# ostadabbas/TePose

Measured on AMD Instinct MI355X. Metric: 16-frame windows/sec (whole node), higher is better.
Workload: dtype f32 via 3 fp16 MFMAs on hi+lo halves (22 bits/operand, fp32 acc); exact-f32 MFMA run = value_exact_fp32; 1 GPU; cfg-C synthetic [8192,16,2133] fp32 windows per GPU, TePose n_layers=2 hidden=1024, random-init weights, synthetic SMPL tables, H36M-14 joint path; seqlen=16, parallelism=clip-sharded dp1

## Files before the change

### tepose_amd/csrc/api.hip

```cpp
#include <stdlib.h>
#include <string.h>

#include <new>

#include "plan.h"

using namespace tepose;

static inline void fault_collected(const tepose_model* m) {
  std::lock_guard<std::mutex> g(m->q_mu);
  ++m->collected;
}

static void read_env_knobs(tepose_model* m) {
  m->opt = options_from_env();
  const char* e = getenv("TEPOSE_EXACT_FP32");
  m->split = m->split_env = !(e && atoi(e) != 0);
  e = getenv("TEPOSE_LARGE_BATCH_KERNELS");
  m->large_scaled = !(e && std::string(e) == "twoacc");
  e = getenv("TEPOSE_GRU_STATE");
  m->state_planes = !(e && std::string(e) == "fp32");
  e = getenv("TEPOSE_COLLAPSE_REGRESSOR");
  m->collapse_env = !(e && atoi(e) == 0);
  e = getenv("TEPOSE_S_MIN_B");
  m->s_min_b = e ? atoi(e) : 640;
  e = getenv("TEPOSE_PERSISTENT");
  m->persist = !(e && atoi(e) == 0);
  e = getenv("TEPOSE_SEQ_SPIN_LIMIT");
  if (e && atol(e) > 0) m->spin_limit = (unsigned)atol(e);
  e = getenv("TEPOSE_TEST_FAULT");
  m->test_fault = e ? (unsigned)atoi(e) : 0u;
  e = getenv("TEPOSE_BLEND16_MIN_N");
  m->blend16_min_n = e ? atoi(e) : 512;
  e = getenv("TEPOSE_GI_BLK");
  m->gi_blk = e ? atoi(e) : 1;
  refresh_kernel_info(m);
}

extern "C" {

int tepose_version(void) { return TEPOSE_ABI_VERSION; }

const char* tepose_build_info(void) {
#ifdef TEPOSE_NO_PACKED_FP32
  return "gfx950 packed_fp32=off";
#else
  return "gfx950 packed_fp32=on";
#endif
}

const char* tepose_kernel_info(const tepose_model* m) { return m ? m->kinfo.c_str() : ""; }

const char* tepose_select_kernels(const tepose_model* m, int B, int T) {
  static thread_local std::string buf;
  if (!m || B < 1 || T < 1) return "";
  buf = describe_plan(m, B, T);
  return buf.c_str();
}

const char* tepose_error_string(int code) {
  switch (code) {
    case 0: return "ok";
    case TEPOSE_E_ARG: return "tepose: bad argument";
    case TEPOSE_E_SHAPE: return "tepose: unsupported shape";
    case TEPOSE_E_WORKSPACE: return "tepose: workspace too small";
    case TEPOSE_E_STATE: return "tepose: model not packed";
    case TEPOSE_E_TIMEOUT: return "tepose: a persistent kernel's bounded wait expired (GPU shared or CU-masked?); "
                                  "outputs of that forward are NaN -- tepose_status() clears, TEPOSE_PERSISTENT=0 / "
                                  "tepose_set_persistent(m, 0) selects the step-per-launch kernels";
    default: return code > 0 ? hipGetErrorString((hipError_t)code) : "tepose: unknown error";
  }
}

int tepose_create(int n_layers, int hidden, tepose_model** out) {
  if (!out || n_layers < 1 || hidden < 1) return TEPOSE_E_ARG;
  if (n_layers > 8 || hidden > 8192) return TEPOSE_E_SHAPE;
  tepose_model* m = new (std::nothrow) tepose_model();
  if (!m) return TEPOSE_E_ARG;
  m->L = n_layers; m->H = hidden; m->Hp = round_up(hidden, 64);
  read_env_knobs(m);
  layout(m);
  *out = m;
  return 0;
}

void tepose_destroy(tepose_model* m) {
  if (!m) return;
  for (hipEvent_t e : m->ev) (void)hipEventDestroy(e);
  for (hipEvent_t e : m->ev_gru) (void)hipEventDestroy(e);
  if (m->fault) (void)hipHostFree(m->fault);
  delete m;
}


int tepose_status_peek(const tepose_model* m) {
  if (!m) return TEPOSE_E_ARG;
  return fault_pending(m) ? TEPOSE_E_TIMEOUT : 0;
}

int tepose_status(tepose_model* m, void* stream) {
  if (!m) return TEPOSE_E_ARG;
  CK(hipStreamSynchronize((hipStream_t)stream));
  if (!m->fault) return 0;
  const unsigned code = __atomic_exchange_n(m->fault, 0u, __ATOMIC_RELAXED);
  if (code) { m->last_fault_code = (int)code; fault_collected(m); }
  return code != 0u ? TEPOSE_E_TIMEOUT : 0;
}

int tepose_forward_status(tepose_model* m, void* workspace, void* stream) {
  if (!m || !workspace) return TEPOSE_E_ARG;
  hipStream_t s = (hipStream_t)stream;
  CK(hipStreamSynchronize(s));
  if (m->fault && __atomic_load_n(m->fault, __ATOMIC_RELAXED) == 0u) {
    std::lock_guard<std::mutex> g(m->q_mu);
    auto it = m->q_gen.find(workspace);
    if (it != m->q_gen.end() && it->second == m->collected) return 0;
  }
  unsigned* sy = (unsigned*)workspace;
  unsigned span[32 + 96 + 1];
  static_assert(sizeof(span) == (32 + 96 + 1) * sizeof(unsigned), "span");
  CK(hipMemcpyAsync(span, sync_gru_status(m, sy), sizeof(span), hipMemcpyDeviceToHost, s));
  CK(hipStreamSynchronize(s));
  const unsigned st[2] = {span[0], span[32 + 96]};
  if ((st[0] | st[1]) == 0u) return 0;
  CK(hipMemsetAsync(sync_gru_status(m, sy), 0, sizeof(unsigned), s));
  CK(hipMemsetAsync(sync_reg_status(m, sy), 0, sizeof(unsigned), s));
  CK(hipStreamSynchronize(s));
  m->last_fault_code = (int)(st[0] ? st[0] : st[1]);
  if (m->fault && __atomic_exchange_n(m->fault, 0u, __ATOMIC_RELAXED) != 0u) fault_collected(m);
  return TEPOSE_E_TIMEOUT;
}

int tepose_set_option(tepose_model* m, const char* name, long value) {
  if (!m || !name) return TEPOSE_E_ARG;
  if (m->enc_packed || m->reg_packed || m->smpl_packed || m->vibe_packed || m->bb_packed) return TEPOSE_E_STATE;
  const char* n = strncmp(name, "TEPOSE_", 7) == 0 ? name + 7 : name;
  if (int* f = option_field(m->opt, n)) *f = (int)value;
  else if (strcmp(n, "S_MIN_B") == 0) m->s_min_b = (int)value;
  else if (strcmp(n, "BLEND16_MIN_N") == 0) m->blend16_min_n = (int)value;
  else if (strcmp(n, "GI_BLK") == 0) m->gi_blk = (int)value;
  else if (strcmp(n, "SEQ_SPIN_LIMIT") == 0) { if (value <= 0) return TEPOSE_E_ARG; m->spin_limit = (unsigned)value; }
  else return TEPOSE_E_ARG;
  refresh_kernel_info(m);
  return 0;
}

long tepose_get_option(const tepose_model* m, const char* name) {
  if (!m || !name) return -1;
  const char* n = strncmp(name, "TEPOSE_", 7) == 0 ? name + 7 : name;
  Options o = m->opt;
  if (const int* f = option_field(o, n)) return *f;
  if (strcmp(n, "S_MIN_B") == 0) return m->s_min_b;
  if (strcmp(n, "BLEND16_MIN_N") == 0) return m->blend16_min_n;
  if (strcmp(n, "GI_BLK") == 0) return m->gi_blk;
  if (strcmp(n, "SEQ_SPIN_LIMIT") == 0) return (long)m->spin_limit;
  return -1;
}

int tepose_fault_code(const tepose_model* m) {
  if (!m) return TEPOSE_E_ARG;
  const unsigned live = m->fault ? __atomic_load_n(m->fault, __ATOMIC_RELAXED) : 0u;
  return live ? (int)live : m->last_fault_code;
}

int tepose_set_persistent(tepose_model* m, int on) {
  if (!m) return TEPOSE_E_ARG;
  __atomic_store_n(&m->persist, on != 0, __ATOMIC_RELAXED);
  return 0;
}

unsigned tepose_debug_kernel_errors(void) { return h3s16c_read_err(); }

int tepose_debug_set_test_fault(tepose_model* m, unsigned bits) {
  if (!m) return TEPOSE_E_ARG;
  m->test_fault = bits;
  return 0;
}

int tepose_uses_persistent(const tepose_model* m, int B, int T) {
  if (!m || B < 1) return 0;
  if (!persist_on(m) || !m->split || B <= m->opt.split_min_m) return 0;
  const int cap = seq_rows_cap(m) > reg_seq_rows_cap(m) ? seq_rows_cap(m) : reg_seq_rows_cap(m);
  (void)T;
  return B <= cap ? 1 : 0;
}

int tepose_create_vibe_ex(int n_layers, int hidden, int bidirectional, int add_linear, tepose_model** out) {
  if (!out || n_layers < 1 || hidden < 1) return TEPOSE_E_ARG;
  if (n_layers > 8 || hidden > 8192) return TEPOSE_E_SHAPE;
  tepose_model* m = new (std::nothrow) tepose_model();
  if (!m) return TEPOSE_E_ARG;
  m->kind = 1; m->L = n_layers; m->H = hidden; m->Hp = round_up(hidden, 64);
  m->vibe_bidir = bidirectional != 0;
  m->vibe_linear = bidirectional != 0 || add_linear != 0;
  read_env_knobs(m);
  layout_vibe(m);
  *out = m;
  return 0;
}

int tepose_create_hmr(tepose_model** out) {
  if (!out) return TEPOSE_E_ARG;
  tepose_model* m = new (std::nothrow) tepose_model();
  if (!m) return TEPOSE_E_ARG;
  m->kind = 2;
  m->L = 1; m->H = m->Hp = 64;
  read_env_knobs(m);
  layout_hmr(m);
  *out = m;
  return 0;
}

int tepose_create_vibe(int n_layers, int hidden, tepose_model** out) {
  return tepose_create_vibe_ex(n_layers, hidden, 0, 1, out);
}

int tepose_vibe_feature_dim(const tepose_model* m) {
  if (!m || m->kind != 1) return 0;
  return m->vibe_linear ? kFeat : m->H;
}

int tepose_profile_enable(tepose_model* m, int on) {
  if (!m) return TEPOSE_E_ARG;
  m->prof = on != 0;
  m->ev_used = 0;
  m->prof_flops = 0.0;
  m->ev_gru_used = 0;
  m->prof_gru_flops = 0.0;
  m->prof_l1_flops = 0.0;
  return 0;
}

int tepose_profile_read(tepose_model* m, double* total_ms, int* n_launches, double* flops_per_launch) {
  if (!m || !total_ms || !n_launches || !flops_per_launch) return TEPOSE_E_ARG;
  double tot = 0.0;
  for (size_t i = 0; i + 1 < m->ev_used; i += 2) {
    CK(hipEventSynchronize(m->ev[i + 1]));
    float ms = 0.f;
    CK(hipEventElapsedTime(&ms, m->ev[i], m->ev[i + 1]));
    tot += ms;
  }
  *total_ms = tot;
  *n_launches = (int)(m->ev_used / 2);
  *flops_per_launch = m->prof_flops;
  m->ev_used = 0;
  return 0;
}

int tepose_profile_read_gru(tepose_model* m, double* total_ms, int* n_forwards, double* flops_per_forward) {
  if (!m || !total_ms || !n_forwards || !flops_per_forward) return TEPOSE_E_ARG;
  double tot = 0.0;
  for (size_t i = 0; i + 1 < m->ev_gru_used; i += 2) {
    CK(hipEventSynchronize(m->ev_gru[i + 1]));
    float ms = 0.f;
    CK(hipEventElapsedTime(&ms, m->ev_gru[i], m->ev_gru[i + 1]));
    tot += ms;
  }
  const int nf = (int)(m->ev_gru_used / (2 * (size_t)m->L));
  *total_ms = tot;
  *n_forwards = nf;
  *flops_per_forward = nf > 0 ? m->prof_gru_flops / nf : 0.0;
  m->ev_gru_used = 0;
  m->prof_gru_flops = 0.0;
  m->prof_l1_flops = 0.0;
  return 0;
}

int tepose_profile_read_l1proj(tepose_model* m, double* total_ms, int* n_forwards, double* flops_per_forward) {
  if (!m || !total_ms || !n_forwards || !flops_per_forward) return TEPOSE_E_ARG;
  const size_t per = 2 * (size_t)m->L;
  double tot = 0.0;
  for (size_t f = 0; (f + 1) * per <= m->ev_gru_used; ++f)
    for (int l = 1; l < m->L; ++l) {
      CK(hipEventSynchronize(m->ev_gru[f * per + 2 * l]));
      float ms = 0.f;
      CK(hipEventElapsedTime(&ms, m->ev_gru[f * per + 2 * l - 1], m->ev_gru[f * per + 2 * l]));
      tot += ms;
    }
  const int nf = (int)(m->ev_gru_used / per);
  *total_ms = tot;
  *n_forwards = nf;
  *flops_per_forward = nf > 0 ? m->prof_l1_flops / nf : 0.0;
  return 0;
}

int tepose_metrics_joints(const float* pred, const float* target, int N, int J, int pelvis_mode, float* mpjpe,
                          float* pa_mpjpe, float* accel, void* stream) {
  if (!pred || !target || !mpjpe || !pa_mpjpe || !accel || N < 1) return TEPOSE_E_ARG;
  if (J < 4 || J > 17 || (pelvis_mode != 0 && pelvis_mode != 1)) return TEPOSE_E_SHAPE;
  CK(launch_metrics_joints(pred, target, N, J, pelvis_mode, mpjpe, pa_mpjpe, accel, (hipStream_t)stream));
  return 0;
}

int tepose_metrics_verts(const float* pred_verts, const float* target_verts, int N, float* mpvpe, void* stream) {
  if (!pred_verts || !target_verts || !mpvpe || N < 1) return TEPOSE_E_ARG;
  CK(launch_metrics_verts(pred_verts, target_verts, N, mpvpe, (hipStream_t)stream));
  return 0;
}

int tepose_filter_one_euro(float* x, int N, int D, float min_cutoff, float beta, float d_cutoff, void* stream) {
  if (!x || N < 1 || D < 1) return TEPOSE_E_ARG;
  CK(launch_one_euro(x, N, D, min_cutoff, beta, d_cutoff, (hipStream_t)stream));
  return 0;
}

int tepose_filter_slerp(const float* rotmat_in, float* rotmat_out, int N, int J, double ratio, void* stream) {
  if (!rotmat_in || !rotmat_out || N < 1 || J < 1) return TEPOSE_E_ARG;
  CK(launch_slerp_smooth(rotmat_in, rotmat_out, N, J, ratio, (hipStream_t)stream));
  return 0;
}

int tepose_rotmat_to_angle_axis(const float* R, int N, float* aa, void* stream) {
  if (!R || !aa || N < 1) return TEPOSE_E_ARG;
  CK(launch_rotmat_to_aa(R, N, aa, (hipStream_t)stream));
  return 0;
}

int tepose_rot6d_to_rotmat(const float* x6, int N, float* R, void* stream) {
  if (!x6 || !R || N < 1) return TEPOSE_E_ARG;
  CK(launch_rot6d_to_rotmat(x6, N, R, (hipStream_t)stream));
  return 0;
}

size_t tepose_gemm_h3_workspace_bytes(int M, int N, int K) {
  if (M < 1 || N < 1 || K < 1) return 0;
  const size_t a = gemm_h3_ws_bytes(M, N, K), b = gemm_h3s_ws_bytes(M, N, K);
  return a > b ? a : b;
}

int tepose_gemm_h3_f32(const float* A, long lda, const float* W, long ldw, const float* bias, float* C, long ldc,
                       int M, int N, int K, void* workspace, size_t ws_bytes, void* stream) {
  if (!A || !W || !C || !workspace || M < 1 || N < 1 || K < 1) return TEPOSE_E_ARG;
  if (K % 32 != 0) return TEPOSE_E_SHAPE;
  if (ws_bytes < gemm_h3_ws_bytes(M, N, K)) return TEPOSE_E_WORKSPACE;
  const char* pe = getenv("TEPOSE_H3S");
  const Options opt = options_from_env();
  if (pe && pe[0] && std::string(pe) != "0" && std::string(pe).rfind("skinny", 0) != 0 && ws_bytes >= gemm_h3s_ws_bytes(M, N, K)) {
    CK(launch_gemm_h3s_f32(A, lda, W, ldw, C, ldc, M, N, K, 256.f, 16384.f, workspace, (hipStream_t)stream, opt, bias, std::string(pe) == "mid" ? 1 : 0));
    return 0;
  }
  CK(launch_gemm_h3_f32(A, lda, W, ldw, bias, C, ldc, M, N, K, workspace, (hipStream_t)stream, opt, pe && std::string(pe) == "skinny" ? 1 : 0));
  return 0;
}

size_t tepose_gemm_workspace_bytes(int N, int K) {
  if (N < 1 || K < 1) return 0;
  return (size_t)round_up(N, 128) * round_up(K, 32) * sizeof(float) + 256;
}

int tepose_gemm_f32(const float* A, long lda, const float* W, long ldw, const float* bias, float* C, long ldc,
                    int M, int N, int K, int relu_a, void* workspace, size_t ws_bytes, void* stream) {
  if (!A || !W || !C || !workspace || M < 1 || N < 1 || K < 1) return TEPOSE_E_ARG;
  if (lda % 4 != 0 || ((uintptr_t)A & 15) != 0 || K % 32 != 0) return TEPOSE_E_SHAPE;
  if (ws_bytes < tepose_gemm_workspace_bytes(N, K)) return TEPOSE_E_WORKSPACE;
  hipStream_t s = (hipStream_t)stream;
  float* wp = (float*)workspace;
  CK((hipError_t)pack(W, ldw, N, K, wp, round_up(N, 128), K, 0, 0, 0, 1, s));
  const GemmArgs g{A, lda, wp, K, C, ldc, bias, nullptr, 0, 1.f, M, N, relu_a};
  CK(launch_gemm(g, s, options_from_env()));
  return 0;
}

}
```

### tepose_amd/csrc/blob.hip

```cpp
#include <algorithm>

#include "hmr.h"
#include "model.h"

using namespace tepose;

namespace {

constexpr size_t kAlignF = 64;

size_t take(size_t& cur, size_t n) {
  const size_t o = cur;
  cur = align_up(cur + n, kAlignF);
  return o;
}

void take_w(size_t& cur, Weight& w, size_t Np, size_t Kp, size_t nb = 0) {
  w.Np = (int)Np; w.Kp = (int)Kp;
  w.w = take(cur, Np * Kp);
  if (nb) w.b = take(cur, nb);
}

void plane(tepose_model* m, size_t& cur, Owner owner, Weight& dst, int rows, size_t R, Fmt f, const Weight* src = nullptr, int k0 = 0) {
  if (f == Fmt::scaled) { dst.s = take(cur, R * dst.Kp); dst.Rs = (int)R; }
// ... 215 lines not shown
    CK(launch_dmm(G3, 1, S, B + m->init, 0, 1, nullptr, 0, nullptr, 0, t2, 1, S, 1, S, 1.0, 0, s));
    CK(launch_dmm(Ss, 1, S, c, 1, 1, t2, 1, nullptr, 0, k0, 1, S, 1, S, 1.0, 0, s));
    CK(launch_d2f_pad(Mf, kFeat, S, kFeat, B + m->mf.w, m->mf.Np, m->mf.Kp, s));
    CK(launch_d2f_pad(k0, S, 1, S, B + m->mf.b, 1, kState, s));
    CK((hipError_t)derive_planes(m, Owner::collapsed_regressor, s));
    CK(hipStreamSynchronize(s));
    return 0;
  };
  const int rc = run();
  (void)hipFree(d);
  if (rc) return rc;
  bool ok = false;
  CK((hipError_t)range_check(m, m->mf.w, m->mf.p, &ok, s));
  m->reg_collapsed = ok;
  return 0;
}

int collapse_tail(tepose_model* m, hipStream_t s) {
  m->tail_collapsed = false;
  if (m->kind != 0 || !m->collapse_env || !m->reg_collapsed || !m->enc_packed) return 0;
  constexpr int S = 157;
  const int Hp = m->Hp, K3 = 3 * Hp;
  float* B = m->blob;
  double* d = nullptr;
  CK(hipMalloc((void**)&d, ((size_t)S * K3 + 2 * S) * sizeof(double)));
  double *Mt = d, *t = Mt + (size_t)S * K3, *kt = t + S;
  auto run = [&]() -> int {
    CK(launch_dmm(B + m->mf.w, 0, kFeat, B + m->wlf.w, 0, Hp, nullptr, 0, nullptr, 0, Mt, K3, S, Hp, kFeat, 0.5, 0, s));
    CK(launch_dmm(B + m->mf.w, 0, kFeat, B + m->wlr.w, 0, 2 * Hp, nullptr, 0, nullptr, 0, Mt + Hp, K3, S, 2 * Hp, kFeat, 0.5, 0, s));
    CK(launch_dmm(B + m->mf.w, 0, kFeat, B + m->wlf.b, 0, 1, nullptr, 0, nullptr, 0, t, 1, S, 1, kFeat, 0.5, 0, s));
    CK(launch_dmm(B + m->mf.w, 0, kFeat, B + m->wlr.b, 0, 1, t, 1, B + m->mf.b, 1, kt, 1, S, 1, kFeat, 0.5, 0, s));
    CK(launch_d2f_pad(Mt, K3, S, K3, B + m->mt.w, m->mt.Np, m->mt.Kp, s));
    CK(launch_d2f_pad(kt, S, 1, S, B + m->mt.b, 1, kState, s));
    CK((hipError_t)derive_planes(m, Owner::collapsed_tail, s));
    CK(hipStreamSynchronize(s));
    return 0;
  };
  const int rc = run();
  (void)hipFree(d);
  if (rc) return rc;
  bool ok = false;
  CK((hipError_t)range_check(m, m->mt.w, m->mt.p, &ok, s));
  m->tail_collapsed = ok;
  return 0;
}
}

extern "C" {

size_t tepose_packed_bytes(const tepose_model* m) { return m ? m->blob_floats * sizeof(float) : 0; }

int tepose_set_blob(tepose_model* m, void* blob, size_t bytes) {
  if (!m || !blob) return TEPOSE_E_ARG;
  if (bytes < m->blob_floats * sizeof(float)) return TEPOSE_E_WORKSPACE;
  m->blob = (float*)blob;
  h3s16c_warm();
  if (!m->fault) {
    unsigned* f = nullptr;
    if (hipHostMalloc((void**)&f, 64, hipHostMallocDefault) == hipSuccess && f) { *f = 0u; m->fault = f; }
    else (void)hipGetLastError();
  }
  return 0;
}

int tepose_adopt_blob(tepose_model* m) {
  if (!m) return TEPOSE_E_ARG;
  if (!m->blob) return TEPOSE_E_STATE;
  BlobHeader h{};
  CK(hipMemcpy(&h, m->blob + m->hdr, sizeof(h), hipMemcpyDeviceToHost));
  const uint64_t lf = ((uint64_t)h.layout_floats_hi << 32) | h.layout_floats_lo;
  if (h.magic != kBlobMagic || h.abi != TEPOSE_ABI_VERSION || h.kind != header_kind(m) || (int)h.L != m->L ||
      (int)h.H != m->H || (int)h.Hp != m->Hp || lf != (uint64_t)m->blob_floats)
    return TEPOSE_E_STATE;
  m->enc_packed = m->kind == 0 && (h.sections & 1u);
  m->vibe_packed = m->kind == 1 && (h.sections & 1u);
  m->reg_packed = (h.sections & 2u) != 0;
  m->smpl_packed = (h.sections & 4u) != 0;
  m->bb_packed = m->kind == 2 && (h.sections & 64u) != 0;
  m->enc_range_ok = m->reg_range_ok = m->smpl_range_ok = m->bb_range_ok = !(h.sections & 8u);
  m->reg_collapsed = m->collapse_env && (h.sections & 16u) != 0;
  m->tail_collapsed = m->collapse_env && m->kind == 0 && (h.sections & 32u) != 0;
  m->split = m->split_env && m->enc_range_ok;
  m->maxdepth = kNJ - 1;
  int max_nnz = kNJ;
  CK(hipMemcpy(&max_nnz, m->blob + m->smpl.lbs_nnz, sizeof(int), hipMemcpyDeviceToHost));
  m->lbs_sparse = max_nnz <= 4 ? 1 : 0;
  for (const PlaneSpec& p : m->planes) {
    if (p.fmt != Fmt::scaled || (p.owner == Owner::encoder && !m->enc_packed)) continue;
    CK(hipMemcpy(&p.dst->scale, m->blob + p.dst->scale_at, sizeof(float), hipMemcpyDeviceToHost));
    if (!(p.dst->scale > 0.f)) p.dst->scale = 1.f;
  }
  return 0;
}

int tepose_fp32_ranges(const tepose_model* m, size_t* offsets, size_t* sizes, int cap) {
  if (!m || !offsets || !sizes) return TEPOSE_E_ARG;
  std::vector<std::pair<size_t, size_t>> derived, r;
  for (const PlaneSpec& p : m->planes) {
    const Weight& w = *p.dst;
    if (p.fmt == Fmt::blocked) derived.emplace_back(w.p, align_up(w.p + (size_t)w.Rp * w.Kp, kAlignF));
    else {
      derived.emplace_back(w.s, align_up(w.s + (size_t)w.Rs * w.Kp, kAlignF));
      derived.emplace_back(w.scale_at / kAlignF * kAlignF, w.scale_at / kAlignF * kAlignF + kAlignF);
    }
  }
  derived.emplace_back(m->blob_floats, m->blob_floats);
  std::sort(derived.begin(), derived.end());
  size_t at = 0;
  for (const auto& d : derived) {
    if (d.first > at) r.emplace_back(at, d.first);
    at = std::max(at, d.second);
  }
  if ((int)r.size() > cap) return TEPOSE_E_ARG;
  for (size_t i = 0; i < r.size(); ++i) { offsets[i] = r[i].first * sizeof(float); sizes[i] = (r[i].second - r[i].first) * sizeof(float); }
  return (int)r.size();
}

int tepose_derive_planes(tepose_model* m, void* stream) {
  if (!m) return TEPOSE_E_ARG;
  if (!m->blob) return TEPOSE_E_STATE;
  int rc = tepose_adopt_blob(m);
  if (rc) return rc;
  hipStream_t s = (hipStream_t)stream;
  const bool enc = m->kind == 0 && m->enc_packed;
  const std::pair<Owner, bool> owners[] = {{Owner::encoder, enc}, {Owner::collapsed_tail, enc && m->tail_collapsed}, {Owner::regressor, m->reg_packed},
                                           {Owner::collapsed_regressor, m->reg_packed && m->reg_collapsed}, {Owner::smpl, m->smpl_packed},
                                           {Owner::backbone, m->bb_packed}};
  for (const auto& o : owners)
    if (o.second) CK((hipError_t)derive_planes(m, o.first, s));
  CK(hipStreamSynchronize(s));
  return 0;
}

int tepose_pack_vibe_encoder(tepose_model* m, const float* const* w, int n_w, void* stream) {
  if (!m || !w || m->kind != 1) return TEPOSE_E_ARG;
  if (!m->blob) return TEPOSE_E_STATE;
  const int L = m->L, H = m->H, Hp = m->Hp, D = m->vibe_bidir ? 2 : 1;
  if (n_w != 4 * L * D + (m->vibe_linear ? 2 : 0)) return TEPOSE_E_ARG;
  for (int i = 0; i < n_w; ++i)
    if (!w[i]) return TEPOSE_E_ARG;
  hipStream_t s = (hipStream_t)stream;
  const Packer pk{m, s};
  const int cmap = D == 2 ? COL_SPLIT2 : COL_PLAIN;
  for (int l = 0; l < L; ++l) {
    const int K = l == 0 ? kFeat : D * H;
    for (int d = 0; d < D; ++d) {
      const float* const* q = w + 4 * (l * D + d);
      const WView ih(m->vibe[l].ih, d * 3 * Hp), hh(m->vibe[l].hh, d * 3 * Hp);
      CK((hipError_t)pk.rows(q[0], K, 3 * H, K, ih, d == D - 1 ? 0 : 3 * Hp, ROW_GATES, l == 0 ? COL_PLAIN : cmap));
      CK((hipError_t)pk.bias(q[2], 3 * H, ih, 3 * Hp, ROW_GATES));
      CK((hipError_t)pk.rows(q[1], H, 3 * H, H, hh, 3 * Hp, ROW_GATES_TILED, COL_PLAIN));
      CK((hipError_t)pk.bias(q[3], 3 * H, hh, 3 * Hp, ROW_GATES));
    }
  }
  if (m->vibe_linear) {
    CK((hipError_t)pk.rows(w[4 * L * D], D * H, kFeat, D * H, m->vlin, 0, ROW_PLAIN, cmap));
    CK((hipError_t)pk.bias(w[4 * L * D + 1], kFeat, m->vlin, kFeat, ROW_PLAIN));
  }
  m->vibe_packed = true;
  CK((hipError_t)range_check(m, m->vibe[0].ih.w, m->w1a.w, &m->enc_range_ok, s));
  return write_header(m, s);
}

int tepose_pack_hmr_backbone(tepose_model* m, const float* const* w, int n_w, void* stream) {
  if (!m || !w || m->kind != 2 || n_w != 5 * kHmrConvs) return TEPOSE_E_ARG;
  if (!m->blob) return TEPOSE_E_STATE;
  for (int i = 0; i < n_w; ++i)
    if (!w[i]) return TEPOSE_E_ARG;
  hipStream_t s = (hipStream_t)stream;
  float* B = m->blob;
  int* err = (int*)(B + m->hdr + 48);
  m->bb_packed = false;
  CK(hipMemsetAsync(err, 0, sizeof(int), s));
  int rc = hmr_walk(1, [&](const ConvStep& c) {
    const float* const* q = w + 5 * c.idx;
    const Weight& bw = m->bb[c.idx];
    return (int)launch_hmr_fold_pack(q[0], q[1], q[2], q[3], q[4], c.l->cout, c.l->cin, c.l->R, B + bw.w, bw.Np, bw.Kp, B + bw.b, err, s);
  });
  if (rc) return rc;
  int bad = 0;
  CK(hipMemcpyAsync(&bad, err, sizeof(int), hipMemcpyDeviceToHost, s));
  CK(hipStreamSynchronize(s));
  if (bad) return TEPOSE_E_ARG;
  CK((hipError_t)derive_planes(m, Owner::backbone, s));
  m->bb_packed = true;
  CK((hipError_t)range_check(m, m->bb[0].w, m->bb[0].p, &m->bb_range_ok, s));
  return write_header(m, s);
}

int tepose_pack_encoder(tepose_model* m, const float* const* w, int n_w, void* stream) {
  if (!m || !w || m->kind != 0) return TEPOSE_E_ARG;
  if (!m->blob) return TEPOSE_E_STATE;
  const int L = m->L, H = m->H, Hp = m->Hp;
  if (n_w != 12 * L + 4) return TEPOSE_E_ARG;
  for (int i = 0; i < n_w; ++i)
    if (!w[i]) return TEPOSE_E_ARG;
  hipStream_t s = (hipStream_t)stream;
  float* B = m->blob;
  const Packer pk{m, s};
  CK(launch_fill(B + m->wih0.w, (size_t)m->wih0.Np * m->wih0.Kp, 0.f, s));
  auto fwd_w = [&](int l, int k) { return w[4 * l + k]; };
  auto rec_w = [&](int l, int rev, int k) { return w[4 * L + 8 * l + 4 * rev + k]; };
  const float* l0[3] = {fwd_w(0, 0), rec_w(0, 1, 0), rec_w(0, 0, 0)};
  const float* l0b[3] = {fwd_w(0, 2), rec_w(0, 1, 2), rec_w(0, 0, 2)};
  for (int d = 0; d < 3; ++d) {
    const WView v(m->wih0, d * 3 * Hp);
    CK((hipError_t)pk.rows(l0[d], kInput, 3 * H, kInput, v, 3 * Hp, ROW_GATES, COL_PLAIN));
    CK((hipError_t)pk.bias(l0b[d], 3 * H, v, 3 * Hp, ROW_GATES));
  }
  for (int l = 0; l < L; ++l) {
    struct { DirW* d; const float *ih, *hh, *bih, *bhh; bool split; } dirs[3] = {
        {&m->fwd[l], fwd_w(l, 0), fwd_w(l, 1), fwd_w(l, 2), fwd_w(l, 3), false},
        {&m->rec_f[l], rec_w(l, 0, 0), rec_w(l, 0, 1), rec_w(l, 0, 2), rec_w(l, 0, 3), true},
        {&m->rec_r[l], rec_w(l, 1, 0), rec_w(l, 1, 1), rec_w(l, 1, 2), rec_w(l, 1, 3), true}};
    for (auto& d : dirs) {
      if (l > 0) {
        const int K = d.split ? 2 * H : H;
        CK((hipError_t)pk.rows(d.ih, K, 3 * H, K, d.d->ih, 0, ROW_GATES, d.split ? COL_SPLIT2 : COL_PLAIN));
        CK((hipError_t)pk.bias(d.bih, 3 * H, d.d->ih, 3 * Hp, ROW_GATES));
      }
      CK((hipError_t)pk.rows(d.hh, H, 3 * H, H, d.d->hh, 0, ROW_GATES_TILED, COL_PLAIN));
      CK((hipError_t)pk.bias(d.bhh, 3 * H, d.d->hh, 3 * Hp, ROW_GATES));
    }
  }
  const float* const* t = w + 12 * L;
  CK((hipError_t)pk.rows(t[0], H, kFeat, H, m->wlf, 0, ROW_PLAIN, COL_PLAIN));
  CK((hipError_t)pk.bias(t[1], kFeat, m->wlf, kFeat, ROW_PLAIN));
  CK((hipError_t)pk.rows(t[2], 2 * H, kFeat, 2 * H, m->wlr, 0, ROW_PLAIN, COL_SPLIT2));
  CK((hipError_t)pk.bias(t[3], kFeat, m->wlr, kFeat, ROW_PLAIN));
  CK((hipError_t)derive_planes(m, Owner::encoder, s));
  m->enc_packed = true;
  CK((hipError_t)range_check(m, m->wih0.w, m->wih0.p, &m->enc_range_ok, s));
  CK((hipError_t)collapse_tail(m, s));
  return write_header(m, s);
}

int tepose_pack_regressor(tepose_model* m, const float* const* w, int n_w, void* stream) {
  if (!m || !w || n_w != 13) return TEPOSE_E_ARG;
  if (!m->blob) return TEPOSE_E_STATE;
  for (int i = 0; i < n_w; ++i)
    if (!w[i]) return TEPOSE_E_ARG;
  hipStream_t s = (hipStream_t)stream;
  float* B = m->blob;
  const Packer pk{m, s};
  const int ld1 = kFeat + kNPose + 13;
  CK((hipError_t)pk.rows(w[0], ld1, 1024, kFeat, m->w1a, 0, ROW_PLAIN, COL_PLAIN));
  CK((hipError_t)pk.bias(w[1], 1024, m->w1a, 1024, ROW_PLAIN));
  CK((hipError_t)pk.rows(w[0] + kFeat, ld1, 1024, 157, m->w1b, 0, ROW_PLAIN, COL_PLAIN));
  CK((hipError_t)pk.rows(w[2], 1024, 1024, 1024, m->w2, 0, ROW_PLAIN, COL_PLAIN));
  CK((hipError_t)pk.bias(w[3], 1024, m->w2, 1024, ROW_PLAIN));
  CK(launch_fill(B + m->wdec.w, (size_t)m->wdec.Np * m->wdec.Kp, 0.f, s));
  CK(launch_fill(B + m->wdec.b, kState, 0.f, s));
  CK(launch_fill(B + m->init, kState, 0.f, s));
  const int rows[3] = {kNPose, 10, 3}, off[3] = {0, kNPose, kNPose + 10};
  for (int i = 0; i < 3; ++i) {
    const WView v(m->wdec, off[i]);
    CK((hipError_t)pk.rows(w[4 + 2 * i], 1024, rows[i], 1024, v, rows[i], ROW_PLAIN, COL_PLAIN));
    CK((hipError_t)pk.bias(w[5 + 2 * i], rows[i], v, rows[i], ROW_PLAIN));
    CK((hipError_t)pack(w[10 + i], 1, rows[i], 1, B + m->init + off[i], rows[i], 1, 0, 0, 0, 1, s));
  }
  CK((hipError_t)derive_planes(m, Owner::regressor, s));
  m->reg_packed = true;
  CK((hipError_t)range_check(m, m->w1a.w, m->smpl.J0, &m->reg_range_ok, s));
  CK((hipError_t)collapse_regressor(m, s));
  CK((hipError_t)collapse_tail(m, s));
  return write_header(m, s);
}

int tepose_pack_smpl(tepose_model* m, const float* v_template, const float* shapedirs,
                     const float* posedirs, const float* J_regressor, const float* lbs_weights,
                     const float* J_regressor_extra, const int32_t* parents_host, void* stream) {
  if (!m || !v_template || !shapedirs || !posedirs || !J_regressor || !lbs_weights ||
      !J_regressor_extra || !parents_host)
    return TEPOSE_E_ARG;
  if (!m->blob) return TEPOSE_E_STATE;
  hipStream_t s = (hipStream_t)stream;
  float* B = m->blob;
  int par[kNJ], dep[kNJ];
  for (int j = 0; j < kNJ; ++j) {
    par[j] = j == 0 ? -1 : parents_host[j];
    if (j > 0 && (par[j] < 0 || par[j] >= j)) return TEPOSE_E_ARG;
  }
  const int maxd = chain_depths(par, dep);
  m->maxdepth = maxd;
  CK(hipMemcpyAsync(B + m->smpl.parents, par, sizeof(par), hipMemcpyHostToDevice, s));
  CK(hipMemcpyAsync(B + m->smpl.depth, dep, sizeof(dep), hipMemcpyHostToDevice, s));
  CK(hipStreamSynchronize(s));
  CK(launch_smpl_consts(v_template, shapedirs, posedirs, J_regressor, B + m->smpl.J0, B + m->smpl.JS,
                        B + m->blend.w, s));
  CK((hipError_t)pack(lbs_weights, kNJ, kNV, kNJ, B + m->smpl.lbsW, kNV, kNJ, 0, 0, 0, 1, s));
  CK(launch_lbs_compact(lbs_weights, (int*)(B + m->smpl.lbs_cidx), B + m->smpl.lbs_cval, (int*)(B + m->smpl.lbs_nnz), s));
  int max_nnz = 0;
  CK(hipMemcpyAsync(&max_nnz, B + m->smpl.lbs_nnz, sizeof(int), hipMemcpyDeviceToHost, s));
  CK(hipStreamSynchronize(s));
  m->lbs_sparse = max_nnz <= 4 ? 1 : 0;
  CK(launch_csr_build(J_regressor_extra, 9, kNV, (int*)(B + m->smpl.xr_ptr), (int*)(B + m->smpl.xr_idx),
                      B + m->smpl.xr_val, 9 * kNV, s));
  CK((hipError_t)derive_planes(m, Owner::smpl, s));
  m->smpl_packed = true;
  CK((hipError_t)range_check(m, m->smpl.J0, m->smpl.lbs_cidx, &m->smpl_range_ok, s));
  return write_header(m, s);
}

size_t tepose_jreg_packed_bytes(void) { return (32 + (size_t)17 * kNV * 2) * 4; }

int tepose_pack_jreg(const float* J, void* packed, void* stream) {
  if (!J || !packed) return TEPOSE_E_ARG;
  int* p = (int*)packed;
  CK(launch_csr_build(J, 17, kNV, p, p + 32, (float*)(p + 32 + 17 * kNV), 17 * kNV, (hipStream_t)stream));
  return 0;
}

}
```

### tepose_amd/csrc/common.h

```cpp
#pragma once
#include <hip/hip_runtime.h>
#include <stdint.h>

#include "formats.h"
#include "shapes.h"

namespace tepose {

typedef _Float16 half_t;
constexpr float kLoScale = 2048.f;
__host__ __device__ inline void split_hi_lo(float a, half_t& hi, half_t& lo) {
  hi = (half_t)a;
  lo = (half_t)((a - (float)hi) * kLoScale);
}
__host__ __device__ inline void split_hi_lo16(float v, half_t& hi, half_t& lo) {
  hi = (half_t)v;
  lo = (half_t)(v - (float)hi);
}

inline dim3 grid_of(const Launch& l) { return dim3(l.gx, l.gy, l.gz); }
inline dim3 block_of(const Launch& l) { return dim3(l.threads); }

struct GemmArgs {
  const float* A; long lda;
  const float* W; int Kp;
  float* C; long ldc;
  const float* bias;
  const float* addend; long ldadd;
  float scale;
  int M, N;
  int relu_a;
};
hipError_t launch_gemm(const GemmArgs& a, hipStream_t s, const Options& o);
hipError_t launch_gemm_tiles(const GemmArgs& a, hipStream_t s, const Options& o);

struct GruDir {
  const float* hprev; long ldh;
  const float* Whh;
  const float* bhh;
  const float* gi; long ldgi;
  float* hout; long ldo;
  long gi_blk = 0;
  const float* hprev_b = nullptr; long hp_blk = 0;
  float* hout_b = nullptr; long ho_blk = 0;
};
struct GruArgs {
  GruDir d[3];
  int ndir;
  int M, Hp;
  int first;
};
hipError_t launch_gru_step(const GruArgs& a, hipStream_t s, const Options& o);
hipError_t launch_gru_step_tiles(const GruArgs& a, hipStream_t s);
hipError_t launch_skinny_gemm(const GemmArgs& a, hipStream_t s);
hipError_t launch_skinny_gru(const GruArgs& a, hipStream_t s);

enum RowMap { ROW_PLAIN = 0, ROW_GATES = 1, ROW_GATES_TILED = 2 };
enum ColMap { COL_PLAIN = 0, COL_SPLIT2 = 1 };
struct PackArgs {
  const float* src; long ld_src; int N, K;
  float* dst; int Np, Kp;
  int rowmap, colmap;
  int H, Hp;
};
hipError_t launch_pack(const PackArgs& a, hipStream_t s);
hipError_t launch_pad_input(const float* x, float* xp, long rows, hipStream_t s);
hipError_t launch_pad_rows(const float* feat, long feat_ld, const float* theta, long theta_ld, float* xp,
                           long rows, hipStream_t s);
hipError_t launch_fill(float* p, size_t n, float v, hipStream_t s);
hipError_t launch_dmm(const void* A, int a64, long lda, const void* B, int b64, long ldb, const double* Cadd, long ldadd,
                      const float* Cadd32, long ldadd32, double* C, long ldc, int M, int N, int K, double alpha,
                      int add_identity, hipStream_t s);
hipError_t launch_d2f_pad(const double* src, long ld, int rows, int cols, float* dst, int Rp, int Cp, hipStream_t s);
hipError_t launch_copy_cols(const float* src, long lds, const float* add, long lda, float* dst, long ldd, long rows,
                            int cols, hipStream_t s);
struct TapView;
hipError_t launch_tap_gather(const TapView& v, const float* ws, float* out, hipStream_t s);
hipError_t launch_init_state(const float* init160, float* xs, int N, hipStream_t s);
hipError_t launch_init_state_rows(const float* init160, const float* pose, const float* shape, const float* cam,
                                  float* xs, int N, hipStream_t s);
hipError_t launch_rotmat_to_aa(const float* R, int N, float* aa, hipStream_t s);
hipError_t launch_rot6d_to_rotmat(const float* x6, int N, float* R, hipStream_t s);

struct SmplConsts {
  const float* J0;
  const float* JS;
  const float* blendW;
  const float* lbsW;
  const int* lbs_cidx;
  const float* lbs_cval;
  int lbs_sparse;
  const int* parents;
  const int* depth;
  int maxdepth;
  const int* xr_ptr;
  const int* xr_idx;
  const float* xr_val;
};
struct JregPacked {
  const int* ptr; const int* idx; const float* val;
};
hipError_t launch_smpl_prep(const SmplConsts& c, const float* xs, int N, float* pf, float* Amat,
                            float* posed, float* rotmat, float* theta, hipStream_t s, void* pf_hi = nullptr,
                            void* pf_lo = nullptr, long pf_kst = 0);
hipError_t launch_smpl_prep_pose(const SmplConsts& c, int mode, const float* pose, int pose_ld,
                                 const float* betas, int betas_ld, int N, float* pf, float* Amat, float* posed,
                                 hipStream_t s, void* pf_hi = nullptr, void* pf_lo = nullptr, long pf_kst = 0);
bool smpl_small_rows_ok(int N, const Options& o);
hipError_t launch_smpl_small(const SmplConsts& c, int mode, const float* pose, int pose_ld, const float* betas, int betas_ld,
                             const float* cam, int cam_ld, int N, float* Amat, float* posed, float* rotmat, float* theta,
                             float* verts, hipStream_t s);
hipError_t launch_smpl_person(const SmplConsts& c, const float* pf, const float* Amat, int N, float* verts, hipStream_t s);
hipError_t launch_lbs_compact(const float* lbsW, int* cidx, float* cval, int* max_nnz, hipStream_t s);
hipError_t launch_smpl_skin(const SmplConsts& c, const float* vposed, const float* Amat, int N,
                            float* verts, hipStream_t s);
hipError_t launch_smpl_joints(const SmplConsts& c, const JregPacked* jr, const float* verts,
                              const float* posed, const float* xs, int N, float* kp3d,
                              float* kp2d, hipStream_t s);
hipError_t launch_csr_build(const float* dense, int rows, int cols, int* ptr, int* idx, float* val,
                            int cap, hipStream_t s);
hipError_t launch_smpl_consts(const float* v_template, const float* shapedirs, const float* posedirs,
                              const float* J_regressor, float* J0, float* JS, float* blendW,
                              hipStream_t s);

hipError_t launch_smpl_joints_bwd(const float* g_j49, int N, float* gsrc, hipStream_t s);
hipError_t launch_smpl_skin_bwd(const SmplConsts& c, const float* vposed, const float* Amat, const float* g_verts, const float* gsrc, int N,
                                float* gvp, float* partial, hipStream_t s);
hipError_t launch_smpl_blend_bwd(const float* blendW, const float* gvp, int N, float* part, float* gf, hipStream_t s);
hipError_t launch_smpl_chain_bwd(const SmplConsts& c, int mode, const float* pose, const float* betas, int N, const float* partial,
                                 const float* gsrc, const float* gf, float* g_pose, float* g_betas, hipStream_t s);

hipError_t launch_metrics_joints(const float* pred, const float* target, int N, int J, int pelvis_mode,
                                 float* mpjpe, float* pa, float* accel, hipStream_t s);
hipError_t launch_metrics_verts(const float* pred, const float* target, int N, float* mpvpe, hipStream_t s);

hipError_t launch_one_euro(float* x, int N, int D, float min_cutoff, float beta, float d_cutoff, hipStream_t s);
hipError_t launch_slerp_smooth(const float* in, float* out, int N, int J, double ratio, hipStream_t s);
hipError_t launch_session_smooth(const float* theta, const float* hist, int S, int T, const int* ops, float* state, float* saved, float min_cutoff,
                                 float beta, float d_cutoff, float* theta_hat, float* pose_hat, float* betas_hat, hipStream_t s);

struct H3Args {
  const half_t *Ah, *Al; long a_kst;
  const half_t *Wh, *Wl; long w_kst;
  int Kp;
  float* C; long ldc;
  const float* bias;
  int M, N;
  const float* addend; long ldadd;
  float scale;
  half_t *Chi, *Clo; long c_kst;
  const float* row_scale;
  int grp_rows, grp_stride;
  float* C2; long ldc2; int c_split;
};
struct GateDir {
  const float* gi; long ldgi;
  const float* bhh;
  const float* hprev; long ldh;
  float* hout; long ldo;
  half_t *hout_hi, *hout_lo; long okst;
  long gi_blk = 0;
  const float* hprev_b = nullptr; long hp_blk = 0;
  float* hout_b = nullptr; long ho_blk = 0;
};
struct H3Batch { H3Args p[3]; GateDir gate[3]; int n; int Hp; };
hipError_t launch_gemm_h3(const H3Batch& b, hipStream_t s, const Options& o);
hipError_t launch_gru_h3(const H3Batch& b, hipStream_t s);
hipError_t launch_skinny_gru_h3(const H3Batch& b, hipStream_t s);
hipError_t launch_skinny_gemm_h3(const H3Args& a, hipStream_t s, const Options& o);
struct H3ArgsBatch { H3Args p[3]; int n; };
hipError_t launch_skinny_gemm_h3_batch(const H3ArgsBatch& b, hipStream_t s, const Options& o);
struct GruSeqStep {
  const float* gi; float* hout;
  int ldgi, ldo;
  unsigned poff, pkst;
};
struct GruSeqArgs {
  GruSeqStep st[3][kSeqMaxT];
  const half_t* whi[3]; const half_t* wlo[3]; long w_kst;
  const float* bhh[3];
  half_t *phi, *plo;
  unsigned* counters;
  unsigned* status;
  unsigned* fault;
  unsigned spin_limit;
  unsigned inject;
  int ndir, T, M, Hp;
  const float* x_gi; const float* x_bhh; float* x_hout;
  int x_ldgi, x_ldo;
  unsigned x_poff, x_pkst;
  half_t *rhi, *rlo;
  unsigned r_off[3], x_roff, r_kst;
  unsigned long long* stamps;
  unsigned long long* gran;
  unsigned tag_base;
};
constexpr unsigned kNoPlane = 0xffffffffu;
struct RegSeqArgs {
  const half_t *fh, *fl; long f_kst;
  const half_t *w1a_h, *w1a_l, *w1b_h, *w1b_l, *w2_h, *w2_l, *wd_h, *wd_l;
  const float *b1, *b2, *bdec;
  const float *init160, *ipose, *ishape, *icam;
  half_t *h1h, *h1l, *h2h, *h2l; long h_kst;
  half_t *xh, *xl; long x_kst;
  float* xs;
  unsigned* counters;
  unsigned* status;
  unsigned* fault; unsigned spin_limit; unsigned inject;
  int N, n_iter;
};
hipError_t launch_reg_seq(const RegSeqArgs& a, hipStream_t s);
int device_cus(const Options& o);
hipError_t launch_gru_seq(const GruSeqArgs& a, hipStream_t s, const Options& o);
struct GateBatch { GateDir d[3]; };
hipError_t launch_gru_first(const GateBatch& gb, int ndir, int M, int Hp, hipStream_t s, int scaled16 = 0, bool rows16 = false);
hipError_t launch_split_planes(const float* src, long ld, long rows, int K, int Kp, long R, void* hi, void* lo,
                               hipStream_t s, int relu = 0);
struct RowPairSrc { const float* f0; const float* th0; const float* f1; long fld, thld; long B; };
hipError_t launch_split_rows(const float* src, long ld, long rows, int K, int Kp, long R, int fmt16, void* hi, void* lo,
                             float* row_scale, hipStream_t s, bool few, void* zero = nullptr, size_t zero_bytes = 0,
                             int permT = 0, const RowPairSrc* pair = nullptr);
hipError_t launch_gemm_h3_f32(const float* A, long lda, const float* W, long ldw, const float* bias, float* C,
                              long ldc, int M, int N, int K, void* ws, hipStream_t s, const Options& o, int kind = 0);
size_t gemm_h3_ws_bytes(int M, int N, int K);
constexpr float kStateScale = 16384.f;
struct H3SArgs {
  const half_t *Ah, *Al; long a_kst;
  const half_t *Wh, *Wl; long w_kst;
  int Kp;
  float* C; long ldc;
  const float* bias;
  float inv_scale;
  int M, N;
  const float* row_scale;
  unsigned* status = nullptr;
  unsigned* fault = nullptr;
  unsigned inject = 0;
  int c_blk_hp = 0;
};
struct H3SBatch { H3SArgs p[3]; GateDir gate[3]; int n; int Hp; float state_scale; };
hipError_t launch_gemm_h3s(const H3SArgs& a, hipStream_t s, const Options& o, int tag = 1);
bool gemm_h3s16_ok(const H3SArgs& a);
hipError_t launch_gemm_h3s16c(const H3SArgs& a, hipStream_t s, int tag, int gm, int walk);
unsigned h3s16c_read_err();
void h3s16c_warm();
bool gru_step16_ok(const H3SBatch& b);
bool gru_step16_planes_ok(const H3SBatch& b);
hipError_t launch_gru_step16(const H3SBatch& b, hipStream_t s, bool planes, int gm);
unsigned* h3s16c_err_of_device();
bool gemm_h3s_mid_ok(const H3SArgs& a);
hipError_t launch_gemm_h3s_mid(const H3SArgs& a, hipStream_t s);
hipError_t launch_split_planes16(const float* src, long ld, long rows, int K, int Kp, long R, float p, void* hi,
                                 void* lo, hipStream_t s);
hipError_t launch_absmax(const float* src, size_t n, float* out, hipStream_t s);
size_t gemm_h3s_ws_bytes(int M, int N, int K);
hipError_t launch_gemm_h3s_f32(const float* A, long lda, const float* W, long ldw, float* C, long ldc, int M, int N,
                               int K, float pA, float pW, void* ws, hipStream_t s, const Options& o, const float* bias = nullptr,
                               int mid = 0);

}
```

### tepose_amd/csrc/forward.hip

```cpp
#include "plan.h"
#include "state.h"
#include "tap.h"

using namespace tepose;

namespace {

struct Carver : Carve {
  char* base; size_t cap;
  Carver(void* p, size_t c) : base((char*)p), cap(c) {}
  float* at(size_t off) const { return base && off != kNoRef ? (float*)base + off : nullptr; }
  float* f(size_t n) { return at(take(n)); }
};

Planes carve_planes(Carver& c, size_t R, size_t C, bool on) {
  Planes p;
  p.hi = (half_t*)c.f(on ? R * C / 2 + 64 : 0);
  p.lo = (half_t*)c.f(on ? R * C / 2 + 64 : 0);
  p.kst = (long)R * 32;
  return p;
}

struct EncWs {
  EncLayout o;
  float* base = nullptr;
  float *xp, *g0, *g0c, *y1, *rs, *rs0;
  half_t *state_hi, *state_lo, *x0h, *x0l;
  unsigned long long* gran;
  unsigned* sync;
  size_t Bs = 0;
  float* at(size_t off) const { return base && off != kNoRef ? base + off : nullptr; }
  float* rows(const StateBuf& b) const { return at(b.off); }
  Planes planes(const StateRef& r) const { return Planes{state_hi + r.p, state_lo + r.p, r.kst}; }
  Planes tail(long k0) const {
    half_t *hi = (half_t*)at(o.tailA.hi), *lo = (half_t*)at(o.tailA.lo);
    return Planes{hi ? hi + o.tailA.k(k0) : nullptr, lo ? lo + o.tailA.k(k0) : nullptr, o.tailA.kst};
  }
};

inline size_t seq_gran_words(const tepose_model* m, const KernelPlan& k) { return k.gran ? (size_t)3 * 2 * kSeqGranRows * m->Hp * 2 : 0; }
inline size_t sync_zero_bytes(const tepose_model* m, const KernelPlan& k) {
  return align_up(sync_words(m) * sizeof(unsigned), 256) + seq_gran_words(m, k) * sizeof(float);
}

void carve_encoder(const tepose_model* m, const KernelPlan& k, int B, int T, Carver& c, EncWs& w) {
  w.o = carve_encoder(EncShape{m->L, m->Hp, B, T, k.h3, k.scaled, k.gblk, sync_words(m), seq_gran_words(m, k)}, c);
  const EncLayout& o = w.o;
  w.base = (float*)c.base; w.Bs = o.Bs;
  w.sync = (unsigned*)c.at(o.sync); w.gran = (unsigned long long*)c.at(o.gran);
  w.xp = c.at(o.xp); w.g0 = c.at(o.g0); w.g0c = c.at(o.g0c); w.y1 = c.at(o.y1); w.rs = c.at(o.rs); w.rs0 = c.at(o.rs0);
  w.state_hi = (half_t*)c.at(o.state_hi); w.state_lo = (half_t*)c.at(o.state_lo);
  w.x0h = (half_t*)c.at(o.x0h); w.x0l = (half_t*)c.at(o.x0l);
}

bool carve_encoder(const tepose_model* m, const KernelPlan& k, int B, int T, void* workspace, size_t bytes, EncWs& w) {
  Carver c(workspace, bytes);
  carve_encoder(m, k, B, T, c, w);
  return c.cur <= bytes;
}

struct Act {
  float* rows = nullptr; long ld = 0; Planes P;
  AOperand A() const { return AOperand{rows, ld, P}; }
};

struct RegWs {
  unsigned* sync;
  bool split;
  Act feat, xs, h1, h2, pf;
  float *base, *amat, *posed, *vposed;
  half_t *pf16h = nullptr, *pf16l = nullptr; float* pfrs = nullptr;
};

void carve_regressor(const tepose_model* m, const KernelPlan& k, int N, Carver& c, RegWs& w) {
  w.split = k.h3;
  w.sync = (unsigned*)c.f(sync_words(m));
  w.feat.ld = kFeat; w.xs.ld = kState; w.h1.ld = w.h2.ld = 1024; w.pf.ld = kBlendK;
  for (Act* a : {&w.feat, &w.xs, &w.h1, &w.h2, &w.pf}) a->P = carve_planes(c, N, a->ld, w.split);
  w.base = c.f((size_t)N * 1024);
  for (Act* a : {&w.h1, &w.h2, &w.xs, &w.pf}) a->rows = c.f((size_t)N * a->ld);
  w.amat = c.f((size_t)N * kNJ * 12);
  w.posed = c.f((size_t)N * kNJ * 3);
  w.vposed = c.f((size_t)N * kVertLd);
  if (k.blend16) {
    w.pf16h = (half_t*)c.f((size_t)N * kBlendK / 2);
    w.pf16l = (half_t*)c.f((size_t)N * kBlendK / 2);
    w.pfrs = c.f((size_t)N);
  }
}

bool carve_regressor(const tepose_model* m, const KernelPlan& k, int N, void* workspace, size_t bytes, RegWs& w) {
  Carver c(workspace, bytes);
  carve_regressor(m, k, N, c, w);
  return c.cur <= bytes;
}

hipError_t init_state(const float* init160, const float* pose, const float* shape, const float* cam, float* xs, int N,
                      hipStream_t s) {
  if (pose || shape || cam) return launch_init_state_rows(init160, pose, shape, cam, xs, N, s);
  return launch_init_state(init160, xs, N, s);
}

H3Args h3_args(const float* blob, const AOperand& A, WView W, float* C, long ldc, int M, int N, const Epilogue& e) {
  const WPlanes wp = w_planes(blob, W, Fmt::blocked);
  H3Args p{A.p.hi, A.p.lo, A.p.kst, wp.hi, wp.lo, wp.kst, W.w->Kp, C, ldc, e.bias, M, N};
  p.addend = e.addend; p.ldadd = e.ldadd; p.scale = e.scale; p.row_scale = A.row_scale;
  if (e.out) { p.Chi = e.out->hi; p.Clo = e.out->lo; p.c_kst = e.out->kst; }
  return p;
}

H3SArgs h3s_args(const tepose_model* m, const AOperand& A, WView W, float* C, long ldc, int M, int N, const Epilogue& e) {
  const WPlanes ws = w_planes(m->blob, W, Fmt::scaled);
  H3SArgs a{A.s.hi, A.s.lo, A.s.kst, ws.hi, ws.lo, ws.kst, W.w->Kp, C, ldc, e.bias, W.w->inv_scale(A.s_scale), M, N, A.row_scale};
  if (e.sync) a.status = e.reg ? sync_reg_status(m, e.sync) : sync_gru_status(m, e.sync);
  a.fault = m->fault;
  a.inject = e.reg ? 0u : (m->test_fault >> 2) & 1u;
  a.c_blk_hp = e.c_blk_hp;
  return a;
}

}

int tepose::product(const tepose_model* m, Mm f, const AOperand& A, WView W, float* C, long ldc, int M, int N, const Epilogue& e, hipStream_t s, bool tail_stage) {
  switch (f) {
    case Mm::f32: return (int)launch_gemm_tiles(f32_args(m->blob, A, W, C, ldc, M, N, e), s, m->opt);
    case Mm::f32_skinny: return (int)launch_skinny_gemm(f32_args(m->blob, A, W, C, ldc, M, N, e), s);
    case Mm::h3:
    case Mm::h3_skinny: {
      H3Batch b{};
      b.p[0] = h3_args(m->blob, A, W, C, ldc, M, N, e);
      if (f == Mm::h3_skinny || (tail_stage && N <= 256)) return (int)launch_skinny_gemm_h3(b.p[0], s, m->opt);
      b.n = 1;
      return (int)launch_gemm_h3(b, s, m->opt);
    }
    case Mm::h3s_mid: return (int)launch_gemm_h3s_mid(h3s_args(m, A, W, C, ldc, M, N, e), s);
    case Mm::h3s0:
    case Mm::h3s: return (int)launch_gemm_h3s(h3s_args(m, A, W, C, ldc, M, N, e), s, m->opt, e.tag);
  }
  return (int)hipErrorInvalidValue;
}

namespace {

int tail_product(const tepose_model* m, const KernelPlan& plan, const AOperand& A, WView W, float* C, long ldc, int M, int N, const Epilogue& e, hipStream_t s) {
  return product(m, plan.tail, A, W, C, ldc, M, N, e, s, true);
}

int blend_shapes(const tepose_model* m, const KernelPlan& k, const RegWs& w, int N, hipStream_t s) {
  AOperand A = w.pf.A();
  Epilogue e;
  if (k.smpl == Smpl::h3s) {
    CK(launch_split_rows(w.pf.rows, kBlendK, N, kBlendK, kBlendK, N, 1, w.pf16h, w.pf16l, w.pfrs, s, k.input_blend == Rows::split_few));
    A.s = Planes{w.pf16h, w.pf16l, (long)N * 16}; A.row_scale = w.pfrs;
    e.sync = w.sync; e.reg = true;
  }
  const Mm f = k.smpl == Smpl::h3s ? Mm::h3s : k.smpl == Smpl::h3 ? Mm::h3 : k.smpl == Smpl::f32_skinny ? Mm::f32_skinny : Mm::f32;
  return product(m, f, A, m->blend, w.vposed, kVertLd, N, 3 * kNV, e, s);
}

template <class Small, class Prep>
int smpl_chain(const tepose_model* m, const KernelPlan& k, const SmplConsts& sc, const RegWs& w, int N, float* verts, hipStream_t s, Small small, Prep prep) {
  if (k.smpl == Smpl::small) return (int)small();
  CK(prep(w.split ? w.pf.P.hi : nullptr, w.split ? w.pf.P.lo : nullptr, w.pf.P.kst));
  CK((hipError_t)blend_shapes(m, k, w, N, s));
  CK(launch_smpl_skin(sc, w.vposed, w.amat, N, verts, s));
  return 0;
}

JregPacked jreg_view(const void* jreg_packed) {
  const int* p = (const int*)jreg_packed;
  return JregPacked{p, p + 32, (const float*)(p + 32 + 17 * kNV)};
}

struct G0Src {
  const float* base; long frame_stride, row_stride;
  int first, ring;
  const float* last; long last_ld;
  const float* single; long single_ld;
  long blk = 0;
};

tepose_model* prof_of(const tepose_model* m) { return m->prof ? const_cast<tepose_model*>(m) : nullptr; }
int prof_mark(std::vector<hipEvent_t>& ev, size_t& used, hipStream_t s) {
  if (ev.size() < used + 1) {
    hipEvent_t e;
    CK(hipEventCreate(&e));
    ev.push_back(e);
  }
  CK(hipEventRecord(ev[used++], s));
  return 0;
}

struct Gi { const float* p; long ld, blk; };
Gi gate_in(const G0Src& src, const EncWs& w, int T, int H3, int l, int dir, const DirStep& d) {
  if (l > 0) return Gi{w.at(d.gi.f), d.gi.ld, d.gi.bst};
  if (d.frame < 0) return Gi{src.single, src.single_ld, 0};
  if (src.last && d.frame == T - 1) return Gi{src.last + (long)dir * H3, src.last_ld, src.blk};
  const int slot = src.ring ? (src.first + d.frame) % src.ring : d.frame;
  return Gi{src.base + (long)slot * src.frame_stride + (long)dir * H3 * (src.blk ? 16 : 1), src.row_stride, src.blk};
}

struct LayerDirs { const DirW* d[3]; };
LayerDirs layer_dirs(const tepose_model* m, int l) { return LayerDirs{{&m->fwd[l], &m->rec_r[l], &m->rec_f[l]}}; }

int project_l1(const tepose_model* m, const KernelPlan& plan, const EncWs& w, Mm f, const StateBuf& in, const DirW& d, const StateBuf& out, int M, hipStream_t s) {
  const int H3 = 3 * m->Hp;
  AOperand A{w.rows(in), d.ih.Kp};
  if (f == Mm::h3s) { A.s = w.planes(in.at(0)); A.s_scale = kStateScale; }
  Epilogue e{w_bias(m->blob, d.ih)};
  e.sync = w.sync; e.c_blk_hp = plan.gblk ? m->Hp : 0;
  return product(m, f, A, d.ih, w.rows(out), H3, M, H3, e, s);
}

int layer_projections(const tepose_model* m, const KernelPlan& plan, const EncWs& w, int B, int T, int l, hipStream_t s) {
  const int Hp = m->Hp, H3 = 3 * Hp;
  const float* Bl = m->blob;
  const long Bs = (long)w.Bs;
  const bool top = l == m->L - 1;
  const StateBuf &inf = w.o.sf[(l - 1) & 1], &inr = w.o.sr[(l - 1) & 1];
  const int MT = (int)(Bs * T);
  const int Mf = top ? B : MT;
  const Mm ff = top ? plan.proj_one : plan.proj_l1;
  if (plan.proj_l1 != Mm::h3 && plan.proj_l1 != Mm::h3_skinny) {
    CK((hipError_t)project_l1(m, plan, w, plan.proj_l1, inf, m->fwd[l], w.o.gf, MT, s));
    CK((hipError_t)project_l1(m, plan, w, plan.proj_l1, inr, m->rec_r[l], w.o.grr, MT, s));
    return project_l1(m, plan, w, ff, inr, m->rec_f[l], w.o.grf, Mf, s);
  }
  const Planes vf = w.planes(inf.at(0)), vr = w.planes(inr.at(0));
  auto mk = [&](const Planes& v, const DirW& d, float* out, int M) {
    return h3_args(Bl, AOperand{nullptr, 0, v}, d.ih, out, H3, M, H3, Epilogue{w_bias(Bl, d.ih)});
  };
  H3Args pa[3] = {mk(vr, m->rec_r[l], w.rows(w.o.grr), MT), mk(vr, m->rec_f[l], w.rows(w.o.grf), Mf), mk(vf, m->fwd[l], w.rows(w.o.gf), MT)};
  const Mm fam[3] = {plan.proj_l1, ff, plan.proj_l1};
  H3ArgsBatch sk{};
  H3Batch big{};
  for (int i = 0; i < 3; ++i) {
    H3Args& a = pa[i];
    if (fam[i] == Mm::h3_skinny) {
      if (a.M == MT && Bs != B) { a.M = B * T; a.grp_rows = B; a.grp_stride = (int)Bs; }
      sk.p[sk.n++] = a;
    }
    else if (big.n == 0 || (big.p[0].M == a.M && big.p[0].N == a.N)) big.p[big.n++] = a;
    else {
      H3Batch one{};
      one.p[0] = a; one.n = 1;
      CK(launch_gemm_h3(one, s, m->opt));
    }
  }
  if (big.n) CK(launch_gemm_h3(big, s, m->opt));
  if (sk.n) CK(launch_skinny_gemm_h3_batch(sk, s, m->opt));
  return 0;
}


GruArgs gru_args(const tepose_model* m, const G0Src& src, const EncWs& w, int B, int T, int l, const CellStep& c, const LayerDirs& dw) {
  GruArgs a{};
  a.M = B; a.Hp = m->Hp; a.first = c.first; a.ndir = c.ndir;
  for (int k = 0; k < c.ndir; ++k) {
    const DirStep& q = c.d[k];
    const Gi gi = gate_in(src, w, T, 3 * m->Hp, l, k, q);
    GruDir& d = a.d[k];
    d.Whh = w_rows(m->blob, dw.d[k]->hh); d.bhh = w_bias(m->blob, dw.d[k]->hh);
    d.gi = gi.p; d.ldgi = gi.ld; d.gi_blk = gi.blk;
    d.hprev = w.at(q.hprev.f); d.ldh = q.hprev.ld;
    d.hout = w.at(q.hout.f); d.ldo = q.hout.ld;
  }
  return a;
}

int launch_cell_step(const tepose_model* m, const KernelPlan& plan, const G0Src& src, const EncWs& w, Step f, int B, int T, int l, const CellStep& c,
                     const LayerDirs& dw, hipStream_t s) {
  if (f == Step::f32_skinny) return (int)launch_skinny_gru(gru_args(m, src, w, B, T, l, c, dw), s);
  if (f == Step::f32) return (int)launch_gru_step_tiles(gru_args(m, src, w, B, T, l, c, dw), s);
  const int Hp = m->Hp, H3 = 3 * Hp;
  const bool s16 = f == Step::s16 || f == Step::s16_planes;
  H3SBatch b16{};
  H3Batch b{};
  GateBatch gb{};
  for (int d = 0; d < c.ndir; ++d) {
    const DirStep& q = c.d[d];
    const Gi gi = gate_in(src, w, T, H3, l, d, q);
    const Planes vo = w.planes(q.hout);
    GateDir g{gi.p, gi.ld, w_bias(m->blob, dw.d[d]->hh), w.at(q.hprev.f), q.hprev.ld, w.at(q.hout.f), q.hout.ld, vo.hi, vo.lo, vo.kst};
    if (s16) {
      g.gi_blk = gi.blk;
      g.hprev_b = w.at(q.hprev.b); g.hp_blk = q.hprev.bst;
      g.hout_b = w.at(q.hout.b); g.ho_blk = q.hout.bst;
    }
    (s16 ? b16.gate[d] : b.gate[d]) = g;
    gb.d[d] = g;
    if (c.first) continue;
    AOperand A;
    Epilogue e;
    if (s16) {
      A.s = w.planes(q.hprev); A.s_scale = kStateScale;
      e.sync = w.sync;
      b16.p[d] = h3s_args(m, A, dw.d[d]->hh, nullptr, 0, B, H3, e);
    } else {
      A.p = w.planes(q.hprev);
      b.p[d] = h3_args(m->blob, A, dw.d[d]->hh, nullptr, 0, B, H3, e);
    }
  }
  if (c.first) return (int)launch_gru_first(gb, c.ndir, B, Hp, s, s16 ? 1 : 0, s16 && plan.first == First::h3_16);
  if (s16) {
    b16.n = c.ndir; b16.Hp = Hp; b16.state_scale = kStateScale;
    const bool planes = f == Step::s16_planes && gru_step16_planes_ok(b16);
    return (int)launch_gru_step16(b16, s, planes, m->opt.gru_gm);
  }
  b.n = c.ndir; b.Hp = Hp;
  if (f == Step::h3_skinny) return (int)launch_skinny_gru_h3(b, s);
  return (int)launch_gru_h3(b, s);
}

int launch_layer_seq(const tepose_model* m, const KernelPlan& plan, const G0Src& src, const EncWs& w, int B, int T, int l, hipStream_t s) {
  const int Hp = m->Hp, H3 = 3 * Hp;
  const bool top = l == m->L - 1;
  const LayerDirs dw = layer_dirs(m, l);
  GruSeqArgs sq{};
  sq.ndir = top ? 2 : 3;
  for (int d = 0; d < sq.ndir; ++d) {
    const WPlanes wp = w_planes(m->blob, dw.d[d]->hh, Fmt::blocked);
    sq.whi[d] = wp.hi; sq.wlo[d] = wp.lo; sq.w_kst = wp.kst; sq.bhh[d] = w_bias(m->blob, dw.d[d]->hh);
  }
  for (int st = 0; st < T; ++st) {
    const CellStep c = cell_step(w.o, m->L, T, l, st);
    for (int d = 0; d < c.ndir; ++d) {
      const DirStep& q = c.d[d];
      const Gi gi = gate_in(src, w, T, H3, l, d, q);
      GruSeqStep& e = sq.st[d][st];
      e.gi = gi.p; e.ldgi = (int)gi.ld; e.hout = w.at(q.hout.f); e.ldo = (int)q.hout.ld;
      e.poff = (unsigned)q.hout.p; e.pkst = (unsigned)q.hout.kst;
    }
  }
  sq.phi = w.state_hi; sq.plo = w.state_lo;
  sq.counters = sync_gru(w.sync, l); sq.status = sync_gru_status(m, w.sync);
  sq.fault = m->fault; sq.spin_limit = m->spin_limit; sq.inject = (m->test_fault & 1u) ? 1u : 0u;
  sq.T = T; sq.M = B; sq.Hp = Hp;
  sq.gran = (l == 0 ? plan.step0 : plan.step1) == Step::seq_gran ? w.gran : nullptr; sq.tag_base = (unsigned)l * 64u;
  const Planes tail = w.tail(0);
  sq.rhi = tail.hi; sq.rlo = tail.lo; sq.r_kst = (unsigned)tail.kst;
  sq.r_off[0] = sq.r_off[1] = sq.r_off[2] = sq.x_roff = kNoPlane;
  if (top) {
    const DirStep x = cell_top_rec_fwd(w.o, l).d[0];
    const Gi gi = gate_in(src, w, T, H3, l, 2, x);
    sq.x_gi = gi.p; sq.x_ldgi = (int)gi.ld;
    sq.x_bhh = w_bias(m->blob, m->rec_f[l].hh); sq.x_hout = w.at(x.hout.f); sq.x_ldo = (int)x.hout.ld;
    sq.x_poff = (unsigned)x.hout.p; sq.x_pkst = (unsigned)x.hout.kst;
    sq.r_off[0] = (unsigned)w.o.tailA.k(0); sq.x_roff = (unsigned)w.o.tailA.k(Hp); sq.r_off[1] = (unsigned)w.o.tailA.k(2 * Hp);
  }
  return (int)launch_gru_seq(sq, s, m->opt);
}

int encoder_tail(const tepose_model* m, const KernelPlan& plan, const EncWs& w, int B, int T, int is_train, float* feat, const Planes* feat_planes,
                 float* xs_out, bool tail_planes_done, hipStream_t s) {
  const int Hp = m->Hp;
  const float* Bl = m->blob;
  const float *hlast = w.rows(w.o.pf[(T - 1) & 1]), *ytop = w.rows(w.o.ytop);
  const Planes tailA = w.tail(0), tailF = tailA, tailR = w.tail(Hp);
  const AOperand Af{hlast, Hp, tailF}, Ar{ytop, 2 * Hp, tailR};
  const float *blf = w_bias(Bl, m->wlf), *blr = w_bias(Bl, m->wlr);
  if (plan.h3) {
    if (!tail_planes_done) {
      CK(launch_split_planes(hlast, Hp, B, Hp, Hp, B, tailF.hi, tailF.lo, s, 1));
      CK(launch_split_planes(ytop, 2 * Hp, B, 2 * Hp, 2 * Hp, B, tailR.hi, tailR.lo, s, 1));
    }
    const AOperand A{nullptr, 0, tailA};
    if (!is_train && xs_out && plan.tail_collapsed) return tail_product(m, plan, A, m->mt, xs_out, kState, B, kState, Epilogue{w_bias(Bl, m->mt)}, s);
    if (!is_train) return tail_product(m, plan, A, m->wlfr, feat, kFeat, B, kFeat, Epilogue{blf, blr, 0, 0.5f, 0, feat_planes}, s);
    CK((hipError_t)tail_product(m, plan, Af, m->wlf, feat, 2 * kFeat, B, kFeat, Epilogue{blf}, s));
    return tail_product(m, plan, Ar, m->wlr, feat + kFeat, 2 * kFeat, B, kFeat, Epilogue{blr}, s);
  }
  float* yf = is_train ? feat : w.y1;
  const long ld = is_train ? 2 * kFeat : kFeat;
  CK((hipError_t)tail_product(m, plan, Af, m->wlf, yf, ld, B, kFeat, Epilogue{blf, nullptr, 0, 0.f, 1}, s));
  const Epilogue er = is_train ? Epilogue{blr, nullptr, 0, 0.f, 1} : Epilogue{blr, w.y1, kFeat, 0.5f, 1};
  return tail_product(m, plan, Ar, m->wlr, is_train ? feat + kFeat : feat, ld, B, kFeat, er, s);
}

int layer_cells(const tepose_model* m, const KernelPlan& plan, const G0Src& src, const EncWs& w, int B, int T, int l, bool seq, hipStream_t s) {
  if (seq) return launch_layer_seq(m, plan, src, w, B, T, l, s);
  const Step f = l == 0 ? plan.step0 : plan.step1;
  const LayerDirs dw = layer_dirs(m, l);
  for (int st = 0; st < T; ++st) CK((hipError_t)launch_cell_step(m, plan, src, w, f, B, T, l, cell_step(w.o, m->L, T, l, st), dw, s));
  if (l < m->L - 1) return 0;
  return launch_cell_step(m, plan, src, w, f, B, T, l, cell_top_rec_fwd(w.o, l), LayerDirs{{&m->rec_f[l], nullptr, nullptr}}, s);
}

int encoder_core(const tepose_model* m, const KernelPlan& plan, const G0Src& src, int B, int T, int is_train, float* feat, EncWs& w,
                 hipStream_t s, const Planes* feat_planes = nullptr, bool sync_zeroed = false, float* xs_out = nullptr) {
  tepose_model* pm = prof_of(m);
  const int L = m->L;
  if (src.blk && !plan.gblk) return (int)hipErrorInvalidValue;
  const bool seq = plan.step0 == Step::seq || plan.step0 == Step::seq_gran;
  if (!sync_zeroed && w.sync) CK(hipMemsetAsync(w.sync, 0, seq ? sync_zero_bytes(m, plan) : sync_words(m) * sizeof(unsigned), s));
  for (int l = 0; l < L; ++l) {
    const bool top = l == L - 1;
    if (l > 0) {
      CK((hipError_t)layer_projections(m, plan, w, B, T, l, s));
      if (pm) pm->prof_l1_flops += 2.0 * 3.0 * m->H * ((double)B * T * m->H + (double)B * T * 2.0 * m->H + (double)(top ? B : B * T) * 2.0 * m->H);
    }
    if (pm) CK((hipError_t)prof_mark(pm->ev_gru, pm->ev_gru_used, s));
    CK((hipError_t)layer_cells(m, plan, src, w, B, T, l, seq, s));
    if (pm) {
      CK((hipError_t)prof_mark(pm->ev_gru, pm->ev_gru_used, s));
      pm->prof_gru_flops += 2.0 * B * 3.0 * m->H * m->H * (2.0 * T + (top ? 1 : T));
    }
  }
  return encoder_tail(m, plan, w, B, T, is_train, feat, feat_planes, xs_out, seq, s);
}

SmplConsts smpl_consts(const tepose_model* m) {
  const float* Bl = m->blob;
  SmplConsts sc{};
  sc.J0 = Bl + m->smpl.J0; sc.JS = Bl + m->smpl.JS; sc.blendW = w_rows(Bl, m->blend);
  sc.lbsW = Bl + m->smpl.lbsW; sc.lbs_cidx = (const int*)(Bl + m->smpl.lbs_cidx); sc.lbs_cval = Bl + m->smpl.lbs_cval;
  sc.lbs_sparse = m->lbs_sparse; sc.parents = (const int*)(Bl + m->smpl.parents);
  sc.depth = (const int*)(Bl + m->smpl.depth); sc.maxdepth = m->maxdepth;
  sc.xr_ptr = (const int*)(Bl + m->smpl.xr_ptr); sc.xr_idx = (const int*)(Bl + m->smpl.xr_idx);
  sc.xr_val = Bl + m->smpl.xr_val;
  return sc;
}

int encoder_fwd_impl(const tepose_model* m, const KernelPlan& plan, const float* x, int B, int T, int is_train, float* feat,
                     void* workspace, size_t ws_bytes, void* stream, const Planes* feat_planes, bool* wrote_planes, float* xs_out) {
  if (wrote_planes) *wrote_planes = false;
  if (!m || m->kind != 0 || !x || !feat || !workspace || B < 1 || T < 1) return TEPOSE_E_ARG;
  if (!m->enc_packed) return TEPOSE_E_STATE;
  if ((size_t)B * T > (1u << 30) / 4) return TEPOSE_E_SHAPE;
  hipStream_t s = (hipStream_t)stream;
  EncWs w;
  if (!carve_encoder(m, plan, B, T, workspace, ws_bytes, w)) return TEPOSE_E_WORKSPACE;
  const int L = m->L, Hp = m->Hp;
  const float* Bl = m->blob;
  const long BT = (long)B * T;
  const int H3 = 3 * Hp;

  const int ld0 = (L >= 2 ? 9 : 6) * Hp;
  half_t* xh = (half_t*)w.xp;
  half_t* xl = xh + (size_t)BT * kInputP;
  const bool g0s = plan.projection == Mm::h3s0 || plan.projection == Mm::h3s_mid, g0blk = plan.g0blk;
  if (plan.input == Rows::pad) {
    CK(launch_pad_input(x, w.xp, BT, s));
    if (w.sync) CK(hipMemsetAsync(w.sync, 0, sync_zero_bytes(m, plan), s));
  } else {
    CK(launch_split_rows(x, kInput, BT, kInput, kInputP, BT, g0s ? 1 : 0, xh, xl, w.rs, s, plan.input == Rows::split_few, (void*)w.sync,
                         w.sync ? sync_zero_bytes(m, plan) : 0, g0blk ? T : 0));
  }
  {
    tepose_model* pm = prof_of(m);
    if (pm) CK((hipError_t)prof_mark(pm->ev, pm->ev_used, s));
    const AOperand A{w.xp, kInputP, {xh, xl, BT * 32}, {xh, xl, BT * 16}, 1.f, w.rs};
    Epilogue e{w_bias(Bl, m->wih0)};
    e.sync = w.sync; e.c_blk_hp = g0blk ? Hp : 0; e.tag = 0;
    CK((hipError_t)product(m, plan.projection, A, m->wih0, w.g0, ld0, (int)BT, ld0, e, s));
    if (pm) {
      CK((hipError_t)prof_mark(pm->ev, pm->ev_used, s));
      pm->prof_flops = 2.0 * (double)BT * (double)(L >= 2 ? 9 : 6) * m->H * kInput;
    }
  }
  if (L == 1) {
    AOperand A{w.xp + (long)(T - 1) * kInputP, (long)T * kInputP};
    if (plan.proj_one == Mm::h3) {
      CK(launch_split_rows(x + (long)(T - 1) * kInput, (long)T * kInput, B, kInput, kInputP, B, 0, w.x0h, w.x0l, w.rs0, s,
                           plan.input_x0 == Rows::split_few));
      A.p = Planes{w.x0h, w.x0l, (long)B * 32}; A.row_scale = w.rs0;
    }
    const WView rec(m->wih0, 6 * Hp);
    CK((hipError_t)product(m, plan.proj_one, A, rec, w.g0c, H3, B, H3, Epilogue{w_bias(Bl, rec)}, s));
  }

  G0Src src{w.g0, ld0, (long)T * ld0, 0, 0, nullptr, 0, w.g0c, H3};
  if (g0blk) { src.frame_stride = (long)B * ld0; src.row_stride = ld0; src.blk = (long)ld0 * 16; }
  if (feat_planes) {
    const char* end = (const char*)(feat_planes->lo + (size_t)B * kFeat + 128);
    const char* first_live = (const char*)w.rows(L >= 2 ? w.o.gf : w.o.pf[0]);
    if (!plan.h3 || is_train || end > first_live) feat_planes = nullptr;
  }
  if (wrote_planes) *wrote_planes = feat_planes != nullptr;
  return encoder_core(m, plan, src, B, T, is_train, feat, w, s, feat_planes, true, xs_out);
}

struct ProjWs {
  float* xp; Planes P; float* rs = nullptr; size_t bytes;
  AOperand A() const { return AOperand{xp, kInputP, P, {}, 1.f, rs}; }
};
ProjWs carve_projection(void* workspace, size_t M, bool h3) {
  Carver c(workspace, 0);
  ProjWs w;
  w.xp = c.f(M * kInputP);
  const size_t xbytes = c.cur;
  if (h3) {
    half_t* hi = (half_t*)c.f(xbytes / 4 + 128);
    w.P = Planes{hi, hi ? hi + xbytes / 4 : nullptr, (long)M * 32};
    w.rs = c.f(M);
  }
  w.bytes = c.cur;
  return w;
}

int project_frames_impl(const tepose_model* m, const KernelPlan& plan, const float* feat, long feat_ld, const float* theta, long theta_ld, int B,
                        float* out, long out_ld, void* workspace, hipStream_t s) {
  const ProjWs w = carve_projection(workspace, B, plan.h3);
  CK(launch_pad_rows(feat, feat_ld, theta, theta_ld, w.xp, B, s));
  if (plan.h3)
    CK(launch_split_rows(w.xp, kInputP, B, kInputP, kInputP, B, 0, w.P.hi, w.P.lo, w.rs, s, plan.input == Rows::split_few));
  return product(m, plan.projection, w.A(), m->wih0, out, out_ld, B, 9 * m->Hp, Epilogue{w_bias(m->blob, m->wih0)}, s);
}

int project_frame_pair_impl(const tepose_model* m, const KernelPlan& plan, const float* feat_prev, const float* feat_new, long feat_ld,
                            const float* theta_prev, long theta_ld, int B, float* out_prev, long out_prev_ld, float* out_new, long out_new_ld,
                            void* workspace, size_t ws_bytes, void* stream, void* zero, size_t zero_bytes, bool* zeroed) {
  if (zeroed) *zeroed = false;
  if (!feat_prev || !feat_new || !theta_prev || !out_prev || !out_new || !workspace) return TEPOSE_E_ARG;
  if (!m->enc_packed) return TEPOSE_E_STATE;
  if (ws_bytes < tepose_project_frames_workspace_bytes(m, 2 * B)) return TEPOSE_E_WORKSPACE;
  hipStream_t s = (hipStream_t)stream;
  if (!plan.pair) {
    CK((hipError_t)project_frames_impl(m, plan, feat_prev, feat_ld, theta_prev, theta_ld, B, out_prev, out_prev_ld, workspace, s));
    return project_frames_impl(m, plan, feat_new, feat_ld, nullptr, 0, B, out_new, out_new_ld, workspace, s);
  }
  const int M = 2 * B;
  const ProjWs w = carve_projection(workspace, M, true);
  const RowPairSrc pr{feat_prev, theta_prev, feat_new, feat_ld, theta_ld, B};
  const bool z = zero && zero_bytes && zero_bytes % 16 == 0;
  CK(launch_split_rows(nullptr, 0, M, kInput, kInputP, M, 0, w.P.hi, w.P.lo, w.rs, s, plan.input_pair == Rows::split_few, z ? zero : nullptr,
                       z ? zero_bytes : 0, 0, &pr));
  if (zeroed) *zeroed = z;
  H3Args p = h3_args(m->blob, w.A(), m->wih0, out_prev, out_prev_ld, M, 9 * m->Hp, Epilogue{w_bias(m->blob, m->wih0)});
  p.C2 = out_new; p.ldc2 = out_new_ld; p.c_split = B;
  CK(launch_skinny_gemm_h3(p, s, m->opt));
  return 0;
}

int regressor_impl(const tepose_model* m, const KernelPlan& plan, const float* feat, int N, int n_iter, const float* init_pose,
                   const float* init_shape, const float* init_cam, const void* jreg_packed, float* theta, float* verts,
                   float* kp_3d, float* kp_2d, float* rotmat, void* workspace, size_t ws_bytes, void* stream,
                   bool feat_planes_ready, bool sync_zeroed, const float* xs_ready = nullptr) {
  if (!m || !feat || !theta || !verts || !kp_3d || !kp_2d || !rotmat || !workspace || N < 1 || n_iter < 0)
    return TEPOSE_E_ARG;
  if (!m->reg_packed || !m->smpl_packed) return TEPOSE_E_STATE;
  hipStream_t s = (hipStream_t)stream;
  RegWs w;
  if (!carve_regressor(m, plan, N, workspace, ws_bytes, w)) return TEPOSE_E_WORKSPACE;
  const float* Bl = m->blob;
  if (!sync_zeroed && w.sync) CK(hipMemsetAsync(w.sync, 0, sync_words(m) * sizeof(unsigned), s));
  AOperand Afeat = w.feat.A();
  Afeat.rows = feat;
  const bool collapsed = !xs_ready && plan.reg_collapsed && n_iter == 3 && !init_pose && !init_shape && !init_cam;
  if (!xs_ready && plan.h3 && !feat_planes_ready) CK(launch_split_planes(feat, kFeat, N, kFeat, kFeat, N, w.feat.P.hi, w.feat.P.lo, s));
  Epilogue e;
  if (xs_ready) {
    w.xs.rows = const_cast<float*>(xs_ready);
  } else if (collapsed) {
    e.bias = w_bias(Bl, m->mf);
    CK((hipError_t)tail_product(m, plan, Afeat, m->mf, w.xs.rows, kState, N, kState, e, s));
  } else if (plan.reg == Reg::seq) {
    RegSeqArgs ra{};
    ra.fh = w.feat.P.hi; ra.fl = w.feat.P.lo; ra.f_kst = w.feat.P.kst;
    WPlanes p;
    p = w_planes(Bl, m->w1a, Fmt::blocked); ra.w1a_h = p.hi; ra.w1a_l = p.lo;
    p = w_planes(Bl, m->w1b, Fmt::blocked); ra.w1b_h = p.hi; ra.w1b_l = p.lo;
    p = w_planes(Bl, m->w2, Fmt::blocked); ra.w2_h = p.hi; ra.w2_l = p.lo;
    p = w_planes(Bl, m->wdec, Fmt::blocked); ra.wd_h = p.hi; ra.wd_l = p.lo;
    ra.b1 = w_bias(Bl, m->w1a); ra.b2 = w_bias(Bl, m->w2); ra.bdec = w_bias(Bl, m->wdec);
    ra.init160 = Bl + m->init; ra.ipose = init_pose; ra.ishape = init_shape; ra.icam = init_cam;
    ra.h1h = w.h1.P.hi; ra.h1l = w.h1.P.lo; ra.h2h = w.h2.P.hi; ra.h2l = w.h2.P.lo; ra.h_kst = w.h1.P.kst;
    ra.xh = w.xs.P.hi; ra.xl = w.xs.P.lo; ra.x_kst = w.xs.P.kst;
    ra.xs = w.xs.rows; ra.counters = sync_reg(m, w.sync); ra.status = sync_reg_status(m, w.sync);
    ra.fault = m->fault; ra.spin_limit = m->spin_limit; ra.inject = (m->test_fault & 2u) ? 1u : 0u;
    ra.N = N; ra.n_iter = n_iter;
    CK(launch_reg_seq(ra, s));
  } else {
    e.bias = w_bias(Bl, m->w1a);
    CK((hipError_t)tail_product(m, plan, Afeat, m->w1a, w.base, 1024, N, 1024, e, s));
    CK(init_state(Bl + m->init, init_pose, init_shape, init_cam, w.xs.rows, N, s));
    if (plan.h3) CK(launch_split_planes(w.xs.rows, kState, N, kState, kState, N, w.xs.P.hi, w.xs.P.lo, s));
    Epilogue e1{nullptr, w.base, 1024}, e2{w_bias(Bl, m->w2)}, e3{w_bias(Bl, m->wdec), w.xs.rows, kState};
    e1.out = &w.h1.P; e2.out = &w.h2.P; e3.out = &w.xs.P;
    for (int it = 0; it < n_iter; ++it) {
      CK((hipError_t)tail_product(m, plan, w.xs.A(), m->w1b, w.h1.rows, 1024, N, 1024, e1, s));
      CK((hipError_t)tail_product(m, plan, w.h1.A(), m->w2, w.h2.rows, 1024, N, 1024, e2, s));
      CK((hipError_t)tail_product(m, plan, w.h2.A(), m->wdec, w.xs.rows, kState, N, kState, e3, s));
    }
  }
  const SmplConsts sc = smpl_consts(m);
  const float* xs = w.xs.rows;
  CK((hipError_t)smpl_chain(
      m, plan, sc, w, N, verts, s,
      [&] { return launch_smpl_small(sc, 0, xs, kState, xs + kNPose, kState, xs + 154, kState, N, w.amat, w.posed, rotmat, theta, verts, s); },
      [&](half_t* ph, half_t* pl, long kst) { return launch_smpl_prep(sc, xs, N, w.pf.rows, w.amat, w.posed, rotmat, theta, s, ph, pl, kst); }));
  const JregPacked jr = jreg_packed ? jreg_view(jreg_packed) : JregPacked{};
  CK(launch_smpl_joints(sc, jreg_packed ? &jr : nullptr, verts, w.posed, xs, N, kp_3d, kp_2d, s));
  return 0;
}

struct FwdWs { char* rest; size_t rest_bytes; float* feat; };
FwdWs split_workspace(void* workspace, size_t ws_bytes, int B) {
  const size_t feat_bytes = align_up((size_t)B * 2 * kFeat * sizeof(float), 256);
  const size_t rest_bytes = (ws_bytes & ~(size_t)255) - feat_bytes;
  return FwdWs{(char*)workspace, rest_bytes, (float*)((char*)workspace + rest_bytes)};
}

int forward_cached_impl(const tepose_model* m, const KernelPlan& plan, const float* ring_base, int ring, int first_slot, long clip_stride,
                        const float* newest, long newest_ld, int B, int T, const void* jreg_packed, float* theta, float* verts, float* kp_3d,
                        float* kp_2d, float* rotmat, void* workspace, size_t ws_bytes, void* stream, bool sync_zeroed) {
  if (m->kind != 0 || !ring_base || !newest || !workspace || ring < T - 1 || ring < 1 || first_slot < 0 || first_slot >= ring)
    return TEPOSE_E_ARG;
  if (!m->enc_packed) return TEPOSE_E_STATE;
  { const int rc = forward_begin(m, workspace); if (rc) return rc; }
  if (ws_bytes < tepose_workspace_bytes(m, B, T)) return TEPOSE_E_WORKSPACE;
  hipStream_t s = (hipStream_t)stream;
  const auto [rest, rest_bytes, feat] = split_workspace(workspace, ws_bytes, B);
  EncWs w;
  if (!carve_encoder(m, plan, B, T, rest, rest_bytes, w)) return TEPOSE_E_WORKSPACE;
  const int ld0 = 9 * m->Hp;
  G0Src src{ring_base, ld0, clip_stride, first_slot, ring, newest, newest_ld, newest + 6 * m->Hp, newest_ld};
  float* xs = plan.tail_collapsed ? feat : nullptr;
  int rc = encoder_core(m, plan, src, B, T, 0, feat, w, s, nullptr, sync_zeroed, xs);
  if (rc) return rc;
  return regressor_impl(m, plan, feat, B, 3, nullptr, nullptr, nullptr, jreg_packed, theta, verts, kp_3d, kp_2d, rotmat, rest,
                        rest_bytes, stream, false, true, xs);
}

}

extern "C" {

size_t tepose_workspace_bytes(const tepose_model* m, int B, int T) {
  if (!m || B < 1 || T < 1) return 0;
  Carver c(nullptr, 0);
  EncWs e;
  carve_encoder(m, select_kernels(m, B, T), B, T, c, e);
  RegWs r;
  c.f((size_t)B * 2 * kFeat);
  carve_regressor(m, select_kernels(m, 2 * B, T), 2 * B, c, r);
  return c.cur + 256;
}

size_t tepose_project_frames_workspace_bytes(const tepose_model* m, int B) {
  if (!m || B < 1) return 0;
  return carve_projection(nullptr, B, select_kernels(m, B, 1, true).h3).bytes;
}

size_t tepose_vibe_workspace_bytes(const tepose_model* m, int B, int N) {
  if (!m || m->kind != 1 || B < 1 || N < 1) return 0;
  const size_t BN = (size_t)B * N, Hp = m->Hp, D = m->vibe_bidir ? 2 : 1;
  return align_up(BN * D * 3 * Hp * 4, 256) + 2 * align_up(BN * D * Hp * 4, 256) + 256;
}

int tepose_vibe_encoder_fwd(const tepose_model* m, const float* x, int B, int N, int use_residual, float* feat,
                            void* workspace, size_t ws_bytes, void* stream) {
  if (!m || m->kind != 1 || !x || !feat || !workspace || B < 1 || N < 1) return TEPOSE_E_ARG;
  if (!m->vibe_packed) return TEPOSE_E_STATE;
  if (ws_bytes < tepose_vibe_workspace_bytes(m, B, N)) return TEPOSE_E_WORKSPACE;
  hipStream_t s = (hipStream_t)stream;
  const int L = m->L, Hp = m->Hp, H3 = 3 * Hp, D = m->vibe_bidir ? 2 : 1;
  const long BN = (long)B * N;
  Carver c(workspace, ws_bytes);
  float* G = c.f((size_t)BN * D * H3);
  float* S[2] = {c.f((size_t)BN * D * Hp), c.f((size_t)BN * D * Hp)};
  const float* Bl = m->blob;
  const float* in = x;
  int ldin = kFeat;
  for (int l = 0; l < L; ++l) {
    const Weight& ih = m->vibe[l].ih;
    CK(launch_gemm(f32_args(Bl, AOperand{in, ldin}, ih, G, (long)D * H3, (int)BN, D * H3, Epilogue{w_bias(Bl, ih)}), s, m->opt));
    float* So = S[l & 1];
    for (int t = 0; t < N; ++t) {
      GruArgs a{};
      a.M = B; a.Hp = Hp; a.first = t == 0; a.ndir = D;
      for (int d = 0; d < D; ++d) {
        const int td = d ? N - 1 - t : t, tp = d ? td + 1 : td - 1;
        GruDir& q = a.d[d];
        const WView hh(m->vibe[l].hh, d * H3);
        q.Whh = w_rows(Bl, hh); q.bhh = w_bias(Bl, hh);
        q.gi = G + (long)td * D * H3 + (long)d * H3; q.ldgi = (long)N * D * H3;
        q.hprev = So + (long)tp * D * Hp + (long)d * Hp; q.ldh = (long)N * D * Hp;
        q.hout = So + (long)td * D * Hp + (long)d * Hp; q.ldo = (long)N * D * Hp;
      }
      CK(launch_gru_step(a, s, m->opt));
    }
    in = So; ldin = D * Hp;
  }
  if (!m->vibe_linear)
    return (int)launch_copy_cols(in, ldin, (use_residual && m->H == kFeat) ? x : nullptr, kFeat, feat, m->H, BN, m->H, s);
  Epilogue e{w_bias(Bl, m->vlin)};
  e.relu_a = 1;
  if (use_residual) { e.addend = x; e.ldadd = kFeat; }
  CK(launch_gemm(f32_args(Bl, AOperand{in, ldin}, m->vlin, feat, kFeat, (int)BN, kFeat, e), s, m->opt));
  return 0;
}

int tepose_smpl_fwd(const tepose_model* m, int pose2rot, const float* pose, const float* betas, int N, float* verts,
                    float* joints49, void* workspace, size_t ws_bytes, void* stream) {
  if (!m || !pose || !betas || !verts || !workspace || N < 1) return TEPOSE_E_ARG;
  if (!m->smpl_packed) return TEPOSE_E_STATE;
  hipStream_t s = (hipStream_t)stream;
  const KernelPlan plan = select_kernels(m, N, 1);
  RegWs w;
  if (!carve_regressor(m, plan, N, workspace, ws_bytes, w)) return TEPOSE_E_WORKSPACE;
  SmplConsts sc = smpl_consts(m);
  const int mode = pose2rot ? 1 : 2, pose_ld = pose2rot ? 72 : 216;
  CK((hipError_t)smpl_chain(
      m, plan, sc, w, N, verts, s,
      [&] { return launch_smpl_small(sc, mode, pose, pose_ld, betas, 10, nullptr, 0, N, w.amat, w.posed, nullptr, nullptr, verts, s); },
      [&](half_t* ph, half_t* pl, long kst) { return launch_smpl_prep_pose(sc, mode, pose, pose_ld, betas, 10, N, w.pf.rows, w.amat, w.posed, s, ph, pl, kst); }));
  if (joints49) CK(launch_smpl_joints(sc, nullptr, verts, w.posed, nullptr, N, joints49, nullptr, s));
  return 0;
}

struct SmplBwdWs { float *gsrc, *gvp, *skin_part, *blend_part, *gf; };
static KernelPlan smpl_bwd_plan(const tepose_model* m, int N) {
  KernelPlan k = select_kernels(m, N, 1);
  if (k.smpl == Smpl::small) k.smpl = N <= gemm_skinny_max_m(m->opt) ? Smpl::f32_skinny : Smpl::f32;
  return k;
}
static void carve_smpl_bwd(const tepose_model* m, const KernelPlan& k, int N, Carver& c, RegWs& w, SmplBwdWs& b) {
  carve_regressor(m, k, N, c, w);
  const SmplBwdFloats f = smpl_bwd_floats(N);
  b.gsrc = c.f(f.gsrc); b.gvp = c.f(f.gvp); b.skin_part = c.f(f.skin_part); b.blend_part = c.f(f.blend_part); b.gf = c.f(f.gf);
}

size_t tepose_smpl_bwd_workspace_bytes(const tepose_model* m, int N) {
  if (!m || N < 1 || N > kSmplBwdMaxN) return 0;
  Carver c(nullptr, 0);
  RegWs w;
  SmplBwdWs b;
  carve_smpl_bwd(m, smpl_bwd_plan(m, N), N, c, w, b);
  return c.cur + 256;
}

int tepose_smpl_bwd(const tepose_model* m, int pose2rot, const float* pose, const float* betas, int N, const float* g_verts,
                    const float* g_joints49, float* g_pose, float* g_betas, void* workspace, size_t ws_bytes, void* stream) {
  if (!m || !pose || !betas || !workspace) return TEPOSE_E_ARG;
  if (!g_verts && !g_joints49 && (g_pose || g_betas)) return TEPOSE_E_ARG;
  if (N < 1 || N > kSmplBwdMaxN) return TEPOSE_E_SHAPE;
  if (!m->smpl_packed) return TEPOSE_E_STATE;
  hipStream_t s = (hipStream_t)stream;
  const KernelPlan plan = smpl_bwd_plan(m, N);
  Carver c(workspace, ws_bytes);
  RegWs w;
  SmplBwdWs b;
  carve_smpl_bwd(m, plan, N, c, w, b);
  if (c.cur > ws_bytes) return TEPOSE_E_WORKSPACE;
  if (!g_pose && !g_betas) return 0;
  SmplConsts sc = smpl_consts(m);
  const int mode = pose2rot ? 1 : 2, pose_ld = pose2rot ? 72 : 216;
  CK(launch_smpl_prep_pose(sc, mode, pose, pose_ld, betas, 10, N, w.pf.rows, w.amat, w.posed, s, w.split ? w.pf.P.hi : nullptr,
                           w.split ? w.pf.P.lo : nullptr, w.pf.P.kst));
  CK((hipError_t)blend_shapes(m, plan, w, N, s));
  CK(launch_smpl_joints_bwd(g_joints49, N, b.gsrc, s));
  CK(launch_smpl_skin_bwd(sc, w.vposed, w.amat, g_verts, b.gsrc, N, b.gvp, b.skin_part, s));
  CK(launch_smpl_blend_bwd(sc.blendW, b.gvp, N, b.blend_part, b.gf, s));
  CK(launch_smpl_chain_bwd(sc, mode, pose, betas, N, b.skin_part, b.gsrc, b.gf, g_pose, g_betas, s));
  return 0;
}

int tepose_joints_from_verts(const tepose_model* m, const void* jreg_packed, const float* verts, int N, float* kp_3d, void* stream) {
  if (!m || !jreg_packed || !verts || !kp_3d || N < 1) return TEPOSE_E_ARG;
  if (!m->smpl_packed) return TEPOSE_E_STATE;
  SmplConsts sc = smpl_consts(m);
  const JregPacked jr = jreg_view(jreg_packed);
  CK(launch_smpl_joints(sc, &jr, verts, nullptr, nullptr, N, kp_3d, nullptr, (hipStream_t)stream));
  return 0;
}

int tepose_smpl_fwd_per_person(const tepose_model* m, const float* pose, const float* betas, int N, float* verts,
                               void* workspace, size_t ws_bytes, void* stream) {
  if (!m || !pose || !betas || !verts || !workspace || N < 1) return TEPOSE_E_ARG;
  if (!m->smpl_packed) return TEPOSE_E_STATE;
  hipStream_t s = (hipStream_t)stream;
  RegWs w;
  if (!carve_regressor(m, select_kernels(m, N, 1), N, workspace, ws_bytes, w)) return TEPOSE_E_WORKSPACE;
  SmplConsts sc = smpl_consts(m);
  CK(launch_smpl_prep_pose(sc, 1, pose, 72, betas, 10, N, w.pf.rows, w.amat, w.posed, s));
  CK(launch_smpl_person(sc, w.pf.rows, w.amat, N, verts, s));
  return 0;
}

int tepose_smpl_verts_from_theta(const tepose_model* m, const float* theta, int N, float* verts, void* workspace,
                                 size_t ws_bytes, void* stream) {
  if (!m || !theta || !verts || !workspace || N < 1) return TEPOSE_E_ARG;
  if (!m->smpl_packed) return TEPOSE_E_STATE;
  hipStream_t s = (hipStream_t)stream;
  const KernelPlan plan = select_kernels(m, N, 1);
  RegWs w;
  if (!carve_regressor(m, plan, N, workspace, ws_bytes, w)) return TEPOSE_E_WORKSPACE;
  SmplConsts sc = smpl_consts(m);
  return smpl_chain(
      m, plan, sc, w, N, verts, s,
      [&] { return launch_smpl_small(sc, 1, theta + 3, kTheta, theta + 75, kTheta, nullptr, 0, N, w.amat, nullptr, nullptr, nullptr, verts, s); },
      [&](half_t* ph, half_t* pl, long kst) { return launch_smpl_prep_pose(sc, 1, theta + 3, kTheta, theta + 75, kTheta, N, w.pf.rows, w.amat, nullptr, s, ph, pl, kst); });
}

int tepose_encoder_fwd(const tepose_model* m, const float* x, int B, int T, int is_train, float* feat,
                       void* workspace, size_t ws_bytes, void* stream) {
  if (m) { const int rc = forward_begin(m, workspace); if (rc) return rc; }
  if (!m || B < 1 || T < 1) return TEPOSE_E_ARG;
  return encoder_fwd_impl(m, select_kernels(m, B, T), x, B, T, is_train, feat, workspace, ws_bytes, stream, nullptr, nullptr, nullptr);
}

int tepose_encoder_tap(const tepose_model* m, int B, int T, int stage, int layer, int dir, int step, float* out, size_t out_floats, int* form,
                       const void* workspace, size_t ws_bytes, void* stream) {
  if (!m || m->kind != 0 || !out || !workspace || B < 1 || T < 1 || stage < kTapGi || stage > kTapTail) return TEPOSE_E_ARG;
  if (!m->enc_packed) return TEPOSE_E_STATE;
  if ((size_t)B * T > (1u << 30) / 4) return TEPOSE_E_SHAPE;
  const KernelPlan plan = select_kernels(m, B, T);
  Carver c(const_cast<void*>(workspace), ws_bytes);
  EncWs w;
  carve_encoder(m, plan, B, T, c, w);
  const TapPlan tp{m->L, m->Hp, B, T, plan.h3, plan.g0blk, plan.step0 == Step::s16_planes, plan.step1 == Step::s16_planes};
  TapView v;
  if (!tap_resolve(w.o, tp, stage, layer, dir, step, &v) || out_floats != v.count()) return TEPOSE_E_SHAPE;
  if (c.cur > ws_bytes) return TEPOSE_E_WORKSPACE;
  if (form) *form = v.form;
  CK(launch_tap_gather(v, (const float*)workspace, out, (hipStream_t)stream));
  return 0;
}

int tepose_project_frames(const tepose_model* m, const float* feat, long feat_ld, const float* theta, long theta_ld,
                          int B, float* out, long out_ld, void* workspace, size_t ws_bytes, void* stream) {
  if (!m || m->kind != 0 || !feat || !out || !workspace || B < 1) return TEPOSE_E_ARG;
  if (!m->enc_packed) return TEPOSE_E_STATE;
  if (ws_bytes < tepose_project_frames_workspace_bytes(m, B)) return TEPOSE_E_WORKSPACE;
  return project_frames_impl(m, select_kernels(m, B, 1, true), feat, feat_ld, theta, theta_ld, B, out, out_ld, workspace, (hipStream_t)stream);
}

int tepose_project_frame_pair(const tepose_model* m, const float* feat_prev, const float* feat_new, long feat_ld, const float* theta_prev,
                              long theta_ld, int B, float* out_prev, long out_prev_ld, float* out_new, long out_new_ld, void* workspace,
                              size_t ws_bytes, void* stream) {
  if (!m || m->kind != 0 || B < 1) return TEPOSE_E_ARG;
  return project_frame_pair_impl(m, select_kernels(m, B, 1, true), feat_prev, feat_new, feat_ld, theta_prev, theta_ld, B, out_prev, out_prev_ld,
                                 out_new, out_new_ld, workspace, ws_bytes, stream, nullptr, 0, nullptr);
}

int tepose_window_step(const tepose_model* m, const float* feat_prev, const float* feat_new, long feat_ld, const float* theta_prev, long theta_ld,
                       float* out_prev, long out_prev_ld, float* newest, long newest_ld, const float* ring_base, int ring, int first_slot,
                       long clip_stride, int B, int T, const void* jreg_packed, float* theta, float* verts, float* kp_3d, float* kp_2d, float* rotmat,
                       void* workspace, size_t ws_bytes, void* pair_workspace, size_t pair_ws_bytes, void* stream) {
  if (!m || m->kind != 0 || !workspace || B < 1 || T < 1) return TEPOSE_E_ARG;
  if (!m->enc_packed) return TEPOSE_E_STATE;
  { const int rc = forward_begin(m, workspace); if (rc) return rc; }
  if (ws_bytes < tepose_workspace_bytes(m, B, T)) return TEPOSE_E_WORKSPACE;
  const KernelPlan plan = select_kernels(m, B, T, true);
  void* zero = nullptr;
  size_t zero_bytes = 0;
  {
    const size_t rest_bytes = split_workspace(workspace, ws_bytes, B).rest_bytes;
    EncWs w;
    if (!carve_encoder(m, plan, B, T, workspace, rest_bytes, w)) return TEPOSE_E_WORKSPACE;
    if (w.sync) { zero = (void*)w.sync; zero_bytes = sync_zero_bytes(m, plan); }
  }
  bool zeroed = false;
  int rc = project_frame_pair_impl(m, plan, feat_prev, feat_new, feat_ld, theta_prev, theta_ld, B, out_prev, out_prev_ld, newest, newest_ld,
                                   pair_workspace, pair_ws_bytes, stream, zero, zero_bytes, &zeroed);
  if (rc) return rc;
  return forward_cached_impl(m, plan, ring_base, ring, first_slot, clip_stride, newest, newest_ld, B, T, jreg_packed, theta, verts, kp_3d, kp_2d,
                             rotmat, workspace, ws_bytes, stream, zeroed);
}

int tepose_forward_cached(const tepose_model* m, const float* ring_base, int ring, int first_slot, long clip_stride,
                          const float* newest, long newest_ld, int B, int T, const void* jreg_packed, float* theta,
                          float* verts, float* kp_3d, float* kp_2d, float* rotmat, void* workspace, size_t ws_bytes,
                          void* stream) {
  if (!m || B < 1 || T < 1) return TEPOSE_E_ARG;
  return forward_cached_impl(m, select_kernels(m, B, T, true), ring_base, ring, first_slot, clip_stride, newest, newest_ld, B, T, jreg_packed, theta,
                             verts, kp_3d, kp_2d, rotmat, workspace, ws_bytes, stream, false);
}

int tepose_regressor_fwd(const tepose_model* m, const float* feat, int N, int n_iter, const void* jreg_packed,
                         float* theta, float* verts, float* kp_3d, float* kp_2d, float* rotmat,
                         void* workspace, size_t ws_bytes, void* stream) {
  return tepose_regressor_fwd_init(m, feat, N, n_iter, nullptr, nullptr, nullptr, jreg_packed, theta, verts, kp_3d, kp_2d,
                                   rotmat, workspace, ws_bytes, stream);
}

int tepose_regressor_fwd_init(const tepose_model* m, const float* feat, int N, int n_iter, const float* init_pose,
                              const float* init_shape, const float* init_cam, const void* jreg_packed, float* theta,
                              float* verts, float* kp_3d, float* kp_2d, float* rotmat, void* workspace, size_t ws_bytes,
                              void* stream) {
  if (m) { const int rc = forward_begin(m, workspace); if (rc) return rc; }
  if (!m || N < 1) return TEPOSE_E_ARG;
  return regressor_impl(m, select_kernels(m, N, 1), feat, N, n_iter, init_pose, init_shape, init_cam, jreg_packed, theta, verts, kp_3d, kp_2d,
                        rotmat, workspace, ws_bytes, stream, false, false);
}

int tepose_forward(const tepose_model* m, const float* x, int B, int T, const void* jreg_packed, float* theta,
                   float* verts, float* kp_3d, float* kp_2d, float* rotmat, void* workspace, size_t ws_bytes,
                   void* stream) {
  if (!m || !workspace || B < 1 || T < 1) return TEPOSE_E_ARG;
  { const int rc = forward_begin(m, workspace); if (rc) return rc; }
  if (ws_bytes < tepose_workspace_bytes(m, B, T)) return TEPOSE_E_WORKSPACE;
  const KernelPlan plan = select_kernels(m, B, T);
  const auto [rest, rest_bytes, feat] = split_workspace(workspace, ws_bytes, B);
  RegWs rw;
  (void)carve_regressor(m, plan, B, rest, rest_bytes, rw);
  if (!rw.sync) return TEPOSE_E_WORKSPACE;
  bool wrote = false;
  float* xs = plan.tail_collapsed ? feat : nullptr;
  int rc = encoder_fwd_impl(m, plan, x, B, T, 0, feat, rest, rest_bytes, stream, rw.split && !xs ? &rw.feat.P : nullptr, &wrote, xs);
  if (rc) return rc;
  return regressor_impl(m, plan, feat, B, 3, nullptr, nullptr, nullptr, jreg_packed, theta, verts, kp_3d, kp_2d, rotmat, rest,
                        rest_bytes, stream, wrote, true, xs);
}

}
```

### tepose_amd/csrc/model.h

```cpp
#pragma once
#include "../../include/tepose_amd.h"

#include <mutex>
#include <string>
#include <unordered_map>
#include <vector>

#include "common.h"

namespace tepose {

struct Weight {
  size_t w = 0; int Np = 0, Kp = 0;
  size_t b = 0;
  size_t p = 0; int Rp = 0;
  size_t s = 0; int Rs = 0;
  size_t scale_at = 0;
  float scale = 1.f;
  float inv_scale(float a_scale = 1.f) const { return 1.f / (a_scale * scale); }
};
enum class Fmt : unsigned char { blocked, scaled };
struct WView {
  const Weight* w; int row0, k0;
  WView(const Weight& wt, int r0 = 0, int k = 0) : w(&wt), row0(r0), k0(k) {}
};

struct DirW { Weight ih, hh; };

struct SmplOff {
  size_t J0, JS, lbsW, lbs_cidx, lbs_cval, lbs_nnz, parents, depth, xr_ptr, xr_idx, xr_val;
};

enum class Owner : unsigned char { encoder, regressor, smpl, collapsed_regressor, collapsed_tail, backbone };
struct PlaneSpec {
  Owner owner;
  const Weight* src; int rows;
  Weight* dst; int k0; Fmt fmt;
};

}

struct tepose_model {
  int kind = 0;
  std::vector<tepose::Weight> bb;
  bool bb_packed = false, bb_range_ok = true;
  std::vector<tepose::DirW> vibe;
  bool vibe_bidir = false, vibe_linear = true;
  tepose::Weight vlin;
  bool vibe_packed = false;
  int L = 0, H = 0, Hp = 0;
  size_t hdr = 0;
  float* blob = nullptr;
  size_t blob_floats = 0;
  std::vector<tepose::PlaneSpec> planes;
  bool enc_packed = false, reg_packed = false, smpl_packed = false;
  tepose::Weight wih0;
  bool large_scaled = true;
  bool state_planes = true;
  std::string kinfo;
  std::vector<tepose::DirW> fwd, rec_f, rec_r;
  tepose::Weight wlf, wlr;
  tepose::Weight wlfr;
  tepose::Weight w1a, w1b, w2, wdec;
  size_t init = 0;
  tepose::Weight blend;
  tepose::Weight mf, mt;
  bool reg_collapsed = false, tail_collapsed = false;
  bool collapse_env = true;
  tepose::SmplOff smpl{};
  int maxdepth = 0;
  int lbs_sparse = 0;
  bool split = true;
  bool split_env = true;
  bool enc_range_ok = true, reg_range_ok = true, smpl_range_ok = true;
  int s_min_b = 640;
  tepose::Options opt;
  unsigned* fault = nullptr;
  bool persist = true;
  unsigned spin_limit = 1u << 21;
  int blend16_min_n = 512;
  int gi_blk = 1;
  int last_fault_code = 0;
  mutable std::mutex q_mu;
  mutable std::unordered_map<const void*, unsigned> q_gen;
  mutable unsigned collected = 0;
  unsigned test_fault = 0;
  bool prof = false;
  std::vector<hipEvent_t> ev;
  size_t ev_used = 0;
  double prof_flops = 0.0;
  std::vector<hipEvent_t> ev_gru;
  size_t ev_gru_used = 0;
  double prof_gru_flops = 0.0;
  double prof_l1_flops = 0.0;
};

namespace tepose {

#define CK(expr)                      \
  do {                                \
    hipError_t e__ = (expr);          \
    if (e__ != hipSuccess) return (int)e__; \
  } while (0)

struct WPlanes { const half_t *hi, *lo; long kst; };
inline WPlanes w_planes(const float* blob, WView v, Fmt f) {
  const Weight& w = *v.w;
  const size_t tile = f == Fmt::scaled ? 16 : 32, R = f == Fmt::scaled ? w.Rs : w.Rp;
  const half_t* hi = (const half_t*)(blob + (f == Fmt::scaled ? w.s : w.p)) + (size_t)v.row0 * tile + (size_t)v.k0 * R;
  return WPlanes{hi, hi + R * w.Kp, (long)(R * tile)};
}
inline const float* w_rows(const float* blob, WView v) { return blob + v.w->w + (size_t)v.row0 * v.w->Kp + v.k0; }
inline const float* w_bias(const float* blob, WView v) { return v.w->b ? blob + v.w->b + v.row0 : nullptr; }

enum class Mm : unsigned char;
struct Planes { half_t *hi = nullptr, *lo = nullptr; long kst = 0; };
struct AOperand {
  const float* rows = nullptr; long lda = 0;
  Planes p;
  Planes s; float s_scale = 1.f;
  const float* row_scale = nullptr;
};
struct Epilogue {
  const float* bias = nullptr;
  const float* addend = nullptr; long ldadd = 0;
  float scale = 0.f;
  int relu_a = 0;
  const Planes* out = nullptr;
  int c_blk_hp = 0;
  unsigned* sync = nullptr; bool reg = false;
  int tag = 1;
};
int product(const tepose_model* m, Mm f, const AOperand& A, WView W, float* C, long ldc, int M, int N, const Epilogue& e, hipStream_t s, bool tail_stage = false);
inline GemmArgs f32_args(const float* blob, const AOperand& A, WView W, float* C, long ldc, int M, int N, const Epilogue& e) {
  return GemmArgs{A.rows, A.lda, w_rows(blob, W), W.w->Kp, C, ldc, e.bias, e.addend, e.ldadd, e.scale != 0.f ? e.scale : 1.f, M, N, e.relu_a};
}

inline bool fault_pending(const tepose_model* m) { return m->fault && __atomic_load_n(m->fault, __ATOMIC_RELAXED) != 0u; }
inline int forward_begin(const tepose_model* m, const void* workspace) {
  if (fault_pending(m)) return TEPOSE_E_TIMEOUT;
  if (workspace) {
    std::lock_guard<std::mutex> g(m->q_mu);
    if (m->q_gen.size() > 4096) m->q_gen.clear();
    m->q_gen[workspace] = m->collected;
  }
  return 0;
}
inline int seq_rows_cap(const tepose_model* m) { return m->opt.seq_max_m > 64 ? 64 : m->opt.seq_max_m; }
inline int reg_seq_rows_cap(const tepose_model* m) { return m->opt.reg_seq_max_n > 64 ? 64 : m->opt.reg_seq_max_n; }
inline bool persist_on(const tepose_model* m) {
  return __atomic_load_n(&m->persist, __ATOMIC_RELAXED) && m->fault != nullptr;
}

inline size_t sync_words(const tepose_model* m) { return (size_t)m->L * 96 + 32 + 96 + 32; }
inline unsigned* sync_gru(unsigned* sy, int l) { return sy + (size_t)l * 96; }
inline unsigned* sync_gru_status(const tepose_model* m, unsigned* sy) { return sy + (size_t)m->L * 96; }
inline unsigned* sync_reg(const tepose_model* m, unsigned* sy) { return sy + (size_t)m->L * 96 + 32; }
inline unsigned* sync_reg_status(const tepose_model* m, unsigned* sy) { return sy + (size_t)m->L * 96 + 32 + 96; }

void layout(tepose_model* m);
void layout_vibe(tepose_model* m);
void layout_hmr(tepose_model* m);
int pack(const float* src, long ld, int N, int K, float* dst, int Np, int Kp, int rowmap, int colmap, int H, int Hp, hipStream_t s);

}
```

### tepose_amd/csrc/plan.h

```cpp
#pragma once
#include "model.h"

namespace tepose {

enum class Rows : unsigned char { pad, split_few, split };
enum class Mm : unsigned char { f32, f32_skinny, h3, h3_skinny, h3s_mid, h3s0, h3s };
enum class Step : unsigned char { f32, f32_skinny, h3, h3_skinny, seq, seq_gran, s16, s16_planes };
enum class First : unsigned char { f32, f32_skinny, h3, h3_16, in_seq };
enum class Reg : unsigned char { loop, seq };
enum class Smpl : unsigned char { small, f32, f32_skinny, h3, h3s };

struct KernelPlan {
  bool h3 = false;
  bool scaled = false;
  bool gblk = false;
  bool g0blk = false;
  bool gran = false;
  bool blend16 = false;
  bool reg_collapsed = false;
  bool tail_collapsed = false;
  bool pair = false;
  Rows input = Rows::pad;
  Rows input_x0 = Rows::pad;
  Rows input_pair = Rows::pad;
  Rows input_blend = Rows::pad;
  Mm projection = Mm::f32;
  Mm proj_l1 = Mm::f32;
  Mm proj_one = Mm::f32;
  First first = First::f32;
  Step step0 = Step::f32, step1 = Step::f32;
  Mm tail = Mm::f32;
  Reg reg = Reg::loop;
  Smpl smpl = Smpl::f32;
};

KernelPlan select_kernels(const tepose_model* m, int B, int T, bool window = false, bool assume_ready = false);
std::string describe_plan(const tepose_model* m, int B, int T);
void refresh_kernel_info(tepose_model* m);

}
```

### tepose_amd/csrc/plan.hip

```cpp
#include "plan.h"

namespace tepose {

KernelPlan select_kernels(const tepose_model* m, int B, int T, bool window, bool assume_ready) {
  KernelPlan k;
  const Options& o = m->opt;
  const int L = m->L, Hp = m->Hp;
  const long BT = (long)B * T;
  const bool persist = assume_ready ? m->persist : persist_on(m);
  auto split = [&](long rows, int Kp, int permT) { return split_rows_few_ok(rows, Kp, permT, o) ? Rows::split_few : Rows::split; };
  auto f32 = [&](long rows) { return rows <= gemm_skinny_max_m(o) ? Mm::f32_skinny : Mm::f32; };
  auto h3 = [&](long rows) { return rows <= o.skinny_max_m ? Mm::h3_skinny : Mm::h3; };
  k.h3 = m->split && B > o.split_min_m;
  k.scaled = k.h3 && m->large_scaled && B >= m->s_min_b;
  k.gblk = k.scaled && m->gi_blk && Hp % 32 == 0;
  const bool planes_state = k.gblk && m->state_planes && B % 128 == 0;
  k.gran = m->split && B <= gru_seq_gran_rows(o) && gru_seq_shape_ok(Hp);
  const bool g0big = k.h3 && m->large_scaled && L >= 2 && BT >= 8192;
  const bool g0mid = k.h3 && m->large_scaled && L >= 2 && !g0big && BT >= o.g0_mid_min_rows && BT > 128 && h3s_mid_cols_ok(9 * Hp) && g0_mid_fewer_rounds(BT, Hp);
  if (window) {
    k.pair = k.h3 && 2 * B <= o.skinny_max_m;
    k.input = k.h3 ? split(B, kInputP, 0) : Rows::pad;
    k.input_pair = split(2L * B, kInputP, 0);
    k.projection = k.h3 ? h3(B) : f32(B);
  } else {
    k.g0blk = g0big && k.gblk && B % 16 == 0;
    k.input = k.h3 ? split(BT, kInputP, k.g0blk ? T : 0) : Rows::pad;
    k.projection = !k.h3 ? f32(BT) : g0big ? Mm::h3s0 : g0mid ? Mm::h3s_mid : BT <= o.g0_skinny_max_m ? Mm::h3_skinny : Mm::h3;
  }
  const long Bs = k.h3 ? round_up(B, 16) : B;
  k.input_x0 = split(B, kInputP, 0);
  if (!k.h3) { k.proj_l1 = f32(BT); k.proj_one = f32(B); }
  else if (L == 1) k.proj_l1 = k.proj_one = Mm::h3;
  else if (k.scaled) k.proj_l1 = k.proj_one = Mm::h3s;
  else {
    k.proj_l1 = Bs * T <= o.skinny_max_m && BT <= o.l1_skinny_max_rows ? Mm::h3_skinny : Mm::h3;
    k.proj_one = B <= o.skinny_max_m && B <= o.l1_skinny_max_rows ? Mm::h3_skinny : Mm::h3;
  }
  const bool seq = k.h3 && !k.scaled && persist && gru_seq_ok(L == 1 ? 2 : 3, B, Hp, T, o, device_cus(o));
  auto step = [&](bool gi_blocked) {
    if (!k.h3) return B <= o.skinny_max_m ? Step::f32_skinny : Step::f32;
    if (k.scaled) return planes_state && gi_blocked ? Step::s16_planes : Step::s16;
    if (seq) return k.gran ? Step::seq_gran : Step::seq;
    return B <= o.skinny_h3_max_m ? Step::h3_skinny : Step::h3;
  };
  k.step0 = step(k.g0blk);
  k.step1 = step(k.gblk);
  k.first = !k.h3 ? (B <= o.skinny_max_m ? First::f32_skinny : First::f32) : seq ? First::in_seq
            : k.scaled && gru_first16_shape_ok(Hp) ? First::h3_16 : First::h3;
  k.reg_collapsed = k.h3 && m->collapse_env && (m->reg_collapsed || !m->reg_packed);
  k.tail_collapsed = k.reg_collapsed && (m->tail_collapsed || !m->enc_packed);
  k.reg = k.h3 && B <= reg_seq_rows_cap(m) && persist ? Reg::seq : Reg::loop;
  k.tail = k.h3 ? h3(B) : f32(B);
  k.blend16 = k.h3 && m->large_scaled && B >= m->blend16_min_n;
  k.input_blend = split(B, kBlendK, 0);
  k.smpl = smpl_small_rows_ok(B, o) && (m->lbs_sparse || !m->smpl_packed) ? Smpl::small : k.blend16 ? Smpl::h3s : k.h3 ? Smpl::h3
           : B <= gemm_skinny_max_m(o) ? Smpl::f32_skinny : Smpl::f32;
  return k;
}

namespace {
const char* name(Rows v) { return v == Rows::pad ? "pad_input_kernel" : v == Rows::split_few ? "split_rows_few_kernel" : "split_rows_kernel"; }
const char* name(Mm v) {
  static const char* const n[] = {"gemm_f32_kernel", "skinny_gemm_kernel", "gemm_h3_kernel", "skinny_gemm_h3_kernel", "gemm_h3s_kernel<1, 3, 4, 3, 4>",
                                  "gemm_h3s_persist16c_kernel<0>", "gemm_h3s_persist16c_kernel<1>"};
  return n[(int)v];
}
const char* name(Step v) {
  static const char* const n[] = {"gru_step_kernel", "skinny_gru_kernel", "gemm_h3_kernel<GRU>", "skinny_gru_h3_kernel", "gru_seq_kernel",
                                  "gru_seq_kernel(granules)", "gru_step16_kernel<false>", "gru_step16_kernel<true>"};
  return n[(int)v];
}
const char* name(First v) {
  static const char* const n[] = {"gru_step_kernel", "skinny_gru_kernel", "gru_first_kernel", "gru_first16_kernel", "(in gru_seq_kernel)"};
  return n[(int)v];
}
const char* name(Smpl v) {
  static const char* const n[] = {"smpl_small_kernel", "smpl_prep_kernel+gemm_f32_kernel+smpl_skin4_kernel", "smpl_prep_kernel+skinny_gemm_kernel+smpl_skin4_kernel",
                                  "smpl_prep_kernel+gemm_h3_kernel+smpl_skin4_kernel", "smpl_prep_kernel+gemm_h3s_persist16c_kernel<1>+smpl_skin4_kernel"};
  return n[(int)v];
}
std::string tail_name(const KernelPlan& k) {
  if (k.tail_collapsed) return "collapsed: one product (skinny_gemm_h3_kernel)";
  const std::string tail = name(k.tail);
  if (k.reg_collapsed) return tail + " + collapsed regressor (skinny_gemm_h3_kernel)";
  if (k.reg == Reg::seq) return "reg_seq_kernel";
  return tail + (k.h3 ? " loop" : " x (2 + 1 + 9)");
}
}

std::string describe_plan(const tepose_model* m, int B, int T) {
  const KernelPlan k = select_kernels(m, B, T, false, true), w = select_kernels(m, B, T, true, true);
  std::string s = std::string("input=") + name(k.input) + ";projection=" + name(k.projection) +
                  ";gi0_layout=" + (k.g0blk ? "frame_major_blocked" : "row_major") + ";gru_step=" + name(k.step0) + ";gru_first=" + name(k.first);
  if (m->L >= 2)
    s += std::string(";projection_l1=") + name(k.proj_l1) + ";gi1_layout=" + (k.gblk ? "blocked" : "row_major") + ";gru_step_l1=" + name(k.step1);
  s += std::string(";projection_one_step=") + name(k.proj_one) + ";tail_regressor=" + tail_name(k) + ";smpl=" + name(k.smpl);
  s += std::string(";projection_window=") + (w.pair ? "skinny_gemm_h3_kernel (pair)" : std::string(name(w.projection)) + " x 2") +
       ";gru_step_window=" + name(w.step0);
  return s;
}

void refresh_kernel_info(tepose_model* m) {
  const std::string d = describe_plan(m, 8192, 16);
  auto field = [&](const char* key) {
    const std::string kk = std::string(";") + key + "=", dd = ";" + d;
    const size_t i = dd.find(kk);
    if (i == std::string::npos) return std::string("?");
    const size_t j = dd.find(';', i + 1);
    return dd.substr(i + kk.size(), j == std::string::npos ? std::string::npos : j - i - kk.size());
  };
  m->kinfo = "projection=" + field("projection") + ";gru_step=" + field("gru_step");
}

}
```

### tepose_amd/csrc/shapes.h

```cpp
#pragma once
#include "formats.h"
#include "options.h"

namespace tepose {

constexpr int kChipCUs = 256;

struct Launch { int kernel; unsigned gx, gy, gz, threads; int a0, a1; };

inline bool split_rows_few_ok(long rows, int Kp, int permT, const Options& o) { return rows <= o.split_few_max_rows && Kp <= 4096 && !permT; }
inline bool gru_first16_shape_ok(int Hp) { return Hp % 128 == 0; }
inline bool gru_seq_shape_ok(int Hp) { return Hp % 256 == 0 && Hp <= 1024; }
inline int gemm_skinny_max_m(const Options& o) { return o.skinny_max_m_gemm >= 0 ? o.skinny_max_m_gemm : o.skinny_max_m; }

enum H3Tile { kH3Tile64x128, kH3Tile128x128, kH3Tile128x192, kH3Tile256x128 };
inline Launch h3_tile_launch(H3Tile k, int tm, int tn, int n) { return {k, (unsigned)(tm * tn), (unsigned)n, 1u, k == kH3Tile64x128 ? 256u : 512u, tm, tn}; }
inline double chip_rounds(double workgroups) { return (double)(long)((workgroups + (kChipCUs - 1.)) / (double)kChipCUs); }
inline double h3_cost128(double w) { return 47. * chip_rounds(w); }
inline double h3_cost64(double w) {
  const double rounds = w / (double)kChipCUs, first_sharing = 1.55;
  return 33. * (w <= (double)kChipCUs ? 1. : (rounds > first_sharing ? rounds : first_sharing));
}
inline double h3_cost192(double w) { return 70. * chip_rounds(w); }
inline Launch h3_product_shape(int M, int N, int n, const Options& o) {
  const int tilesM = (M + 255) / 256, tilesN = (N + 127) / 128;
  if (o.h3_tile == 64) return h3_tile_launch(kH3Tile64x128, (M + 63) / 64, tilesN, n);
  if (o.h3_tile == 192) return h3_tile_launch(kH3Tile128x192, (M + 127) / 128, (N + 191) / 192, n);
  if (o.h3_tile == 256) return h3_tile_launch(kH3Tile256x128, tilesM, tilesN, n);
  if (M <= 2048 && tilesM * tilesN * n < 1024) {
    const int tm = (M + 127) / 128;
    const int tm64 = (M + 63) / 64;
    const double w128 = (double)tm * tilesN * n, w64 = (double)tm64 * tilesN * n;
    const double c64 = h3_cost64(w64), keep128 = 0.9 * h3_cost128(w128);
    if (o.h3_tile192 && N % 192 == 0) {
      const double c192 = h3_cost192((double)tm * (N / 192) * n);
      if (c192 < keep128 && c192 <= c64) return h3_tile_launch(kH3Tile128x192, tm, N / 192, n);
    }
    if (o.h3_tile64 && c64 < keep128) return h3_tile_launch(kH3Tile64x128, tm64, tilesN, n);
    return h3_tile_launch(kH3Tile128x128, tm, tilesN, n);
  }
  return h3_tile_launch(kH3Tile256x128, tilesM, tilesN, n);
}

enum GruH3Rows { kGruH3Rows64, kGruH3Rows128 };
inline Launch gru_h3_shape(int M, int Hp, int n) {
  const int tilesJ = Hp / 64;
  if ((M + 127) / 128 * tilesJ * n <= 160) return {kGruH3Rows64, (unsigned)((M + 63) / 64 * tilesJ), (unsigned)n, 1u, 256u, (M + 63) / 64, tilesJ};
  return {kGruH3Rows128, (unsigned)((M + 127) / 128 * tilesJ), (unsigned)n, 1u, 512u, (M + 127) / 128, tilesJ};
}

enum SkinnyH3 { kSkinnyH3_1x1w8, kSkinnyH3_2x1w8, kSkinnyH3_2x1w4, kSkinnyH3_4x1w8, kSkinnyH3_4x1w4, kSkinnyH3_1, kSkinnyH3_2, kSkinnyH3_3, kSkinnyH3_4 };
inline Launch skinny_h3_product_shape(int maxM, int maxN, int n, const Options& o) {
  const int nt = (maxN + 47) / 48;
  const int nt1_max = o.skinny_nt1_below;
  const unsigned gx16 = (unsigned)((maxN + 15) / 16);
  const int rowtiles = (maxM + 15) / 16;
  if (o.skinny_mt1 != 0 && nt * n < nt1_max && (maxN + 15) / 16 * n * rowtiles <= kChipCUs) return {kSkinnyH3_1x1w8, gx16, (unsigned)rowtiles, (unsigned)n, 512u, 0, 0};
  const bool w8 = o.skinny_w8 != 0 && (maxN + 15) / 16 * n <= 128;
  if (maxM <= 32 && nt * n < nt1_max)
    return {w8 ? kSkinnyH3_2x1w8 : kSkinnyH3_2x1w4, gx16, 1u, (unsigned)n, w8 ? 512u : 256u, 0, 0};
  if (maxM <= 64 && maxM > 32 && nt * n < 96 && o.skinny_narrow64 != 0)
    return {w8 ? kSkinnyH3_4x1w8 : kSkinnyH3_4x1w4, gx16, 1u, (unsigned)n, w8 ? 512u : 256u, 0, 0};
  const int tiles = (maxM + 15) / 16, passes = (tiles + 3) / 4;
  const int mt = o.skinny_mt1 != 0 ? (tiles + passes - 1) / passes : (maxM <= 32 ? 2 : 4);
  return {mt <= 1 ? kSkinnyH3_1 : mt == 2 ? kSkinnyH3_2 : mt == 3 ? kSkinnyH3_3 : kSkinnyH3_4, (unsigned)nt, (unsigned)((tiles + mt - 1) / mt), (unsigned)n, 256u, 0, 0};
}
enum SkinnyRows { kSkinnyRows16, kSkinnyRows32, kSkinnyRows64 };
inline Launch skinny_h3_step_shape(int M, int Hp, int n) {
  if (M <= 32) return {kSkinnyRows32, (unsigned)(Hp / 16), 1u, (unsigned)n, 256u, 0, 0};
  return {kSkinnyRows64, (unsigned)(Hp / 16), (unsigned)((M + 63) / 64), (unsigned)n, 256u, 0, 0};
}
inline Launch skinny_f32_shape(int M, int blocks_x, int n, int nw1) {
  if (M <= 16) return {kSkinnyRows16, (unsigned)blocks_x, 1u, (unsigned)n, (unsigned)(64 * nw1), 0, 0};
  if (M <= 32) return {kSkinnyRows32, (unsigned)blocks_x, 1u, (unsigned)n, 256u, 0, 0};
  return {kSkinnyRows64, (unsigned)blocks_x, (unsigned)((M + 63) / 64), (unsigned)n, 256u, 0, 0};
}
inline Launch skinny_f32_product_shape(int M, int N, int nw1) { return skinny_f32_shape(M, (N + 47) / 48, 1, nw1); }
inline Launch skinny_f32_step_shape(int M, int Hp, int ndir, int nw1) { return skinny_f32_shape(M, Hp / 16, ndir, nw1); }

enum F32Rows { kF32Rows64, kF32Rows128 };
inline Launch f32_tiles_shape(int M, int N, const Options& o) {
  const int tilesN = (N + 127) / 128, tiles128 = (M + 127) / 128;
  if (tiles128 * tilesN <= o.gemm_half_max_blocks) return {kF32Rows64, (unsigned)((M + 63) / 64 * tilesN), 1u, 1u, 256u, (M + 63) / 64, tilesN};
  return {kF32Rows128, (unsigned)(tiles128 * tilesN), 1u, 1u, 256u, tiles128, tilesN};
}

constexpr int kSeqMaxT = 36;
constexpr size_t kSeqGranRows = 4;
inline int gru_seq_gran_rows(const Options& o) { return o.seq_gran_max_m > (int)kSeqGranRows ? (int)kSeqGranRows : o.seq_gran_max_m; }
inline bool gru_seq_ok(int ndir, int M, int Hp, int T, const Options& o, int cus) {
  const int max_m = o.seq_max_m > 64 ? 64 : o.seq_max_m;
  return M >= 1 && M <= max_m && T >= 2 && T <= kSeqMaxT && gru_seq_shape_ok(Hp) && ndir >= 1 &&
         ndir <= 3 && ndir * (Hp / 16) <= cus;
}
inline int gru_seq_row_tiles(int M) { return M <= 16 ? 1 : M <= 32 ? 2 : M <= 48 ? 3 : 4; }
inline Launch gru_seq_shape(int M, int Hp, int ndir) { return {gru_seq_row_tiles(M), (unsigned)(Hp / 16), 1u, (unsigned)ndir, 512u, 0, 0}; }

inline Launch h3s16c_shape(int M, int N) {
  const int tilesM = (M + 255) / 256, tilesN = (N + 255) / 256, nt = tilesM * tilesN;
  return {0, (unsigned)(nt < kChipCUs ? nt : kChipCUs), 1u, 1u, 512u, tilesM, tilesN};
}
inline int h3s16c_gm_arg(int gm_opt, int walk_opt) { return (gm_opt >= 1 && gm_opt <= 32 ? gm_opt : 8) | (walk_opt == 1 ? 1 << 16 : 0); }
inline Launch gru_step16_shape(int M, int Hp, int n) { return {0, (unsigned)((M + 127) / 128 * (Hp / 64)), (unsigned)n, 1u, 256u, (M + 127) / 128, Hp / 64}; }
inline int gru_step16_gm(int gm_opt) { return gm_opt >= 1 && gm_opt <= 64 ? gm_opt : 4; }
inline bool h3s_mid_cols_ok(int N) { return N % 288 == 0; }
inline Launch h3s_mid_shape(int M, int N) { return {0, (unsigned)((M + 127) / 128 * (N / 288)), 1u, 1u, 768u, (M + 127) / 128, N / 288}; }
inline bool g0_mid_fewer_rounds(long BT, int Hp) {
  const long rt = (BT + 127) / 128;
  const long r_mid = (rt * (9 * Hp / 288) + (kChipCUs - 1)) / kChipCUs, r_old = (rt * ((9 * Hp + 127) / 128) + (kChipCUs - 1)) / kChipCUs;
  return 2.1 * (double)r_mid <= (double)r_old + 0.15;
}

constexpr int kSkinPG = 32;
inline Launch skin_shape(int N) {
  const int vb = (kNV + 255) / 256;
  int pg = (int)((long)N * vb / 512);
  pg = pg < 1 ? 1 : (pg > kSkinPG ? kSkinPG : pg);
  return {0, (unsigned)vb, (unsigned)((N + pg - 1) / pg), 1u, 256u, 0, pg};
}

constexpr int kBwdSrc = 54;
constexpr int kBwdSkinVB = 512;
constexpr int kBwdSkinBlocks = (kNV + kBwdSkinVB - 1) / kBwdSkinVB;
constexpr int kBwdSkinSlice = 25;
constexpr int kBwdSkinSlices = (kBwdSkinVB + kBwdSkinSlice - 1) / kBwdSkinSlice;
static_assert(kBwdSkinSlices * kNJ <= kBwdSkinVB, "one reducing thread per (slice, joint)");
inline Launch skin_bwd_shape(int N) {
  int pg = (int)((long)N * kBwdSkinBlocks / 512);
  pg = pg < 1 ? 1 : (pg > kSkinPG ? kSkinPG : pg);
  return {0, (unsigned)kBwdSkinBlocks, (unsigned)((N + pg - 1) / pg), 1u, (unsigned)kBwdSkinVB, 0, pg};
}
constexpr int kBwdBlendRows = 3 * kNV;
constexpr int kBwdChunk = 64;
constexpr int kBwdChunks = (kBwdBlendRows + kBwdChunk - 1) / kBwdChunk;
enum BlendBwdTile { kBlendBwd8, kBlendBwd32 };
inline int blend_bwd_persons(int kernel) { return kernel == kBlendBwd8 ? 8 : 32; }
inline Launch blend_bwd_shape(int N) {
  const int kernel = N <= 8 ? kBlendBwd8 : kBlendBwd32, pt = blend_bwd_persons(kernel);
  const int tiles = (N + pt - 1) / pt;
  int splits = (8 * kChipCUs + tiles - 1) / tiles;
  splits = splits < 1 ? 1 : (splits > kBwdChunks ? kBwdChunks : splits);
  const int per = (kBwdChunks + splits - 1) / splits;
  splits = (kBwdChunks + per - 1) / per;
  return {kernel, (unsigned)splits, (unsigned)tiles, 1u, 128u, per, 0};
}
inline Launch chain_bwd_shape(int N) { return {0, (unsigned)((N + 3) / 4), 1u, 1u, 256u, 0, 0}; }
inline Launch joints_bwd_shape(int N) { return {0, (unsigned)N, 1u, 1u, 192u, 0, 0}; }
inline Launch blend_bwd_sum_shape(int N) { return {0, (unsigned)(((long)N * kBlendK + 63) / 64), 1u, 1u, 256u, 0, 0}; }
constexpr int kSmplBwdMaxN = 1 << 16;
struct SmplBwdFloats { size_t gsrc, gvp, skin_part, blend_part, gf; };
inline size_t blend_bwd_part_rows(int N) {
  const size_t a = (size_t)kBwdChunks * (size_t)N, b = (size_t)(8 * kChipCUs * 32 + 32) + (size_t)N;
  return a < b ? a : b;
}
inline SmplBwdFloats smpl_bwd_floats(int N) {
  const size_t n = (size_t)N;
  return {n * kBwdSrc * 3, n * kVertLd, n * kBwdSkinBlocks * kNJ * 12, blend_bwd_part_rows(N) * kBlendK, n * kBlendK};
}
inline int chain_depths(const int* parents, int* depth) {
  int maxd = 0;
  depth[0] = 0;
  for (int j = 1; j < kNJ; ++j) { depth[j] = depth[parents[j]] + 1; if (depth[j] > maxd) maxd = depth[j]; }
  return maxd;
}
inline void chain_bwd_order(const int* parents, int* order) {
  int depth[kNJ], n = 0;
  const int maxd = chain_depths(parents, depth);
  for (int lvl = maxd; lvl >= 0; --lvl)
    for (int j = 0; j < kNJ; ++j)
      if (depth[j] == lvl) order[n++] = j;
}

constexpr int kSessionMaxSlots = 4096;
inline Launch session_advance_shape(int S) { return {0, (unsigned)((kInput + 255) / 256), (unsigned)S, 1u, 256u, 0, 0}; }
inline Launch session_commit_shape(int S) { return {0, (unsigned)((S * kTheta + 127) / 128), 1u, 1u, 128u, 0, 0}; }
inline Launch session_smooth_shape(int S) { return {0, (unsigned)((S * kTheta + 127) / 128), 1u, 1u, 128u, 0, 0}; }

constexpr int kCropBlock = 256;
constexpr int kCropMaxSide = 32768;
inline Launch crop_shape(int S, int n) { return {0, (unsigned)(((long)S * S + kCropBlock - 1) / kCropBlock), (unsigned)(n < 65535 ? n : 65535), 1u, (unsigned)kCropBlock, 0, 0}; }

}
```

### tepose_amd/csrc/smpl.hip

```cpp
#include "device.h"

namespace tepose {

__global__ void __launch_bounds__(256) smpl_joint_consts_kernel(const float* __restrict__ vt,
                                                                const float* __restrict__ sd,
                                                                const float* __restrict__ jr,
                                                                float* J0, float* JS) {
  const int l = blockIdx.x % 11, jc = blockIdx.x / 11, c = jc % 3, j = jc / 3;
  double acc = 0.0;
  for (int v = threadIdx.x; v < kNV; v += 256) {
    const double w = jr[(long)j * kNV + v];
    const double x = l == 0 ? vt[v * 3 + c] : sd[((long)v * 3 + c) * 10 + (l - 1)];
    acc += w * x;
  }
  __shared__ double red[256];
  red[threadIdx.x] = acc;
  __syncthreads();
  for (int s = 128; s > 0; s >>= 1) {
    if (threadIdx.x < s) red[threadIdx.x] += red[threadIdx.x + s];
    __syncthreads();
  }
  if (threadIdx.x == 0) {
    if (l == 0) J0[j * 3 + c] = (float)red[0];
    else JS[(j * 3 + c) * 10 + (l - 1)] = (float)red[0];
  }
}

__global__ void __launch_bounds__(256) smpl_blendw_kernel(const float* __restrict__ vt,
                                                          const float* __restrict__ sd,
                                                          const float* __restrict__ pd, float* bw) {
  const long total = (long)kBlendN * kBlendK;
  for (long idx = (long)blockIdx.x * 256 + threadIdx.x; idx < total; idx += (long)gridDim.x * 256) {
    const int n = (int)(idx / kBlendK), k = (int)(idx % kBlendK);
    float v = 0.f;
    if (n < 3 * kNV) {
      if (k == 0) v = vt[n];
      else if (k <= 10) v = sd[(long)n * 10 + (k - 1)];
      else if (k < 218) v = pd[(long)(k - 11) * (3 * kNV) + n];
    }
    bw[idx] = v;
  }
}

hipError_t launch_smpl_consts(const float* vt, const float* sd, const float* pd, const float* jr,
                              float* J0, float* JS, float* blendW, hipStream_t s) {
  hipLaunchKernelGGL(smpl_joint_consts_kernel, dim3(24 * 3 * 11), dim3(256), 0, s, vt, sd, jr, J0, JS);
  hipLaunchKernelGGL(smpl_blendw_kernel, dim3(4096), dim3(256), 0, s, vt, sd, pd, blendW);
  return hipGetLastError();
}

__global__ void __launch_bounds__(256) csr_build_kernel(const float* __restrict__ dense, int rows,
                                                        int cols, int* ptr, int* idx, float* val,
                                                        int cap) {
  __shared__ int wsum[4];
  __shared__ int base_sh;
  const int row = blockIdx.x, tid = threadIdx.x, lane = tid & 63, wave = tid >> 6;
  int cnt = 0;
  for (long i = tid; i < (long)row * cols; i += 256) cnt += dense[i] != 0.f;
  for (int o = 32; o > 0; o >>= 1) cnt += __shfl_down(cnt, o);
  if (lane == 0) wsum[wave] = cnt;
  __syncthreads();
  if (tid == 0) base_sh = wsum[0] + wsum[1] + wsum[2] + wsum[3];
  __syncthreads();
  int base = base_sh;
  if (tid == 0) ptr[row] = base;
  for (int c0 = 0; c0 < cols; c0 += 256) {
    const int c = c0 + tid;
    const float v = c < cols ? dense[(long)row * cols + c] : 0.f;
    const bool nz = v != 0.f;
    const unsigned long long m = __ballot(nz);
    const int before = __popcll(m & ((1ull << lane) - 1ull));
    __syncthreads();
    if (lane == 0) wsum[wave] = __popcll(m);
    __syncthreads();
    int off = base + before;
    for (int w = 0; w < wave; ++w) off += wsum[w];
    if (nz && off < cap) { idx[off] = c; val[off] = v; }
    base += wsum[0] + wsum[1] + wsum[2] + wsum[3];
  }
  if (row == rows - 1 && tid == 0) ptr[rows] = base;
}

hipError_t launch_csr_build(const float* dense, int rows, int cols, int* ptr, int* idx, float* val,
                            int cap, hipStream_t s) {
  hipLaunchKernelGGL(csr_build_kernel, dim3(rows), dim3(256), 0, s, dense, rows, cols, ptr, idx, val, cap);
  return hipGetLastError();
}

__device__ __forceinline__ void rotmat_to_aa(const float R[3][3], float aa[3]) {
#pragma clang fp contract(off)
  const float m00 = R[0][0], m01 = R[1][0], m02 = R[2][0];
  const float m10 = R[0][1], m11 = R[1][1], m12 = R[2][1];
  const float m20 = R[0][2], m21 = R[1][2], m22 = R[2][2];
  const bool d2 = m22 < 1e-6f, d01 = m00 > m11, d0n1 = m00 < -m11;
  float w, x, y, z, t;
  if (d2 && d01) {
    t = 1.f + m00 - m11 - m22; w = m12 - m21; x = t; y = m01 + m10; z = m20 + m02;
  } else if (d2) {
    t = 1.f - m00 + m11 - m22; w = m20 - m02; x = m01 + m10; y = t; z = m12 + m21;
  } else if (d0n1) {
    t = 1.f - m00 - m11 + m22; w = m01 - m10; x = m20 + m02; y = m12 + m21; z = t;
  } else {
    t = 1.f + m00 + m11 + m22; w = t; x = m12 - m21; y = m20 - m02; z = m01 - m10;
  }
  const float st = sqrtf(t);
  w = (w / st) * 0.5f; x = (x / st) * 0.5f; y = (y / st) * 0.5f; z = (z / st) * 0.5f;
  const float s2 = x * x + y * y + z * z;
  const float sn = sqrtf(s2);
  const float two_theta = 2.f * (w < 0.f ? atan2f(-sn, -w) : atan2f(sn, w));
  const float k = s2 > 0.f ? two_theta / sn : 2.f;
  aa[0] = x * k; aa[1] = y * k; aa[2] = z * k;
#pragma unroll
  for (int i = 0; i < 3; ++i)
    if (aa[i] != aa[i]) aa[i] = 0.f;
}

__device__ __forceinline__ void rot6d_to_rotmat(const float* __restrict__ x, float R[3][3]) {
#pragma clang fp contract(off)
  const float a1[3] = {x[0], x[2], x[4]};
  const float a2[3] = {x[1], x[3], x[5]};
  const float n1 = fmaxf(sqrtf(a1[0] * a1[0] + a1[1] * a1[1] + a1[2] * a1[2]), 1e-6f);
  const float b1[3] = {a1[0] / n1, a1[1] / n1, a1[2] / n1};
  const float dp = b1[0] * a2[0] + b1[1] * a2[1] + b1[2] * a2[2];
  const float u[3] = {a2[0] - dp * b1[0], a2[1] - dp * b1[1], a2[2] - dp * b1[2]};
  const float n2 = fmaxf(sqrtf(u[0] * u[0] + u[1] * u[1] + u[2] * u[2]), 1e-6f);
  const float b2[3] = {u[0] / n2, u[1] / n2, u[2] / n2};
  const float b3[3] = {b1[1] * b2[2] - b1[2] * b2[1], b1[2] * b2[0] - b1[0] * b2[2],
                       b1[0] * b2[1] - b1[1] * b2[0]};
#pragma unroll
  for (int r = 0; r < 3; ++r) { R[r][0] = b1[r]; R[r][1] = b2[r]; R[r][2] = b3[r]; }
}

struct PrepIn {
  const float* pose; int pose_ld;
  const float* betas; int betas_ld;
  const float* cam; int cam_ld;
  int mode;
  half_t *pf_hi, *pf_lo; long pf_kst;
};
__device__ __forceinline__ void pf_put(const PrepIn& in, float* f, long p, int col, float v) {
  f[col] = v;
  if (in.pf_hi) {
    const long o = (long)(col >> 5) * in.pf_kst + plane_index(p, col & 31, 0);
    split_hi_lo(v, in.pf_hi[o], in.pf_lo[o]);
  }
}
__device__ __forceinline__ void smpl_prep_person(const SmplConsts& c, int maxdepth, const PrepIn& in, int p, int lane,
                                                 float* A_p, float* f, float* posed_p, float* rotmat_p, float* th) {
  const float* x = in.pose + (long)p * in.pose_ld;
  const float* bx = in.betas + (long)p * in.betas_ld;
  const int mode = in.mode;
  const int j = lane < kNJ ? lane : 0;
  const bool act = lane < kNJ;
  float R[3][3];
  float beta[10];
#pragma unroll
  for (int l = 0; l < 10; ++l) beta[l] = bx[l];
  if (mode == 2) {
#pragma unroll
    for (int r = 0; r < 3; ++r)
#pragma unroll
      for (int cc = 0; cc < 3; ++cc) R[r][cc] = x[9 * j + 3 * r + cc];
  } else if (mode == 1) {
    const float ax = x[3 * j], ay = x[3 * j + 1], az = x[3 * j + 2];
    const float ex = ax + 1e-8f, ey = ay + 1e-8f, ez = az + 1e-8f;
    const float ang = sqrtf(ex * ex + ey * ey + ez * ez);
    const float rx = ax / ang, ry = ay / ang, rz = az / ang;
    const float sn = sinf(ang), cs = 1.f - cosf(ang);
    const float K[3][3] = {{0.f, -rz, ry}, {rz, 0.f, -rx}, {-ry, rx, 0.f}};
#pragma unroll
    for (int r = 0; r < 3; ++r)
#pragma unroll
      for (int cc = 0; cc < 3; ++cc) {
        const float kk = K[r][0] * K[0][cc] + K[r][1] * K[1][cc] + K[r][2] * K[2][cc];
        R[r][cc] = (r == cc ? 1.f : 0.f) + sn * K[r][cc] + cs * kk;
      }
  } else {
    rot6d_to_rotmat(x + 6 * j, R);
  }
  float aa[3] = {0.f, 0.f, 0.f};
  if (th) rotmat_to_aa(R, aa);

  float Jr[3];
#pragma unroll
  for (int cc = 0; cc < 3; ++cc) {
    float v = c.J0[j * 3 + cc];
#pragma unroll
    for (int l = 0; l < 10; ++l) v += c.JS[(j * 3 + cc) * 10 + l] * beta[l];
    Jr[cc] = v;
  }
  const int par = act ? c.parents[j] : -1;
  const int dep = act ? c.depth[j] : 0;
  const int src = par < 0 ? 0 : par;
  float rel[3];
#pragma unroll
  for (int cc = 0; cc < 3; ++cc) {
    const float pj = __shfl(Jr[cc], src);
    rel[cc] = par < 0 ? Jr[cc] : Jr[cc] - pj;
  }
  float G[3][4];
#pragma unroll
  for (int r = 0; r < 3; ++r) { G[r][0] = R[r][0]; G[r][1] = R[r][1]; G[r][2] = R[r][2]; G[r][3] = rel[r]; }
  for (int lvl = 1; lvl <= maxdepth; ++lvl) {
    float P[3][4];
#pragma unroll
    for (int r = 0; r < 3; ++r)
#pragma unroll
      for (int cc = 0; cc < 4; ++cc) P[r][cc] = __shfl(G[r][cc], src);
    if (dep == lvl) {
#pragma unroll
      for (int r = 0; r < 3; ++r) {
#pragma unroll
        for (int cc = 0; cc < 3; ++cc)
          G[r][cc] = P[r][0] * R[0][cc] + P[r][1] * R[1][cc] + P[r][2] * R[2][cc];
        G[r][3] = P[r][0] * rel[0] + P[r][1] * rel[1] + P[r][2] * rel[2] + P[r][3];
      }
    }
  }
  if (act) {
    float* Ao = A_p + j * 12;
#pragma unroll
    for (int r = 0; r < 3; ++r) {
      Ao[r * 4 + 0] = G[r][0]; Ao[r * 4 + 1] = G[r][1]; Ao[r * 4 + 2] = G[r][2];
      Ao[r * 4 + 3] = G[r][3] - (G[r][0] * Jr[0] + G[r][1] * Jr[1] + G[r][2] * Jr[2]);
      if (posed_p) posed_p[j * 3 + r] = G[r][3];
      if (rotmat_p) {
        float* Ro = rotmat_p + j * 9;
        Ro[r * 3 + 0] = R[r][0]; Ro[r * 3 + 1] = R[r][1]; Ro[r * 3 + 2] = R[r][2];
      }
    }
    if (th) { th[3 + 3 * j + 0] = aa[0]; th[3 + 3 * j + 1] = aa[1]; th[3 + 3 * j + 2] = aa[2]; }
    if (j >= 1) {
#pragma unroll
      for (int r = 0; r < 3; ++r)
#pragma unroll
        for (int cc = 0; cc < 3; ++cc) pf_put(in, f, p, 11 + 9 * (j - 1) + 3 * r + cc, R[r][cc] - (r == cc ? 1.f : 0.f));
    } else {
      pf_put(in, f, p, 0, 1.f);
#pragma unroll
      for (int l = 0; l < 10; ++l) { pf_put(in, f, p, 1 + l, beta[l]); if (th) th[75 + l] = beta[l]; }
#pragma unroll
      for (int l = 218; l < kBlendK; ++l) pf_put(in, f, p, l, 0.f);
      if (th && in.cam) { const float* cm = in.cam + (long)p * in.cam_ld; th[0] = cm[0]; th[1] = cm[1]; th[2] = cm[2]; }
    }
  }
}

__global__ void __launch_bounds__(256) smpl_prep_kernel(SmplConsts c, int maxdepth, PrepIn in, int N,
                                                        float* __restrict__ pf, float* __restrict__ Amat,
                                                        float* __restrict__ posed,
                                                        float* __restrict__ rotmat,
                                                        float* __restrict__ theta) {
  const int lane = threadIdx.x & 63;
  const int p = blockIdx.x * 4 + (threadIdx.x >> 6);
  if (p >= N) return;
  smpl_prep_person(c, maxdepth, in, p, lane, Amat + (long)p * kNJ * 12, pf + (long)p * kBlendK,
                   posed ? posed + (long)p * kNJ * 3 : nullptr, rotmat ? rotmat + (long)p * kNJ * 9 : nullptr,
                   theta ? theta + (long)p * kTheta : nullptr);
}

__global__ void __launch_bounds__(256) smpl_skin_kernel(const float* __restrict__ lbsW,
                                                        const float* __restrict__ vposed,
                                                        const float* __restrict__ Amat, int N,
                                                        float* __restrict__ verts, int pg) {
  __shared__ float As[kNJ * 12];
  const int v = blockIdx.x * 256 + threadIdx.x;
  const bool ok = v < kNV;
  float w[kNJ];
#pragma unroll
  for (int j = 0; j < kNJ; ++j) w[j] = ok ? lbsW[(long)v * kNJ + j] : 0.f;
  const int p0 = blockIdx.y * pg;
  const int p1 = min(p0 + pg, N);
  for (int p = p0; p < p1; ++p) {
    __syncthreads();
    for (int i = threadIdx.x; i < kNJ * 12; i += 256) As[i] = Amat[(long)p * kNJ * 12 + i];
    __syncthreads();
    float t[12];
#pragma unroll
    for (int e = 0; e < 12; ++e) t[e] = 0.f;
#pragma unroll
    for (int j = 0; j < kNJ; ++j)
#pragma unroll
      for (int e = 0; e < 12; ++e) t[e] += w[j] * As[j * 12 + e];
    if (ok) {
      const float* vp = vposed + (long)p * kVertLd + 3 * v;
      const float x = vp[0], y = vp[1], z = vp[2];
      float* o = verts + ((long)p * kNV + v) * 3;
      o[0] = t[0] * x + t[1] * y + t[2] * z + t[3];
      o[1] = t[4] * x + t[5] * y + t[6] * z + t[7];
      o[2] = t[8] * x + t[9] * y + t[10] * z + t[11];
    }
  }
}

__global__ void __launch_bounds__(256) lbs_compact_kernel(const float* __restrict__ lbsW, int* __restrict__ cidx,
                                                          float* __restrict__ cval, int* __restrict__ max_nnz) {
  const int v = blockIdx.x * 256 + threadIdx.x;
  if (v >= kNV) return;
  int n = 0;
  for (int j = 0; j < kNJ; ++j) {
    const float w = lbsW[(long)v * kNJ + j];
    if (w != 0.f) {
      if (n < 4) { cidx[v * 4 + n] = j; cval[v * 4 + n] = w; }
      ++n;
    }
  }
  for (int k = n; k < 4; ++k) { cidx[v * 4 + k] = 0; cval[v * 4 + k] = 0.f; }
  atomicMax(max_nnz, n);
}

hipError_t launch_lbs_compact(const float* lbsW, int* cidx, float* cval, int* max_nnz, hipStream_t s) {
  hipError_t e = hipMemsetAsync(max_nnz, 0, sizeof(int), s);
  if (e != hipSuccess) return e;
  hipLaunchKernelGGL(lbs_compact_kernel, dim3((kNV + 255) / 256), dim3(256), 0, s, lbsW, cidx, cval, max_nnz);
  return hipGetLastError();
}

#ifndef TEPOSE_SKIN_DIAG
#define TEPOSE_SKIN_DIAG 0
#endif
#if TEPOSE_SKIN_DIAG
__device__ unsigned tepose_skin_check_buf[16 + 64 * 32];
extern "C" int tepose_debug_skin_check(unsigned* host, int n, int reset) {
  int rc = (int)hipMemcpyFromSymbol(host, HIP_SYMBOL(tepose_skin_check_buf), (size_t)n * 4);
  if (reset) { unsigned z = 0; rc |= (int)hipMemcpyToSymbol(HIP_SYMBOL(tepose_skin_check_buf), &z, 4); }
  return rc;
}
__device__ unsigned long long tepose_skin_diag_buf[64 * 27 * 4 * 4];
extern "C" int tepose_debug_skin_diag(unsigned long long* host, int n) {
  return (int)hipMemcpyFromSymbol(host, HIP_SYMBOL(tepose_skin_diag_buf), (size_t)n * 8);
}
#endif
__global__ void __launch_bounds__(256) smpl_skin4_kernel(const int* __restrict__ cidx,
                                                         const float* __restrict__ cval,
                                                         const float* __restrict__ vposed,
                                                         const float* __restrict__ Amat, int N,
                                                         float* __restrict__ verts, int pg) {
  __shared__ __attribute__((aligned(16))) float As[kNJ * 12];
#if TEPOSE_SKIN_DIAG
  const unsigned long long diag_t0 = __builtin_amdgcn_s_memrealtime();
  const unsigned diag_hw0 = __builtin_amdgcn_s_getreg((4 << 0) | (0 << 6) | (31 << 11));
#endif
  const int v = blockIdx.x * 256 + threadIdx.x;
  const bool ok = v < kNV;
  int jx[4];
  float wv[4];
#pragma unroll
  for (int k = 0; k < 4; ++k) { jx[k] = ok ? cidx[v * 4 + k] * 12 : 0; wv[k] = ok ? cval[v * 4 + k] : 0.f; }
  const int p0 = blockIdx.y * pg;
  const int p1 = min(p0 + pg, N);
  static_assert(kNJ * 12 <= 512, "two loads per thread cover the transforms");
  float a0 = 0.f, a1 = 0.f, nx = 0.f, ny = 0.f, nz = 0.f;
  if (p0 < p1) {
    a0 = Amat[(long)p0 * kNJ * 12 + threadIdx.x];
    if (threadIdx.x + 256 < kNJ * 12) a1 = Amat[(long)p0 * kNJ * 12 + 256 + threadIdx.x];
    if (ok) { const float* vp = vposed + (long)p0 * kVertLd + 3 * v; nx = vp[0]; ny = vp[1]; nz = vp[2]; }
  }
  for (int p = p0; p < p1; ++p) {
    __syncthreads();
    As[threadIdx.x] = a0;
    if (threadIdx.x + 256 < kNJ * 12) As[256 + threadIdx.x] = a1;
    __syncthreads();
    const float x = nx, y = ny, z = nz;
    if (p + 1 < p1) {
      a0 = Amat[(long)(p + 1) * kNJ * 12 + threadIdx.x];
      if (threadIdx.x + 256 < kNJ * 12) a1 = Amat[(long)(p + 1) * kNJ * 12 + 256 + threadIdx.x];
      if (ok) { const float* vp = vposed + (long)(p + 1) * kVertLd + 3 * v; nx = vp[0]; ny = vp[1]; nz = vp[2]; }
    }
    float t[12];
#pragma unroll
    for (int e = 0; e < 12; ++e) t[e] = 0.f;
#pragma unroll
    for (int k = 0; k < 4; ++k) {
      const f32x4 r0 = *(const f32x4*)(As + jx[k]), r1 = *(const f32x4*)(As + jx[k] + 4), r2 = *(const f32x4*)(As + jx[k] + 8);
#pragma unroll
      for (int e = 0; e < 4; ++e) { t[e] += wv[k] * r0[e]; t[4 + e] += wv[k] * r1[e]; t[8 + e] += wv[k] * r2[e]; }
    }
    if (ok) {
      float* o = verts + ((long)p * kNV + v) * 3;
      o[0] = t[0] * x + t[1] * y + t[2] * z + t[3];
      o[1] = t[4] * x + t[5] * y + t[6] * z + t[7];
      o[2] = t[8] * x + t[9] * y + t[10] * z + t[11];
#if TEPOSE_SKIN_DIAG >= 2
      {
        float u[4] = {0.f, 0.f, 0.f, 0.f};
        f32x4 q[4];
#pragma unroll
        for (int k = 0; k < 4; ++k) {
          q[k] = *(volatile const f32x4*)(As + jx[k]);
#pragma unroll
          for (int e = 0; e < 4; ++e) asm volatile("v_fma_f32 %0, %1, %2, %0" : "+v"(u[e]) : "v"(wv[k]), "v"(q[k][e]));
        }
        const bool diff = __float_as_uint(u[0]) != __float_as_uint(t[0]) || __float_as_uint(u[1]) != __float_as_uint(t[1]) ||
                          __float_as_uint(u[2]) != __float_as_uint(t[2]) || __float_as_uint(u[3]) != __float_as_uint(t[3]);
        if (diff) {
          const unsigned slot = atomicAdd(&tepose_skin_check_buf[0], 1u);
          if (slot < 64) {
            unsigned* d = tepose_skin_check_buf + 16 + slot * 32;
            d[0] = (unsigned)p; d[1] = (unsigned)v;
            for (int e = 0; e < 4; ++e) { d[2 + e] = __float_as_uint(t[e]); d[6 + e] = __float_as_uint(u[e]); }
            for (int k = 0; k < 4; ++k) { d[10 + k] = __float_as_uint(wv[k]); d[14 + k] = (unsigned)jx[k]; d[18 + k] = __float_as_uint(q[k][0]); }
          }
        }
      }
#endif
    }
  }
#if TEPOSE_SKIN_DIAG
  if ((threadIdx.x & 63) == 0 && blockIdx.y < 64) {
    const unsigned long long t1 = __builtin_amdgcn_s_memrealtime();
    const unsigned hw1 = __builtin_amdgcn_s_getreg((4 << 0) | (0 << 6) | (31 << 11));
    unsigned long long* d = tepose_skin_diag_buf + (((size_t)blockIdx.y * 27 + blockIdx.x) * 4 + (threadIdx.x >> 6)) * 4;
    d[0] = diag_t0; d[1] = t1; d[2] = diag_hw0; d[3] = hw1;
  }
#endif
}

hipError_t launch_smpl_skin(const SmplConsts& c, const float* vposed, const float* Amat, int N,
                            float* verts, hipStream_t s) {
  if (N <= 0) return hipSuccess;
  const Launch l = skin_shape(N);
  if (c.lbs_sparse)
    hipLaunchKernelGGL(smpl_skin4_kernel, grid_of(l), block_of(l), 0, s, c.lbs_cidx, c.lbs_cval, vposed, Amat, N, verts, l.a1);
  else
    hipLaunchKernelGGL(smpl_skin_kernel, grid_of(l), block_of(l), 0, s, c.lbsW, vposed, Amat, N, verts, l.a1);
  return hipGetLastError();
}

constexpr int kSmallN = 4;
constexpr int kSmallVB = 32;
__global__ void __launch_bounds__(256) smpl_small_kernel(SmplConsts c, int maxdepth, PrepIn in, int N,
                                                         float* __restrict__ Amat, float* __restrict__ posed,
                                                         float* __restrict__ rotmat, float* __restrict__ theta,
                                                         float* __restrict__ verts) {
  __shared__ __attribute__((aligned(16))) float sA[kSmallN][kNJ * 12];
  __shared__ __attribute__((aligned(16))) float spf[kSmallN][kBlendK];
  __shared__ float svp[kSmallN][3 * kSmallVB];
  const int lane = threadIdx.x & 63, wave = threadIdx.x >> 6;
  constexpr int NPASS = 3 * kSmallVB / 32, KQ = kBlendK / 8 / 4;
  static_assert(kBlendK == 8 * 4 * KQ && NPASS * 32 == 3 * kSmallVB, "row cut");
  const int row0 = blockIdx.x * 3 * kSmallVB;
  const int sub = lane & 7;
  f32x4 wv[NPASS][KQ];
#pragma unroll
  for (int i = 0; i < NPASS; ++i) {
    const int gr = row0 + wave * (8 * NPASS) + i * 8 + (lane >> 3);
#pragma unroll
    for (int q = 0; q < KQ; ++q)
      wv[i][q] = gr < 3 * kNV ? *(const f32x4*)(c.blendW + (long)gr * kBlendK + sub * (4 * KQ) + 4 * q) : f32x4{0.f, 0.f, 0.f, 0.f};
  }
  const int sp = threadIdx.x / kSmallVB, sv = blockIdx.x * kSmallVB + (threadIdx.x % kSmallVB);
  const bool sok = sp < N && sv < kNV;
  int jx[4];
  float wj[4];
#pragma unroll
  for (int k = 0; k < 4; ++k) { jx[k] = sok ? c.lbs_cidx[sv * 4 + k] * 12 : 0; wj[k] = sok ? c.lbs_cval[sv * 4 + k] : 0.f; }
  if (wave < N) {
    const bool out = blockIdx.x == 0;
    PrepIn q = in;
    q.pf_hi = nullptr; q.pf_lo = nullptr;
    smpl_prep_person(c, maxdepth, q, wave, lane, sA[wave], spf[wave], out && posed ? posed + (long)wave * kNJ * 3 : nullptr,
                     out && rotmat ? rotmat + (long)wave * kNJ * 9 : nullptr, out && theta ? theta + (long)wave * kTheta : nullptr);
  }
  __syncthreads();
  if (blockIdx.x == 0 && Amat)
    for (int i = threadIdx.x; i < N * kNJ * 12; i += 256) Amat[i] = sA[i / (kNJ * 12)][i % (kNJ * 12)];
  for (int p = 0; p < N; ++p) {
    f32x4 f[KQ];
#pragma unroll
    for (int q = 0; q < KQ; ++q) f[q] = *(const f32x4*)(&spf[p][sub * (4 * KQ) + 4 * q]);
#pragma unroll
    for (int i = 0; i < NPASS; ++i) {
      float a = 0.f;
#pragma unroll
      for (int q = 0; q < KQ; ++q) a += wv[i][q][0] * f[q][0] + wv[i][q][1] * f[q][1] + wv[i][q][2] * f[q][2] + wv[i][q][3] * f[q][3];
      a += __shfl_xor(a, 1);
      a += __shfl_xor(a, 2);
      a += __shfl_xor(a, 4);
      if (sub == 0) svp[p][wave * (8 * NPASS) + i * 8 + (lane >> 3)] = a;
    }
  }
  __syncthreads();
  if (sok) {
    float t[12];
#pragma unroll
    for (int e = 0; e < 12; ++e) t[e] = 0.f;
#pragma unroll
    for (int k = 0; k < 4; ++k) {
      const f32x4 r0 = *(const f32x4*)(&sA[sp][jx[k]]), r1 = *(const f32x4*)(&sA[sp][jx[k] + 4]), r2 = *(const f32x4*)(&sA[sp][jx[k] + 8]);
#pragma unroll
      for (int e = 0; e < 4; ++e) { t[e] += wj[k] * r0[e]; t[4 + e] += wj[k] * r1[e]; t[8 + e] += wj[k] * r2[e]; }
    }
    const int lv = threadIdx.x % kSmallVB;
    const float x = svp[sp][3 * lv], y = svp[sp][3 * lv + 1], z = svp[sp][3 * lv + 2];
    float* o = verts + ((long)sp * kNV + sv) * 3;
    o[0] = t[0] * x + t[1] * y + t[2] * z + t[3];
    o[1] = t[4] * x + t[5] * y + t[6] * z + t[7];
    o[2] = t[8] * x + t[9] * y + t[10] * z + t[11];
  }
}

bool smpl_small_rows_ok(int N, const Options& o) {
  const int max_n = o.smpl_small_max_n < 0 ? 0 : (o.smpl_small_max_n > kSmallN ? kSmallN : o.smpl_small_max_n);
  return N >= 1 && N <= max_n && 256 / kSmallVB >= N;
}

hipError_t launch_smpl_small(const SmplConsts& c, int mode, const float* pose, int pose_ld, const float* betas, int betas_ld,
                             const float* cam, int cam_ld, int N, float* Amat, float* posed, float* rotmat, float* theta,
                             float* verts, hipStream_t s) {
  PrepIn in{pose, pose_ld, betas, betas_ld, cam, cam_ld, mode, nullptr, nullptr, 0};
  hipLaunchKernelGGL(smpl_small_kernel, dim3((kNV + kSmallVB - 1) / kSmallVB), dim3(256), 0, s, c, c.maxdepth, in, N, Amat,
                     posed, rotmat, theta, verts);
  return hipGetLastError();
}

template <int NT>
__global__ void __launch_bounds__(NT) smpl_joints_kernel(SmplConsts c, JregPacked jr, int use_jr,
                                                          const float* __restrict__ verts,
                                                          const float* __restrict__ posed,
                                                          const float* __restrict__ xs, int N,
                                                          float* __restrict__ kp3d,
                                                          float* __restrict__ kp2d) {
  __shared__ float reg[17][3];
  const int p = blockIdx.x, lane = threadIdx.x & 63, wave = threadIdx.x >> 6;
  const float* V = verts + (long)p * kNV * 3;
  const int nrows = use_jr ? 17 : 9;
  const int* ptr = use_jr ? jr.ptr : c.xr_ptr;
  const int* idx = use_jr ? jr.idx : c.xr_idx;
  const float* val = use_jr ? jr.val : c.xr_val;
  for (int row = wave; row < nrows; row += NT / 64) {
    float a0 = 0.f, a1 = 0.f, a2 = 0.f;
    const int e1 = ptr[row + 1];
    for (int e = ptr[row] + lane; e < e1; e += 64) {
      const float wv = val[e];
      const float* q = V + (long)idx[e] * 3;
      a0 += wv * q[0]; a1 += wv * q[1]; a2 += wv * q[2];
    }
    for (int o = 32; o > 0; o >>= 1) {
      a0 += __shfl_down(a0, o); a1 += __shfl_down(a1, o); a2 += __shfl_down(a2, o);
    }
    if (lane == 0) { reg[row][0] = a0; reg[row][1] = a1; reg[row][2] = a2; }
  }
  __syncthreads();
  const int nj = use_jr ? 14 : 49;
  const int k = threadIdx.x;
  if (k < nj) {
    float q[3];
    if (use_jr) {
      const int s = kH36mToJ14[k];
      q[0] = reg[s][0]; q[1] = reg[s][1]; q[2] = reg[s][2];
    } else {
      const int s = kJointMap49[k];
      if (s < 24) {
        const float* ps = posed + ((long)p * kNJ + s) * 3;
        q[0] = ps[0]; q[1] = ps[1]; q[2] = ps[2];
      } else if (s < 45) {
        const float* ps = V + (long)kExtraVerts[s - 24] * 3;
        q[0] = ps[0]; q[1] = ps[1]; q[2] = ps[2];
      } else {
        q[0] = reg[s - 45][0]; q[1] = reg[s - 45][1]; q[2] = reg[s - 45][2];
      }
    }
    float* o3 = kp3d + ((long)p * nj + k) * 3;
    o3[0] = q[0]; o3[1] = q[1]; o3[2] = q[2];
    if (kp2d) {
      const float* cam = xs + (long)p * kState + 154;
      const float tz = 10000.f / (224.f * cam[0] + 1e-9f);
      const float px = q[0] + cam[1], py = q[1] + cam[2], pz = q[2] + tz;
      float* o2 = kp2d + ((long)p * nj + k) * 2;
      o2[0] = (5000.f * (px / pz)) / 112.f;
      o2[1] = (5000.f * (py / pz)) / 112.f;
    }
  }
}

hipError_t launch_smpl_joints(const SmplConsts& c, const JregPacked* jr, const float* verts,
                              const float* posed, const float* xs, int N, float* kp3d, float* kp2d,
                              hipStream_t s) {
  if (N <= 0) return hipSuccess;
  JregPacked j = jr ? *jr : JregPacked{nullptr, nullptr, nullptr};
  if (N <= 16)
    hipLaunchKernelGGL(smpl_joints_kernel<1024>, dim3(N), dim3(1024), 0, s, c, j, jr ? 1 : 0, verts, posed, xs, N, kp3d, kp2d);
  else
    hipLaunchKernelGGL(smpl_joints_kernel<256>, dim3(N), dim3(256), 0, s, c, j, jr ? 1 : 0, verts, posed, xs, N, kp3d, kp2d);
  return hipGetLastError();
}

hipError_t launch_smpl_prep(const SmplConsts& c, const float* xs, int N, float* pf, float* Amat,
                            float* posed, float* rotmat, float* theta, hipStream_t s, void* pf_hi, void* pf_lo,
                            long pf_kst) {
  if (N <= 0) return hipSuccess;
  PrepIn in{xs, kState, xs + kNPose, kState, xs + 154, kState, 0, (half_t*)pf_hi, (half_t*)pf_lo, pf_kst};
  hipLaunchKernelGGL(smpl_prep_kernel, dim3((N + 3) / 4), dim3(256), 0, s, c, c.maxdepth, in, N, pf, Amat,
                     posed, rotmat, theta);
  return hipGetLastError();
}

hipError_t launch_smpl_prep_pose(const SmplConsts& c, int mode, const float* pose, int pose_ld,
                                 const float* betas, int betas_ld, int N, float* pf, float* Amat, float* posed,
                                 hipStream_t s, void* pf_hi, void* pf_lo, long pf_kst) {
  if (N <= 0) return hipSuccess;
  PrepIn in{pose, pose_ld, betas, betas_ld, nullptr, 0, mode, (half_t*)pf_hi, (half_t*)pf_lo, pf_kst};
  hipLaunchKernelGGL(smpl_prep_kernel, dim3((N + 3) / 4), dim3(256), 0, s, c, c.maxdepth, in, N, pf, Amat, posed,
                     (float*)nullptr, (float*)nullptr);
  return hipGetLastError();
}

__global__ void __launch_bounds__(256) smpl_person_kernel(const float* __restrict__ blendW, const int* __restrict__ cidx,
                                                          const float* __restrict__ cval, const float* __restrict__ pf,
                                                          const float* __restrict__ Amat, int N, float* __restrict__ verts) {
  __shared__ __attribute__((aligned(16))) float spf[4][kBlendK];
  __shared__ __attribute__((aligned(16))) float sA[4][kNJ * 12];
  const int lane = threadIdx.x & 63, wave = threadIdx.x >> 6;
  const int p = blockIdx.x * 4 + wave;
  if (p >= N) return;
  for (int i = lane; i < kBlendK; i += 64) spf[wave][i] = pf[(long)p * kBlendK + i];
  for (int i = lane; i < kNJ * 12; i += 64) sA[wave][i] = Amat[(long)p * kNJ * 12 + i];
  __builtin_amdgcn_wave_barrier();
  for (int v = lane; v < kNV; v += 64) {
    float x[3];
#pragma unroll
    for (int c = 0; c < 3; ++c) {
      const f32x4* w = (const f32x4*)(blendW + (long)(3 * v + c) * kBlendK);
      float acc = 0.f;
      for (int k = 0; k < kBlendK / 4; ++k) {
        const f32x4 wv = w[k], fv = *(const f32x4*)(spf[wave] + 4 * k);
        acc += wv[0] * fv[0] + wv[1] * fv[1] + wv[2] * fv[2] + wv[3] * fv[3];
      }
      x[c] = acc;
    }
    float t[12];
#pragma unroll
    for (int e = 0; e < 12; ++e) t[e] = 0.f;
#pragma unroll
    for (int k = 0; k < 4; ++k) {
      const int j = cidx[v * 4 + k] * 12;
      const float wgt = cval[v * 4 + k];
#pragma unroll
      for (int e = 0; e < 12; ++e) t[e] += wgt * sA[wave][j + e];
    }
    float* o = verts + ((long)p * kNV + v) * 3;
    o[0] = t[0] * x[0] + t[1] * x[1] + t[2] * x[2] + t[3];
    o[1] = t[4] * x[0] + t[5] * x[1] + t[6] * x[2] + t[7];
    o[2] = t[8] * x[0] + t[9] * x[1] + t[10] * x[2] + t[11];
  }
}

hipError_t launch_smpl_person(const SmplConsts& c, const float* pf, const float* Amat, int N, float* verts, hipStream_t s) {
  if (N <= 0) return hipSuccess;
  if (!c.lbs_sparse) return hipErrorInvalidValue;
  hipLaunchKernelGGL(smpl_person_kernel, dim3((N + 3) / 4), dim3(256), 0, s, c.blendW, c.lbs_cidx, c.lbs_cval, pf, Amat, N,
                     verts);
  return hipGetLastError();
}

__global__ void __launch_bounds__(256) rotmat_to_aa_kernel(const float* __restrict__ R, int N, float* __restrict__ aa) {
  const int i = blockIdx.x * 256 + threadIdx.x;
  if (i >= N) return;
  float M[3][3], a[3];
#pragma unroll
  for (int r = 0; r < 3; ++r)
#pragma unroll
    for (int c = 0; c < 3; ++c) M[r][c] = R[(long)i * 9 + 3 * r + c];
  rotmat_to_aa(M, a);
  aa[(long)i * 3 + 0] = a[0]; aa[(long)i * 3 + 1] = a[1]; aa[(long)i * 3 + 2] = a[2];
}

__global__ void __launch_bounds__(256) rot6d_to_rotmat_kernel(const float* __restrict__ x6, int N, float* __restrict__ R) {
  const int i = blockIdx.x * 256 + threadIdx.x;
  if (i >= N) return;
  float M[3][3];
  rot6d_to_rotmat(x6 + (long)i * 6, M);
#pragma unroll
  for (int r = 0; r < 3; ++r)
#pragma unroll
    for (int c = 0; c < 3; ++c) R[(long)i * 9 + 3 * r + c] = M[r][c];
}

hipError_t launch_rotmat_to_aa(const float* R, int N, float* aa, hipStream_t s) {
  if (N <= 0) return hipSuccess;
  hipLaunchKernelGGL(rotmat_to_aa_kernel, dim3((N + 255) / 256), dim3(256), 0, s, R, N, aa);
  return hipGetLastError();
}

hipError_t launch_rot6d_to_rotmat(const float* x6, int N, float* R, hipStream_t s) {
  if (N <= 0) return hipSuccess;
  hipLaunchKernelGGL(rot6d_to_rotmat_kernel, dim3((N + 255) / 256), dim3(256), 0, s, x6, N, R);
  return hipGetLastError();
}

}
```

Measured before the change: 297,900 windows/s.

## Gather joint-regressor vertices during skinning and fuse blend-plane split into prep

At pack time, the joint regressor's nonzero vertices get a compact slot table. The skinning kernel then also writes those vertices into a small per-person buffer reused from the FC workspace, so the joints kernel reads a compact set instead of scattered full-mesh vertices. The scaled fp16 hi/lo split of the blend features is now done inside the SMPL prep kernel, which removes a separate split_rows launch and its extra pass over the data. The joints kernel also prefetches its first CSR entries. The cost is extra stores in skinning, a larger packed regressor blob, and aliasing of the FC workspace, which depends on the carve layout.

Result: no change. 299,100 windows/s, median of 6 (+0.4%).

```diff
diff --git a/tepose_amd/csrc/api.hip b/tepose_amd/csrc/api.hip
--- a/tepose_amd/csrc/api.hip
+++ b/tepose_amd/csrc/api.hip
@@ -32,6 +32,8 @@
   m->test_fault = e ? (unsigned)atoi(e) : 0u;
   e = getenv("TEPOSE_BLEND16_MIN_N");
   m->blend16_min_n = e ? atoi(e) : 512;
+  e = getenv("TEPOSE_SKIN_PICKS_MIN_N");
+  m->skin_picks_min_n = e ? atoi(e) : 512;
   e = getenv("TEPOSE_GI_BLK");
   m->gi_blk = e ? atoi(e) : 1;
   refresh_kernel_info(m);
@@ -138,6 +140,7 @@
   if (int* f = option_field(m->opt, n)) *f = (int)value;
   else if (strcmp(n, "S_MIN_B") == 0) m->s_min_b = (int)value;
   else if (strcmp(n, "BLEND16_MIN_N") == 0) m->blend16_min_n = (int)value;
+  else if (strcmp(n, "SKIN_PICKS_MIN_N") == 0) m->skin_picks_min_n = (int)value;
   else if (strcmp(n, "GI_BLK") == 0) m->gi_blk = (int)value;
   else if (strcmp(n, "SEQ_SPIN_LIMIT") == 0) { if (value <= 0) return TEPOSE_E_ARG; m->spin_limit = (unsigned)value; }
   else return TEPOSE_E_ARG;
@@ -152,6 +155,7 @@
   if (const int* f = option_field(o, n)) return *f;
   if (strcmp(n, "S_MIN_B") == 0) return m->s_min_b;
   if (strcmp(n, "BLEND16_MIN_N") == 0) return m->blend16_min_n;
+  if (strcmp(n, "SKIN_PICKS_MIN_N") == 0) return m->skin_picks_min_n;
   if (strcmp(n, "GI_BLK") == 0) return m->gi_blk;
   if (strcmp(n, "SEQ_SPIN_LIMIT") == 0) return (long)m->spin_limit;
   return -1;
diff --git a/tepose_amd/csrc/blob.hip b/tepose_amd/csrc/blob.hip
--- a/tepose_amd/csrc/blob.hip
+++ b/tepose_amd/csrc/blob.hip
@@ -541,13 +541,15 @@
   return write_header(m, s);
 }
 
-size_t tepose_jreg_packed_bytes(void) { return (32 + (size_t)17 * kNV * 2) * 4; }
+size_t tepose_jreg_packed_bytes(void) { return (32 + (size_t)17 * kNV * 2 + 32 + 6912 + (size_t)17 * kNV) * 4; }
 
 int tepose_pack_jreg(const float* J, void* packed, void* stream) {
   if (!J || !packed) return TEPOSE_E_ARG;
   int* p = (int*)packed;
   CK(launch_csr_build(J, 17, kNV, p, p + 32, (float*)(p + 32 + 17 * kNV), 17 * kNV, (hipStream_t)stream));
-  return 0;
-}
-
-}
+  int* q = p + 32 + 2 * 17 * kNV;
+  CK(launch_jreg_picks(J, 17, p, p + 32, q, q + 32, q + 32 + 6912, (hipStream_t)stream));
+  return 0;
+}
+
+}
diff --git a/tepose_amd/csrc/common.h b/tepose_amd/csrc/common.h
--- a/tepose_amd/csrc/common.h
+++ b/tepose_amd/csrc/common.h
@@ -97,15 +97,24 @@
   const int* xr_idx;
   const float* xr_val;
 };
+struct JregPicks {
+  const int* n = nullptr;
+  const int* slot_of = nullptr;
+  const int* idx = nullptr;
+};
 struct JregPacked {
-  const int* ptr; const int* idx; const float* val;
-};
+  const int* ptr = nullptr; const int* idx = nullptr; const float* val = nullptr;
+  JregPicks picks;
+};
+hipError_t launch_jreg_picks(const float* dense, int rows, const int* ptr, const int* idx, int* n_out, int* slot_of, int* pidx, hipStream_t s);
+struct PfScaled { void* hi = nullptr; void* lo = nullptr; float* row_scale = nullptr; long R = 0; };
 hipError_t launch_smpl_prep(const SmplConsts& c, const float* xs, int N, float* pf, float* Amat,
                             float* posed, float* rotmat, float* theta, hipStream_t s, void* pf_hi = nullptr,
-                            void* pf_lo = nullptr, long pf_kst = 0);
+                            void* pf_lo = nullptr, long pf_kst = 0, const PfScaled& p16 = PfScaled{});
 hipError_t launch_smpl_prep_pose(const SmplConsts& c, int mode, const float* pose, int pose_ld,
                                  const float* betas, int betas_ld, int N, float* pf, float* Amat, float* posed,
-                                 hipStream_t s, void* pf_hi = nullptr, void* pf_lo = nullptr, long pf_kst = 0);
+                                 hipStream_t s, void* pf_hi = nullptr, void* pf_lo = nullptr, long pf_kst = 0,
+                                 const PfScaled& p16 = PfScaled{});
 bool smpl_small_rows_ok(int N, const Options& o);
 hipError_t launch_smpl_small(const SmplConsts& c, int mode, const float* pose, int pose_ld, const float* betas, int betas_ld,
                              const float* cam, int cam_ld, int N, float* Amat, float* posed, float* rotmat, float* theta,
@@ -113,10 +122,10 @@
 hipError_t launch_smpl_person(const SmplConsts& c, const float* pf, const float* Amat, int N, float* verts, hipStream_t s);
 hipError_t launch_lbs_compact(const float* lbsW, int* cidx, float* cval, int* max_nnz, hipStream_t s);
 hipError_t launch_smpl_skin(const SmplConsts& c, const float* vposed, const float* Amat, int N,
-                            float* verts, hipStream_t s);
+                            float* verts, hipStream_t s, const JregPicks* pk = nullptr, float* picked = nullptr);
 hipError_t launch_smpl_joints(const SmplConsts& c, const JregPacked* jr, const float* verts,
                               const float* posed, const float* xs, int N, float* kp3d,
-                              float* kp2d, hipStream_t s);
+                              float* kp2d, hipStream_t s, const float* picked = nullptr);
 hipError_t launch_csr_build(const float* dense, int rows, int cols, int* ptr, int* idx, float* val,
                             int cap, hipStream_t s);
 hipError_t launch_smpl_consts(const float* v_template, const float* shapedirs, const float* posedirs,
diff --git a/tepose_amd/csrc/forward.hip b/tepose_amd/csrc/forward.hip
--- a/tepose_amd/csrc/forward.hip
+++ b/tepose_amd/csrc/forward.hip
@@ -70,6 +70,8 @@
   Act feat, xs, h1, h2, pf;
   float *base, *amat, *posed, *vposed;
   half_t *pf16h = nullptr, *pf16l = nullptr; float* pfrs = nullptr;
+  float* picked = nullptr;
+  PfScaled pf16(int N) const { return PfScaled{pf16h, pf16l, pfrs, (long)N}; }
 };
 
 void carve_regressor(const tepose_model* m, const KernelPlan& k, int N, Carver& c, RegWs& w) {
@@ -87,6 +89,8 @@
     w.pf16l = (half_t*)c.f((size_t)N * kBlendK / 2);
     w.pfrs = c.f((size_t)N);
   }
+  static_assert(kPickMax * 3 == 3 * 1024, "a person's picked vertices fit the FC stack's three 1024-float rows");
+  if (k.skin_picks && w.base && w.h1.rows == w.base + (size_t)N * 1024 && w.h2.rows == w.h1.rows + (size_t)N * 1024) w.picked = w.base;
 }
 
 bool carve_regressor(const tepose_model* m, const KernelPlan& k, int N, void* workspace, size_t bytes, RegWs& w) {
@@ -150,7 +154,6 @@
   AOperand A = w.pf.A();
   Epilogue e;
   if (k.smpl == Smpl::h3s) {
-    CK(launch_split_rows(w.pf.rows, kBlendK, N, kBlendK, kBlendK, N, 1, w.pf16h, w.pf16l, w.pfrs, s, k.input_blend == Rows::split_few));
     A.s = Planes{w.pf16h, w.pf16l, (long)N * 16}; A.row_scale = w.pfrs;
     e.sync = w.sync; e.reg = true;
   }
@@ -159,17 +162,24 @@
 }
 
 template <class Small, class Prep>
-int smpl_chain(const tepose_model* m, const KernelPlan& k, const SmplConsts& sc, const RegWs& w, int N, float* verts, hipStream_t s, Small small, Prep prep) {
+int smpl_chain(const tepose_model* m, const KernelPlan& k, const SmplConsts& sc, const RegWs& w, int N, float* verts, hipStream_t s, Small small, Prep prep,
+               const JregPicks* picks = nullptr) {
   if (k.smpl == Smpl::small) return (int)small();
-  CK(prep(w.split ? w.pf.P.hi : nullptr, w.split ? w.pf.P.lo : nullptr, w.pf.P.kst));
+  const bool s16 = k.smpl == Smpl::h3s, blk = w.split && !s16;
+  CK(prep(blk ? w.pf.P.hi : nullptr, blk ? w.pf.P.lo : nullptr, w.pf.P.kst, s16 ? w.pf16(N) : PfScaled{}));
   CK((hipError_t)blend_shapes(m, k, w, N, s));
-  CK(launch_smpl_skin(sc, w.vposed, w.amat, N, verts, s));
-  return 0;
+  CK(launch_smpl_skin(sc, w.vposed, w.amat, N, verts, s, picks, picks ? w.picked : nullptr));
+  return 0;
+}
+bool picks_on(const KernelPlan& k, const SmplConsts& sc, const RegWs& w, const void* jreg_packed) {
+  return k.skin_picks && k.smpl != Smpl::small && sc.lbs_sparse && jreg_packed && w.picked;
 }
 
 JregPacked jreg_view(const void* jreg_packed) {
   const int* p = (const int*)jreg_packed;
-  return JregPacked{p, p + 32, (const float*)(p + 32 + 17 * kNV)};
+  static_assert(kNV <= 6912, "the padded slot table");
+  const int* q = p + 32 + 2 * 17 * kNV;
+  return JregPacked{p, p + 32, (const float*)(p + 32 + 17 * kNV), JregPicks{q, q + 32, q + 32 + 6912}};
 }
 
 struct G0Src {
@@ -585,12 +595,14 @@
   }
   const SmplConsts sc = smpl_consts(m);
   const float* xs = w.xs.rows;
+  const JregPacked jr = jreg_packed ? jreg_view(jreg_packed) : JregPacked{};
+  const bool picks = picks_on(plan, sc, w, jreg_packed);
   CK((hipError_t)smpl_chain(
       m, plan, sc, w, N, verts, s,
       [&] { return launch_smpl_small(sc, 0, xs, kState, xs + kNPose, kState, xs + 154, kState, N, w.amat, w.posed, rotmat, theta, verts, s); },
-      [&](half_t* ph, half_t* pl, long kst) { return launch_smpl_prep(sc, xs, N, w.pf.rows, w.amat, w.posed, rotmat, theta, s, ph, pl, kst); }));
-  const JregPacked jr = jreg_packed ? jreg_view(jreg_packed) : JregPacked{};
-  CK(launch_smpl_joints(sc, jreg_packed ? &jr : nullptr, verts, w.posed, xs, N, kp_3d, kp_2d, s));
+      [&](half_t* ph, half_t* pl, long kst, const PfScaled& p16) { return launch_smpl_prep(sc, xs, N, w.pf.rows, w.amat, w.posed, rotmat, theta, s, ph, pl, kst, p16); },
+      picks ? &jr.picks : nullptr));
+  CK(launch_smpl_joints(sc, jreg_packed ? &jr : nullptr, verts, w.posed, xs, N, kp_3d, kp_2d, s, picks ? w.picked : nullptr));
   return 0;
 }
 
@@ -704,7 +716,7 @@
   CK((hipError_t)smpl_chain(
       m, plan, sc, w, N, verts, s,
       [&] { return launch_smpl_small(sc, mode, pose, pose_ld, betas, 10, nullptr, 0, N, w.amat, w.posed, nullptr, nullptr, verts, s); },
-      [&](half_t* ph, half_t* pl, long kst) { return launch_smpl_prep_pose(sc, mode, pose, pose_ld, betas, 10, N, w.pf.rows, w.amat, w.posed, s, ph, pl, kst); }));
+      [&](half_t* ph, half_t* pl, long kst, const PfScaled& p16) { return launch_smpl_prep_pose(sc, mode, pose, pose_ld, betas, 10, N, w.pf.rows, w.amat, w.posed, s, ph, pl, kst, p16); }));
   if (joints49) CK(launch_smpl_joints(sc, nullptr, verts, w.posed, nullptr, N, joints49, nullptr, s));
   return 0;
 }
@@ -747,7 +759,7 @@
   SmplConsts sc = smpl_consts(m);
   const int mode = pose2rot ? 1 : 2, pose_ld = pose2rot ? 72 : 216;
   CK(launch_smpl_prep_pose(sc, mode, pose, pose_ld, betas, 10, N, w.pf.rows, w.amat, w.posed, s, w.split ? w.pf.P.hi : nullptr,
-                           w.split ? w.pf.P.lo : nullptr, w.pf.P.kst));
+                           w.split ? w.pf.P.lo : nullptr, w.pf.P.kst, plan.smpl == Smpl::h3s ? w.pf16(N) : PfScaled{}));
   CK((hipError_t)blend_shapes(m, plan, w, N, s));
   CK(launch_smpl_joints_bwd(g_joints49, N, b.gsrc, s));
   CK(launch_smpl_skin_bwd(sc, w.vposed, w.amat, g_verts, b.gsrc, N, b.gvp, b.skin_part, s));
@@ -790,7 +802,7 @@
   return smpl_chain(
       m, plan, sc, w, N, verts, s,
       [&] { return launch_smpl_small(sc, 1, theta + 3, kTheta, theta + 75, kTheta, nullptr, 0, N, w.amat, nullptr, nullptr, nullptr, verts, s); },
-      [&](half_t* ph, half_t* pl, long kst) { return launch_smpl_prep_pose(sc, 1, theta + 3, kTheta, theta + 75, kTheta, N, w.pf.rows, w.amat, nullptr, s, ph, pl, kst); });
+      [&](half_t* ph, half_t* pl, long kst, const PfScaled& p16) { return launch_smpl_prep_pose(sc, 1, theta + 3, kTheta, theta + 75, kTheta, N, w.pf.rows, w.amat, nullptr, s, ph, pl, kst, p16); });
 }
 
 int tepose_encoder_fwd(const tepose_model* m, const float* x, int B, int T, int is_train, float* feat,
diff --git a/tepose_amd/csrc/model.h b/tepose_amd/csrc/model.h
--- a/tepose_amd/csrc/model.h
+++ b/tepose_amd/csrc/model.h
@@ -78,6 +78,7 @@
   unsigned* fault = nullptr;
   bool persist = true;
   unsigned spin_limit = 1u << 21;
+  int skin_picks_min_n = 512;
   int blend16_min_n = 512;
   int gi_blk = 1;
   int last_fault_code = 0;
diff --git a/tepose_amd/csrc/plan.h b/tepose_amd/csrc/plan.h
--- a/tepose_amd/csrc/plan.h
+++ b/tepose_amd/csrc/plan.h
@@ -17,13 +17,13 @@
   bool g0blk = false;
   bool gran = false;
   bool blend16 = false;
+  bool skin_picks = false;
   bool reg_collapsed = false;
   bool tail_collapsed = false;
   bool pair = false;
   Rows input = Rows::pad;
   Rows input_x0 = Rows::pad;
   Rows input_pair = Rows::pad;
-  Rows input_blend = Rows::pad;
   Mm projection = Mm::f32;
   Mm proj_l1 = Mm::f32;
   Mm proj_one = Mm::f32;
diff --git a/tepose_amd/csrc/plan.hip b/tepose_amd/csrc/plan.hip
--- a/tepose_amd/csrc/plan.hip
+++ b/tepose_amd/csrc/plan.hip
@@ -53,7 +53,7 @@
   k.reg = k.h3 && B <= reg_seq_rows_cap(m) && persist ? Reg::seq : Reg::loop;
   k.tail = k.h3 ? h3(B) : f32(B);
   k.blend16 = k.h3 && m->large_scaled && B >= m->blend16_min_n;
-  k.input_blend = split(B, kBlendK, 0);
+  k.skin_picks = B >= m->skin_picks_min_n && (m->lbs_sparse || !m->smpl_packed);
   k.smpl = smpl_small_rows_ok(B, o) && (m->lbs_sparse || !m->smpl_packed) ? Smpl::small : k.blend16 ? Smpl::h3s : k.h3 ? Smpl::h3
            : B <= gemm_skinny_max_m(o) ? Smpl::f32_skinny : Smpl::f32;
   return k;
diff --git a/tepose_amd/csrc/shapes.h b/tepose_amd/csrc/shapes.h
--- a/tepose_amd/csrc/shapes.h
+++ b/tepose_amd/csrc/shapes.h
@@ -112,6 +112,7 @@
 }
 
 constexpr int kSkinPG = 32;
+constexpr int kPickMax = 1024;
 inline Launch skin_shape(int N) {
   const int vb = (kNV + 255) / 256;
   int pg = (int)((long)N * vb / 512);
diff --git a/tepose_amd/csrc/smpl.hip b/tepose_amd/csrc/smpl.hip
--- a/tepose_amd/csrc/smpl.hip
+++ b/tepose_amd/csrc/smpl.hip
@@ -87,6 +87,48 @@
   return hipGetLastError();
 }
 
+__global__ void __launch_bounds__(1024) jreg_picks_kernel(const float* __restrict__ dense, int rows, const int* __restrict__ ptr,
+                                                          const int* __restrict__ idx, int* n_out, int* slot_of, int* pidx) {
+  __shared__ int scan[1024];
+  constexpr int VPT = 7;
+  static_assert(1024 * VPT >= kNV, "every vertex has a thread");
+  const int tid = threadIdx.x, v0 = tid * VPT;
+  bool used[VPT];
+  int cnt = 0;
+#pragma unroll
+  for (int i = 0; i < VPT; ++i) {
+    const int v = v0 + i;
+    bool u = false;
+    if (v < kNV)
+      for (int r = 0; r < rows; ++r) u |= dense[(long)r * kNV + v] != 0.f;
+    used[i] = u;
+    cnt += u ? 1 : 0;
+  }
+  scan[tid] = cnt;
+  __syncthreads();
+  for (int o = 1; o < 1024; o <<= 1) {
+    const int add = tid >= o ? scan[tid - o] : 0;
+    __syncthreads();
+    scan[tid] += add;
+    __syncthreads();
+  }
+  int next = scan[tid] - cnt;
+#pragma unroll
+  for (int i = 0; i < VPT; ++i) {
+    const int v = v0 + i;
+    if (v < kNV) slot_of[v] = used[i] ? next++ : -1;
+  }
+  if (tid == 1023) *n_out = scan[1023];
+  __syncthreads();
+  const int nnz = ptr[rows];
+  for (int e = tid; e < nnz; e += 1024) pidx[e] = slot_of[idx[e]];
+}
+
+hipError_t launch_jreg_picks(const float* dense, int rows, const int* ptr, const int* idx, int* n_out, int* slot_of, int* pidx, hipStream_t s) {
+  hipLaunchKernelGGL(jreg_picks_kernel, dim3(1), dim3(1024), 0, s, dense, rows, ptr, idx, n_out, slot_of, pidx);
+  return hipGetLastError();
+}
+
 __device__ __forceinline__ void rotmat_to_aa(const float R[3][3], float aa[3]) {
 #pragma clang fp contract(off)
   const float m00 = R[0][0], m01 = R[1][0], m02 = R[2][0];
@@ -137,16 +179,18 @@
   const float* cam; int cam_ld;
   int mode;
   half_t *pf_hi, *pf_lo; long pf_kst;
+  half_t *pf16_hi = nullptr, *pf16_lo = nullptr; float* pf16_rs = nullptr; long pf16_R = 0;
 };
-__device__ __forceinline__ void pf_put(const PrepIn& in, float* f, long p, int col, float v) {
+__device__ __forceinline__ void pf_put(const PrepIn& in, float* f, float* st, long p, int col, float v) {
   f[col] = v;
+  if (st) st[col] = v;
   if (in.pf_hi) {
     const long o = (long)(col >> 5) * in.pf_kst + plane_index(p, col & 31, 0);
     split_hi_lo(v, in.pf_hi[o], in.pf_lo[o]);
   }
 }
 __device__ __forceinline__ void smpl_prep_person(const SmplConsts& c, int maxdepth, const PrepIn& in, int p, int lane,
-                                                 float* A_p, float* f, float* posed_p, float* rotmat_p, float* th) {
+                                                 float* A_p, float* f, float* posed_p, float* rotmat_p, float* th, float* st = nullptr) {
   const float* x = in.pose + (long)p * in.pose_ld;
   const float* bx = in.betas + (long)p * in.betas_ld;
   const int mode = in.mode;
@@ -234,13 +278,13 @@
 #pragma unroll
       for (int r = 0; r < 3; ++r)
 #pragma unroll
-        for (int cc = 0; cc < 3; ++cc) pf_put(in, f, p, 11 + 9 * (j - 1) + 3 * r + cc, R[r][cc] - (r == cc ? 1.f : 0.f));
+        for (int cc = 0; cc < 3; ++cc) pf_put(in, f, st, p, 11 + 9 * (j - 1) + 3 * r + cc, R[r][cc] - (r == cc ? 1.f : 0.f));
     } else {
-      pf_put(in, f, p, 0, 1.f);
-#pragma unroll
-      for (int l = 0; l < 10; ++l) { pf_put(in, f, p, 1 + l, beta[l]); if (th) th[75 + l] = beta[l]; }
-#pragma unroll
-      for (int l = 218; l < kBlendK; ++l) pf_put(in, f, p, l, 0.f);
+      pf_put(in, f, st, p, 0, 1.f);
+#pragma unroll
+      for (int l = 0; l < 10; ++l) { pf_put(in, f, st, p, 1 + l, beta[l]); if (th) th[75 + l] = beta[l]; }
+#pragma unroll
+      for (int l = 218; l < kBlendK; ++l) pf_put(in, f, st, p, l, 0.f);
       if (th && in.cam) { const float* cm = in.cam + (long)p * in.cam_ld; th[0] = cm[0]; th[1] = cm[1]; th[2] = cm[2]; }
     }
   }
@@ -251,12 +295,52 @@
                                                         float* __restrict__ posed,
                                                         float* __restrict__ rotmat,
                                                         float* __restrict__ theta) {
-  const int lane = threadIdx.x & 63;
-  const int p = blockIdx.x * 4 + (threadIdx.x >> 6);
+  __shared__ __attribute__((aligned(16))) float srow[4][kBlendK];
+  const int lane = threadIdx.x & 63, wave = threadIdx.x >> 6;
+  const int p = blockIdx.x * 4 + wave;
   if (p >= N) return;
+  float* st = in.pf16_hi ? srow[wave] : nullptr;
   smpl_prep_person(c, maxdepth, in, p, lane, Amat + (long)p * kNJ * 12, pf + (long)p * kBlendK,
                    posed ? posed + (long)p * kNJ * 3 : nullptr, rotmat ? rotmat + (long)p * kNJ * 9 : nullptr,
-                   theta ? theta + (long)p * kTheta : nullptr);
+                   theta ? theta + (long)p * kTheta : nullptr, st);
+  if (!st) return;
+  static_assert(kBlendK % 8 == 0 && kBlendK / 8 <= 64, "one 8-column run per lane");
+  __builtin_amdgcn_wave_barrier();
+  const bool mine = lane < kBlendK / 8;
+  float v[8];
+  float mx = 0.f;
+  bool bad = false;
+#pragma unroll
+  for (int i = 0; i < 8; ++i) {
+    v[i] = mine ? st[8 * lane + i] : 0.f;
+    mx = fmaxf(mx, fabsf(v[i]));
+    bad |= !(fabsf(v[i]) <= 3.0e38f);
+  }
+#pragma unroll
+  for (int o = 32; o > 0; o >>= 1) mx = fmaxf(mx, __shfl_xor(mx, o));
+  bad = __any(bad);
+  float sc = 1.f, inv = 1.f;
+  if (mx > 0.f && !bad) {
+    int ex;
+    (void)frexpf(mx, &ex);
+    int e = 14 - ex;
+    e = e > 100 ? 100 : (e < -100 ? -100 : e);
+    sc = ldexpf(1.f, e);
+    inv = ldexpf(1.f, -e);
+  }
+  if (lane == 0) in.pf16_rs[p] = inv;
+  if (mine) {
+    h16x8 h, l;
+#pragma unroll
+    for (int i = 0; i < 8; ++i) {
+      half_t hh, ll;
+      split_hi_lo16(v[i] * sc, hh, ll);
+      h[i] = hh; l[i] = ll;
+    }
+    const long off = plane16_index(p, 8 * lane, in.pf16_R);
+    *(h16x8*)(in.pf16_hi + off) = h;
+    *(h16x8*)(in.pf16_lo + off) = l;
+  }
 }
 
 __global__ void __launch_bounds__(256) smpl_skin_kernel(const float* __restrict__ lbsW,
@@ -335,7 +419,8 @@
                                                          const float* __restrict__ cval,
                                                          const float* __restrict__ vposed,
                                                          const float* __restrict__ Amat, int N,
-                                                         float* __restrict__ verts, int pg) {
+                                                         float* __restrict__ verts, int pg, JregPicks pk,
+                                                         float* __restrict__ picked) {
   __shared__ __attribute__((aligned(16))) float As[kNJ * 12];
 #if TEPOSE_SKIN_DIAG
   const unsigned long long diag_t0 = __builtin_amdgcn_s_memrealtime();
@@ -347,6 +432,8 @@
   float wv[4];
 #pragma unroll
   for (int k = 0; k < 4; ++k) { jx[k] = ok ? cidx[v * 4 + k] * 12 : 0; wv[k] = ok ? cval[v * 4 + k] : 0.f; }
+  const int pick_n = picked ? *pk.n : 0;
+  const int slot = picked && ok && pick_n <= kPickMax ? pk.slot_of[v] : -1;
   const int p0 = blockIdx.y * pg;
   const int p1 = min(p0 + pg, N);
   static_assert(kNJ * 12 <= 512, "two loads per thread cover the transforms");
@@ -378,9 +465,14 @@
     }
     if (ok) {
       float* o = verts + ((long)p * kNV + v) * 3;
-      o[0] = t[0] * x + t[1] * y + t[2] * z + t[3];
-      o[1] = t[4] * x + t[5] * y + t[6] * z + t[7];
-      o[2] = t[8] * x + t[9] * y + t[10] * z + t[11];
+      const float ox = t[0] * x + t[1] * y + t[2] * z + t[3];
+      const float oy = t[4] * x + t[5] * y + t[6] * z + t[7];
+      const float oz = t[8] * x + t[9] * y + t[10] * z + t[11];
+      o[0] = ox; o[1] = oy; o[2] = oz;
+      if (slot >= 0) {
+        float* q = picked + ((long)p * pick_n + slot) * 3;
+        q[0] = ox; q[1] = oy; q[2] = oz;
+      }
 #if TEPOSE_SKIN_DIAG >= 2
       {
         float u[4] = {0.f, 0.f, 0.f, 0.f};
@@ -417,11 +509,13 @@
 }
 
 hipError_t launch_smpl_skin(const SmplConsts& c, const float* vposed, const float* Amat, int N,
-                            float* verts, hipStream_t s) {
+                            float* verts, hipStream_t s, const JregPicks* pk, float* picked) {
   if (N <= 0) return hipSuccess;
+  if (picked && (!pk || !c.lbs_sparse)) return hipErrorInvalidValue;
   const Launch l = skin_shape(N);
   if (c.lbs_sparse)
-    hipLaunchKernelGGL(smpl_skin4_kernel, grid_of(l), block_of(l), 0, s, c.lbs_cidx, c.lbs_cval, vposed, Amat, N, verts, l.a1);
+    hipLaunchKernelGGL(smpl_skin4_kernel, grid_of(l), block_of(l), 0, s, c.lbs_cidx, c.lbs_cval, vposed, Amat, N, verts, l.a1,
+                       pk ? *pk : JregPicks{}, picked);
   else
     hipLaunchKernelGGL(smpl_skin_kernel, grid_of(l), block_of(l), 0, s, c.lbsW, vposed, Amat, N, verts, l.a1);
   return hipGetLastError();
@@ -520,7 +614,8 @@
                                                           const float* __restrict__ posed,
                                                           const float* __restrict__ xs, int N,
                                                           float* __restrict__ kp3d,
-                                                          float* __restrict__ kp2d) {
+                                                          float* __restrict__ kp2d,
+                                                          const float* __restrict__ picked) {
   __shared__ float reg[17][3];
   const int p = blockIdx.x, lane = threadIdx.x & 63, wave = threadIdx.x >> 6;
   const float* V = verts + (long)p * kNV * 3;
@@ -528,13 +623,45 @@
   const int* ptr = use_jr ? jr.ptr : c.xr_ptr;
   const int* idx = use_jr ? jr.idx : c.xr_idx;
   const float* val = use_jr ? jr.val : c.xr_val;
-  for (int row = wave; row < nrows; row += NT / 64) {
+  const float* VR = V;
+  if (picked) {
+    const int pick_n = *jr.picks.n;
+    if (pick_n <= kPickMax) { VR = picked + (long)p * pick_n * 3; idx = jr.picks.idx; }
+  }
+  constexpr int RPW = (17 + NT / 64 - 1) / (NT / 64);
+  int e0[RPW], e1[RPW];
+#pragma unroll
+  for (int r = 0; r < RPW; ++r) {
+    const int row = wave + r * (NT / 64);
+    const bool live = row < nrows;
+    e0[r] = live ? ptr[row] + lane : 0;
+    e1[r] = live ? ptr[row + 1] : 0;
+  }
+  float wv[RPW];
+  int vi[RPW];
+#pragma unroll
+  for (int r = 0; r < RPW; ++r) {
+    const bool on = e0[r] < e1[r];
+    wv[r] = on ? val[e0[r]] : 0.f;
+    vi[r] = on ? idx[e0[r]] : 0;
+  }
+  float q[RPW][3];
+#pragma unroll
+  for (int r = 0; r < RPW; ++r) {
+    const bool on = e0[r] < e1[r];
+#pragma unroll
+    for (int cc = 0; cc < 3; ++cc) q[r][cc] = on ? VR[(long)vi[r] * 3 + cc] : 0.f;
+  }
+#pragma unroll
+  for (int r = 0; r < RPW; ++r) {
+    const int row = wave + r * (NT / 64);
+    if (row >= nrows) continue;
     float a0 = 0.f, a1 = 0.f, a2 = 0.f;
-    const int e1 = ptr[row + 1];
-    for (int e = ptr[row] + lane; e < e1; e += 64) {
-      const float wv = val[e];
-      const float* q = V + (long)idx[e] * 3;
-      a0 += wv * q[0]; a1 += wv * q[1]; a2 += wv * q[2];
+    if (e0[r] < e1[r]) { a0 += wv[r] * q[r][0]; a1 += wv[r] * q[r][1]; a2 += wv[r] * q[r][2]; }
+    for (int e = e0[r] + 64; e < e1[r]; e += 64) {
+      const float w2 = val[e];
+      const float* q2 = VR + (long)idx[e] * 3;
+      a0 += w2 * q2[0]; a1 += w2 * q2[1]; a2 += w2 * q2[2];
     }
     for (int o = 32; o > 0; o >>= 1) {
       a0 += __shfl_down(a0, o); a1 += __shfl_down(a1, o); a2 += __shfl_down(a2, o);
@@ -576,21 +703,23 @@
 
 hipError_t launch_smpl_joints(const SmplConsts& c, const JregPacked* jr, const float* verts,
                               const float* posed, const float* xs, int N, float* kp3d, float* kp2d,
-                              hipStream_t s) {
+                              hipStream_t s, const float* picked) {
   if (N <= 0) return hipSuccess;
-  JregPacked j = jr ? *jr : JregPacked{nullptr, nullptr, nullptr};
+  if (picked && !jr) return hipErrorInvalidValue;
+  JregPacked j = jr ? *jr : JregPacked{};
   if (N <= 16)
-    hipLaunchKernelGGL(smpl_joints_kernel<1024>, dim3(N), dim3(1024), 0, s, c, j, jr ? 1 : 0, verts, posed, xs, N, kp3d, kp2d);
+    hipLaunchKernelGGL(smpl_joints_kernel<1024>, dim3(N), dim3(1024), 0, s, c, j, jr ? 1 : 0, verts, posed, xs, N, kp3d, kp2d, picked);
   else
-    hipLaunchKernelGGL(smpl_joints_kernel<256>, dim3(N), dim3(256), 0, s, c, j, jr ? 1 : 0, verts, posed, xs, N, kp3d, kp2d);
+    hipLaunchKernelGGL(smpl_joints_kernel<256>, dim3(N), dim3(256), 0, s, c, j, jr ? 1 : 0, verts, posed, xs, N, kp3d, kp2d, picked);
   return hipGetLastError();
 }
 
 hipError_t launch_smpl_prep(const SmplConsts& c, const float* xs, int N, float* pf, float* Amat,
                             float* posed, float* rotmat, float* theta, hipStream_t s, void* pf_hi, void* pf_lo,
-                            long pf_kst) {
+                            long pf_kst, const PfScaled& p16) {
   if (N <= 0) return hipSuccess;
   PrepIn in{xs, kState, xs + kNPose, kState, xs + 154, kState, 0, (half_t*)pf_hi, (half_t*)pf_lo, pf_kst};
+  in.pf16_hi = (half_t*)p16.hi; in.pf16_lo = (half_t*)p16.lo; in.pf16_rs = p16.row_scale; in.pf16_R = p16.R;
   hipLaunchKernelGGL(smpl_prep_kernel, dim3((N + 3) / 4), dim3(256), 0, s, c, c.maxdepth, in, N, pf, Amat,
                      posed, rotmat, theta);
   return hipGetLastError();
@@ -598,9 +727,10 @@
 
 hipError_t launch_smpl_prep_pose(const SmplConsts& c, int mode, const float* pose, int pose_ld,
                                  const float* betas, int betas_ld, int N, float* pf, float* Amat, float* posed,
-                                 hipStream_t s, void* pf_hi, void* pf_lo, long pf_kst) {
+                                 hipStream_t s, void* pf_hi, void* pf_lo, long pf_kst, const PfScaled& p16) {
   if (N <= 0) return hipSuccess;
   PrepIn in{pose, pose_ld, betas, betas_ld, nullptr, 0, mode, (half_t*)pf_hi, (half_t*)pf_lo, pf_kst};
+  in.pf16_hi = (half_t*)p16.hi; in.pf16_lo = (half_t*)p16.lo; in.pf16_rs = p16.row_scale; in.pf16_R = p16.R;
   hipLaunchKernelGGL(smpl_prep_kernel, dim3((N + 3) / 4), dim3(256), 0, s, c, c.maxdepth, in, N, pf, Amat, posed,
                      (float*)nullptr, (float*)nullptr);
   return hipGetLastError();
```
